# JamesBrofos/Stein

Measured on AMD Instinct MI355X. Metric: SVGD particle-updates/sec, higher is better.
Workload: dtype f32; 1 GPU; C3 bayesian-logreg-shaped synthetic block n=16384 d=256 fp32 (roofline config); n=16384, d=256, rows_per_rank=16384, optimizer=adagrad lr=1e-3 alpha=0.9, parallelism=single GPU

## Files before the change

stein_amd/csrc/stein_common.h:

```cpp
#pragma once

#include <hip/hip_runtime.h>
#include <stdint.h>
#include <math.h>

#include "steinhip.h"

typedef float f32x16 __attribute__((ext_vector_type(16)));
typedef unsigned long long u64;
typedef unsigned int u32;

int stein_fail(int code, const char* fmt, ...);

#define HIP_TRY(expr)                                                                          \
  do {                                                                                         \
    hipError_t e_ = (expr);                                                                    \
    if (e_ != hipSuccess) return stein_fail(STEIN_E_HIP, "%s: %s", #expr, hipGetErrorString(e_)); \
  } while (0)

#define LAUNCH_CHECK(name)                                                                           \
  do {                                                                                               \
    hipError_t e_ = hipGetLastError();                                                               \
    if (e_ != hipSuccess) return stein_fail(STEIN_E_HIP, "launch %s: %s", name, hipGetErrorString(e_)); \
  } while (0)

constexpr int BM = 128;
constexpr int BN = 128;
constexpr int BK = 32;
constexpr int NTHREADS = 256;

__device__ __forceinline__ int xcd_remap(int bid, int nblk) {
  const int q = nblk >> 3, r = nblk & 7, x = bid & 7;
  return (x < r ? x * (q + 1) : r * (q + 1) + (x - r) * q) + (bid >> 3);
}

constexpr int DT_ROWS = 128, DT_COLS = 32, DT_ELEMS = DT_ROWS * DT_COLS;
__host__ __device__ __forceinline__ size_t d_index(long row, long col, long ntc) {
  return ((size_t)(row >> 7) * ntc + (col >> 5)) * DT_ELEMS + (row & 127) * DT_COLS + (col & 31);
}

__device__ __forceinline__ float4 ld4_or_zero(const float* p, bool ok) {
  return ok ? *reinterpret_cast<const float4*>(p) : make_float4(0.f, 0.f, 0.f, 0.f);
}

constexpr int DSB = 8;
__host__ __device__ __forceinline__ long distance_grid(bool sym, int tiles_m, int tiles_n) {
  const long sm = (tiles_m + DSB - 1) / DSB, sn = (tiles_n + DSB - 1) / DSB;
  return (sym ? sn * (sn + 1) / 2 : sm * sn) * (DSB * DSB);
}
template <bool SYM>
__device__ __forceinline__ bool distance_tile(int logical, int tiles_m, int tiles_n, int& tile_m, int& tile_n) {
  const int sb = logical / (DSB * DSB), in = logical % (DSB * DSB);
  int sbm, sbn;
  if (SYM) {
    const int t_ = (tiles_n + DSB - 1) / DSB;
    int tm = (int)(((2.0 * t_ + 1.0) - sqrt((2.0 * t_ + 1.0) * (2.0 * t_ + 1.0) - 8.0 * (double)sb)) * 0.5);
    tm = max(0, min(tm, t_ - 1));
    while (tm > 0 && (long)tm * t_ - (long)tm * (tm - 1) / 2 > sb) --tm;
    while ((long)(tm + 1) * t_ - (long)(tm + 1) * tm / 2 <= sb) ++tm;
    sbm = tm;
    sbn = tm + (sb - (int)((long)tm * t_ - (long)tm * (tm - 1) / 2));
  } else {
    const int sn = (tiles_n + DSB - 1) / DSB;
    sbm = sb / sn;
    sbn = sb % sn;
  }
  tile_m = sbm * DSB + in / DSB;
  tile_n = sbn * DSB + in % DSB;
  return tile_m < tiles_m && tile_n < tiles_n && (!SYM || tile_n >= tile_m);
}

struct SelState {
  u64 rank[2];
  u32 prefix[2];
  u32 diverged;
  u32 even;
  float median;
  float h2;
  float lo, hi;
  u32 pad[4];
};
static_assert(sizeof(SelState) == 64, "SelState must stay 64 bytes");

struct SpecState {
  u32 magic;
  u32 center;
  u32 halfwidth;
  u32 lo_key;
  u32 width;
  u32 count;
  u32 overflow;
  u32 hit;
  u32 earned_hw;
  u32 reserved;
  u64 total;
  u32 last_key;
  u32 skip_l0;
  u32 n_steps;
  u32 n_hits;
};
static_assert(sizeof(SpecState) == 64, "SpecState must stay 64 bytes");
struct FuseState {
  u32 pad0[2];
  u32 gave_up;
  u32 folded;
  u32 pad[12];
};
static_assert(sizeof(FuseState) == 64, "FuseState must stay 64 bytes");
constexpr int HS_NV = 2048;
constexpr int HS_CLASSES = 64;
struct HistSync {
  u32 claim[STEIN_HIST_LEVELS][HS_NV];
  struct Leaf { u32 done; u32 pad[15]; } leaf[STEIN_HIST_LEVELS][HS_CLASSES];
  struct Top { u32 classes; u32 pad[15]; } top[STEIN_HIST_LEVELS];
  struct Line { u32 gen; u32 pub[6]; u32 pad[9]; } line[HS_CLASSES];
  Leaf fin_leaf[HS_CLASSES];
  Top fin_top;
  Leaf cm_leaf[HS_CLASSES];
  Top cm_top;
};
__device__ __forceinline__ bool tree_report_done(HistSync::Leaf* leaf, HistSync::Top* top, u32 id, u32 nblocks) {
  const u32 c = id % HS_CLASSES;
  const u32 quota = (nblocks - c + HS_CLASSES - 1) / HS_CLASSES;
  if (__hip_atomic_fetch_add(&leaf[c].done, 1u, __ATOMIC_RELAXED, __HIP_MEMORY_SCOPE_AGENT) + 1u != quota) return false;
  const u32 nclasses = nblocks < (u32)HS_CLASSES ? nblocks : (u32)HS_CLASSES;
  return __hip_atomic_fetch_add(&top->classes, 1u, __ATOMIC_RELAXED, __HIP_MEMORY_SCOPE_AGENT) + 1u == nclasses;
}
static_assert(sizeof(HistSync) % 8 == 0, "HistSync is carved out of a u64 table");
constexpr u32 SPEC_MAGIC1 = 0x5EED0001u, SPEC_MAGIC2 = 0x5EED0002u;
constexpr u32 SPEC_QCAP = 1016;
constexpr u32 SPEC_CAP = (1u << 21) - 2048u;
constexpr u32 SPEC_SLOTS = 256;
constexpr u32 SPEC_HW_MAX = 32767;
constexpr u32 SPEC_TABLE_HDR = 8;
constexpr u32 SPEC_TABLE = SPEC_TABLE_HDR + 2 * SPEC_HW_MAX + 2;
constexpr u32 SPEC_TABLE_AT = SPEC_SLOTS * 8 + SPEC_CAP;
static_assert(SPEC_TABLE_AT == (1u << 21), "the table starts 2^21 words into the SPEC section (stein_amd/_lib.py)");

__device__ __forceinline__ u32 f32_key(float x) {
  const u32 u = __float_as_uint(x);
  return (u & 0x80000000u) ? ~u : (u | 0x80000000u);
}
__device__ __forceinline__ float key_f32(u32 k) {
  return __uint_as_float((k & 0x80000000u) ? (k & 0x7fffffffu) : ~k);
}

struct MedianBw { float med, h2; };
__device__ __forceinline__ MedianBw median_bandwidth(float lo, float hi, u32 even, float ln_n) {
  MedianBw m;
  m.med = even ? 0.5f * (lo + hi) : lo;
  const float bw = sqrtf(m.med / ln_n);
  m.h2 = bw * bw;
  return m;
}

__device__ __forceinline__ void ksd_terms(float g, double og, float ot, float th, float rs, double ih, double& s, double& sd) {
  const double gd = g, dk = ((double)rs * (double)th - (double)ot) * ih;
  s += gd * og + 2.0 * (gd - (double)th * ih) * dk + (double)rs * ih;
  sd += gd * gd + ih;
}

__device__ __forceinline__ float elem_f32(const float* p) { return *p; }
__device__ __forceinline__ float elem_f32(const unsigned short* p) { return __uint_as_float((u32)*p << 16); }

template <typename TIN>
__device__ __forceinline__ float wave_row_sqnorm(const TIN* row, int d, int lane) {
  float s = 0.f;
  for (int k = lane; k < d; k += 64) {
    const float x = elem_f32(row + k);
    s = fmaf(x, x, s);
  }
#pragma unroll
  for (int o = 32; o > 0; o >>= 1) s += __shfl_xor(s, o);
  return s;
}

template <int N>
__device__ __forceinline__ void block_sum256(double (&v)[N], double* red) {
#pragma unroll
  for (int k = 0; k < N; ++k)
#pragma unroll
    for (int o = 32; o > 0; o >>= 1) v[k] += __shfl_xor(v[k], o);
  if ((threadIdx.x & 63) == 0) {
#pragma unroll
    for (int k = 0; k < N; ++k) red[4 * k + (threadIdx.x >> 6)] = v[k];
  }
  __syncthreads();
#pragma unroll
  for (int k = 0; k < N; ++k) v[k] = (red[4 * k] + red[4 * k + 1]) + (red[4 * k + 2] + red[4 * k + 3]);
}

__device__ __forceinline__ u64 load_fresh(const u64* p) { return __hip_atomic_load(p, __ATOMIC_RELAXED, __HIP_MEMORY_SCOPE_AGENT); }
__device__ __forceinline__ u32 load_fresh(const u32* p) { return __hip_atomic_load(p, __ATOMIC_RELAXED, __HIP_MEMORY_SCOPE_AGENT); }

__device__ __forceinline__ void hist_add(u32* h, u32 digit, bool valid, int lane, u32 w = 1u) {
#pragma unroll
  for (int it = 0; it < 2; ++it) {
    const u64 act = __ballot(valid);
    if (act == 0ull) return;
    const int leader = __ffsll((long long)act) - 1;
    const u32 ld = (u32)__builtin_amdgcn_readlane((int)digit, leader);
    const bool same = valid && digit == ld;
    const u64 m = __ballot(same);
    if (lane == leader) atomicAdd(&h[ld], (u32)__popcll(m) * w);
    valid = valid && !same;
  }
  if (valid) atomicAdd(&h[digit], w);
}

constexpr int EPI_STAGE_LD = 132;
constexpr int EPI_STAGE_BYTES = 64 * EPI_STAGE_LD * 4;
constexpr int EPI_LDS_BYTES = EPI_STAGE_BYTES + 8192 + 64 + 1024;

__device__ __forceinline__ void store_d4(float* p, float a, float b, float c, float d) {
  *reinterpret_cast<float4*>(p) = make_float4(a, b, c, d);
}

__device__ __forceinline__ void distance_store_rows(const float* __restrict__ stage, float* __restrict__ D, long ntc,
                                                    int tile_m, int brow0, int p) {
  const int t = threadIdx.x, f4 = t & 31;
#pragma unroll
  for (int k = 0; k < 8; ++k) {
    const int sr = (t >> 5) + 8 * k;
    const int row = tile_m * BM + (sr >> 5) * 64 + p * 32 + (sr & 31);
    const float4 v4 = *reinterpret_cast<const float4*>(stage + sr * EPI_STAGE_LD + 4 * f4);
    store_d4(D + d_index(row, brow0 + 4 * f4, ntc), v4.x, v4.y, v4.z, v4.w);
  }
}

struct SpecCtx {
  u32 lo, width;
  u32* qcnt;
  u64* q;
  u32 below;
};

template <bool MIRROR, bool PRED, bool DIAG, bool HIST, bool SPEC, bool STOREM>
__device__ __forceinline__ void distance_epilogue_body(const f32x16 (&acc)[2][2], u32* hl, float* __restrict__ D, int n,
                                                       int n_local, long ldD, int tile_m, int brow0, u32 base,
                                                       u64& packed, float two_s,
                                                       SpecCtx& sx, const float* rr, const float* rc, int i,
                                                       float* __restrict__ stage) {
  constexpr bool STAGED = !PRED && !DIAG;
  const long ntc = ldD >> 5;
  const int t = threadIdx.x, lane = t & 63, wid = t >> 6;
  const int wy = wid >> 1, wx = wid & 1;
  const int l31 = lane & 31, h4 = (lane >> 5) * 4;
  u32 below_cnt = 0u;
  {
#pragma unroll
    for (int j = 0; j < 2; ++j) {
      const int col = brow0 + wx * 64 + j * 32 + l31;
      const bool cok = !PRED || col < n;
      const float rj = rc[wx * 64 + j * 32 + l31];
#pragma unroll
      for (int g = 0; g < 4; ++g) {
        const int lrow4 = tile_m * BM + wy * 64 + i * 32 + 8 * g + h4;
        const float4 ri4 = *reinterpret_cast<const float4*>(rr + wy * 64 + i * 32 + 8 * g + h4);
        const float ris[4] = {ri4.x, ri4.y, ri4.z, ri4.w};
        float v[4];
        u32 wq[4];
#pragma unroll
        for (int q = 0; q < 4; ++q) {
          const int lrow = lrow4 + q;
          const bool rok = !PRED || lrow < n_local;
          v[q] = (ris[q] + rj) - two_s * acc[i][j][4 * g + q];
          u32 w = MIRROR ? 2u : 1u;
          if (DIAG) w = lrow < col ? 2u : (lrow == col ? 1u : 0u);
          if (PRED && !(cok && rok)) w = 0u;
          wq[q] = w;
          if ((!PRED && !DIAG) || w) {
            if (STAGED) stage[(wy * 32 + 8 * g + h4 + q) * EPI_STAGE_LD + wx * 64 + j * 32 + l31] = v[q];
            else D[d_index(lrow, col, ntc)] = v[q];
          }
        }
        if (DIAG) {
          if (wq[0] == 2u && wq[3] == 2u) {
            *reinterpret_cast<float4*>(D + d_index(col, lrow4, ntc)) = make_float4(v[0], v[1], v[2], v[3]);
          } else {
#pragma unroll
            for (int q = 0; q < 4; ++q)
              if (wq[q] == 2u) D[d_index(col, lrow4 + q, ntc)] = v[q];
          }
        }
        if (HIST) {
          u32 dg[4];
          bool far = false;
#pragma unroll
          for (int q = 0; q < 4; ++q) {
            dg[q] = f32_key(v[q]) >> 21;
            const u32 off = dg[q] - base;
            const bool near = off < 8u;
            packed += near ? (u64)wq[q] << (8u * (off & 7u)) : 0ull;
            far |= !near && wq[q] != 0u;
          }
          if (__builtin_expect(far, 0)) {
#pragma unroll
            for (int q = 0; q < 4; ++q)
              if (dg[q] - base >= 8u && wq[q]) atomicAdd(&hl[dg[q]], wq[q]);
          }
        }
        if (SPEC) {
          u32 off[4];
#pragma unroll
          for (int q = 0; q < 4; ++q) {
            const u32 raw = __float_as_uint(v[q]);
            const bool lower = (int)raw < (int)sx.lo;
            if (!PRED && !DIAG) below_cnt += lower ? 1u : 0u;
            else sx.below += lower ? wq[q] : 0u;
            off[q] = raw - sx.lo;
            if ((PRED || DIAG) && wq[q] == 0u) off[q] = 0xffffffffu;
          }
          if (__builtin_expect(min(min(off[0], off[1]), min(off[2], off[3])) <= sx.width, 0)) {
#pragma unroll
            for (int q = 0; q < 4; ++q)
              if (off[q] <= sx.width) {
                const u32 slot = atomicAdd(sx.qcnt, 1u);
                if (slot < SPEC_QCAP) sx.q[slot] = ((u64)(__float_as_uint(v[q]) | 0x80000000u) << 2) | wq[q];
              }
          }
        }
        if (MIRROR && STOREM && cok && (!PRED || lrow4 < n_local))
          store_d4(D + d_index(col, lrow4, ntc), v[0], v[1], v[2], v[3]);
      }
    }
  }
  if (SPEC && !PRED && !DIAG) sx.below += below_cnt * (MIRROR ? 2u : 1u);
}

struct EpiPrefetch {
  float norm;
  u32 lo_key, width;
};
__device__ __forceinline__ EpiPrefetch distance_epilogue_prefetch(const float* __restrict__ r, int n, int row0,
                                                                  int n_local, int tile_m, int tile_n,
                                                                  const SpecState* __restrict__ spec) {
  EpiPrefetch pf;
  const int t = threadIdx.x;
  const int idx = t < BM ? tile_m * BM + t : tile_n * BN + (t - BM);
  const bool ok = t < BM ? idx < n_local : idx < n;
  pf.norm = ok ? r[(t < BM ? row0 : 0) + idx] : 0.f;
  pf.lo_key = spec ? spec->lo_key : 0xffffffffu;
  pf.width = spec ? spec->width : 0u;
  return pf;
}

template <bool SYM, bool STORE_MIRROR = SYM>
__device__ __forceinline__ void distance_epilogue(const f32x16 (&acc)[2][2], u32* lds, float* __restrict__ D, int n,
                                                  int n_local, long ldD, int tile_m, int tile_n,
                                                  u64* __restrict__ hist0,
                                                  const EpiPrefetch& pf, float two_s = 2.f,
                                                  SpecState* __restrict__ spec = nullptr,
                                                  u64* __restrict__ spec_buf = nullptr) {
  const int t = threadIdx.x, lane = t & 63, wid = t >> 6;
  const int wy = wid >> 1, wx = wid & 1;
  const int brow0 = tile_n * BN;
  float* stage = reinterpret_cast<float*>(lds);
  u32* hl = lds + EPI_STAGE_BYTES / 4;
  u64 packed = 0ull;
  u32 base = 0u;
  SpecCtx sx;
  sx.lo = 0xffffffffu; sx.width = 0u; sx.below = 0u;
  sx.qcnt = hl + STEIN_HIST_BINS;
  sx.q = reinterpret_cast<u64*>(hl);
  static_assert(8 * SPEC_QCAP <= 4 * STEIN_HIST_BINS, "the window queue lives in the histogram's LDS");
  float* rr = reinterpret_cast<float*>(hl + STEIN_HIST_BINS + 16);
  float* rc = rr + BM;
  rr[t] = pf.norm;
  const bool window = spec && pf.width != 0u;
  const bool hist = hist0 && !window;
  if (window) {
    if (t == 0) { sx.qcnt[0] = 0u; sx.qcnt[2] = 0u; }
    sx.lo = pf.lo_key & 0x7fffffffu;
    sx.width = pf.width;
  }
  if (hist) {
    for (int b = t; b < STEIN_HIST_BINS; b += NTHREADS) hl[b] = 0u;
    __syncthreads();
    const float v0 = (rr[wy * 64] + rc[wx * 64]) - two_s * acc[0][0][0];
    base = (u32)__builtin_amdgcn_readfirstlane((int)(f32_key(v0) >> 21));
    base = base < 3u ? 0u : base - 3u;
  } else {
    __syncthreads();
  }
  const bool diag = SYM && tile_m == tile_n;
  const bool edge = brow0 + BN > n || tile_m * BM + BM > n_local;
#define STEIN_EPI_I(MIRROR, PRED, DIAG, I)                                                                             \
  do {                                                                                                                 \
    if (window)                                                                                                        \
      distance_epilogue_body<MIRROR, PRED, DIAG, false, true, STORE_MIRROR>(acc, hl, D, n, n_local, ldD, tile_m, brow0,             \
                                                              base, packed, two_s, sx, rr, rc, I, stage);             \
    else if (hist)                                                                                                     \
      distance_epilogue_body<MIRROR, PRED, DIAG, true, false, STORE_MIRROR>(acc, hl, D, n, n_local, ldD, tile_m, brow0,             \
                                                              base, packed, two_s, sx, rr, rc, I, stage);             \
    else                                                                                                               \
      distance_epilogue_body<MIRROR, PRED, DIAG, false, false, STORE_MIRROR>(acc, hl, D, n, n_local, ldD, tile_m, brow0,            \
                                                               base, packed, two_s, sx, rr, rc, I, stage);            \
  } while (0)
  const long ntc = ldD >> 5;
  if (diag) {
    STEIN_EPI_I(false, true, true, 0);
    STEIN_EPI_I(false, true, true, 1);
  } else if (edge) {
    STEIN_EPI_I(SYM, true, false, 0);
    STEIN_EPI_I(SYM, true, false, 1);
  } else {
    STEIN_EPI_I(SYM, false, false, 0);
    __syncthreads();
    distance_store_rows(stage, D, ntc, tile_m, brow0, 0);
    __syncthreads();
    STEIN_EPI_I(SYM, false, false, 1);
    __syncthreads();
    distance_store_rows(stage, D, ntc, tile_m, brow0, 1);
  }
#undef STEIN_EPI_I
  if (hist) {
#pragma unroll
    for (int k = 0; k < 8; ++k) {
      u32 c = (u32)(packed >> (8 * k)) & 255u;
#pragma unroll
      for (int o = 32; o > 0; o >>= 1) c += __shfl_xor(c, o);
      if (lane == 0 && c) atomicAdd(&hl[base + k], c);
    }
    __syncthreads();
    for (int b = t; b < STEIN_HIST_BINS; b += NTHREADS)
      if (hl[b]) atomicAdd(&hist0[b], (u64)hl[b]);
  }
  if (window) {
    u32 b = sx.below;
#pragma unroll
    for (int o = 32; o > 0; o >>= 1) b += __shfl_xor(b, o);
    if (lane == 0 && b) atomicAdd(&sx.qcnt[2], b);
    __syncthreads();
    if (t == 0 && sx.qcnt[2])
      atomicAdd(reinterpret_cast<unsigned long long*>(spec_buf + (blockIdx.x % SPEC_SLOTS) * 8),
                (unsigned long long)sx.qcnt[2]);
    const u32 pushed = sx.qcnt[0];
    const u32 nq = min(pushed, SPEC_QCAP);
    if (nq) {
      __syncthreads();
      if (t == 0) {
        if (pushed > SPEC_QCAP) spec->overflow = 1u;
        sx.qcnt[1] = atomicAdd(&spec->count, nq);
      }
      __syncthreads();
      const u32 gbase = sx.qcnt[1];
      for (u32 i = t; i < nq; i += NTHREADS)
        if (gbase + i < SPEC_CAP) spec_buf[SPEC_SLOTS * 8 + gbase + i] = sx.q[i];
    }
  }
}

__device__ __forceinline__ void phi_epilogue(const f32x16 (&acc)[2][2], const float (&rs)[4], float* __restrict__ Oz,
                                             float* __restrict__ RSz, int d, int n_local, int i0, int c0,
                                             bool write_rowsum) {
  const int t = threadIdx.x, lane = t & 63, wid = t >> 6;
  const int wy = wid >> 1, wx = wid & 1;
  const int l31 = lane & 31, h4 = (lane >> 5) * 4;
  const int lr = t >> 3;
#pragma unroll
  for (int i = 0; i < 2; ++i) {
#pragma unroll
    for (int j = 0; j < 2; ++j) {
      const int col = c0 + wx * 64 + j * 32 + l31;
      if (col >= d) continue;
#pragma unroll
      for (int e = 0; e < 16; ++e) {
        const int row = i0 + wy * 64 + i * 32 + (e & 3) + 8 * (e >> 2) + h4;
        if (row < n_local) Oz[(size_t)row * d + col] = acc[i][j][e];
      }
    }
  }
  if (write_rowsum) {
#pragma unroll
    for (int p = 0; p < 4; ++p) {
      float s = rs[p];
      s += __shfl_xor(s, 1);
      s += __shfl_xor(s, 2);
      s += __shfl_xor(s, 4);
      const int row = i0 + lr + 32 * p;
      if ((t & 7) == 0 && row < n_local) RSz[row] = s;
    }
  }
}

struct SteinLayout {
  size_t off[STEIN_WS_NSECTIONS];
  size_t total;
  int64_t ld_dist, split, sq_blocks, jchunk, tiles_m, cblocks;
  int64_t x3_rows, x3_dk;
  int64_t x3_dc, x3_nk;
  size_t x3_t3, x3_tt3, x3_gt3;
  size_t x3_sc;
  int64_t fold, fsplit, fjchunk;
  size_t fold_ow, fold_ot, fold_rs;
};
int stein_make_layout(int64_t n_local, int64_t n, int64_t d, int dtype, int flags, SteinLayout* L);

__device__ __forceinline__ void median_init_body(int gt, int gn, SelState* st, SpecState* sp, u64 total,
                                                 u64* __restrict__ hist, u64* __restrict__ slots, int allow_window = 1) {
  for (int i = gt; i < STEIN_HIST_LEVELS * 2 * STEIN_HIST_BINS; i += gn) hist[i] = 0ull;
  for (int i = gt; i < (int)SPEC_SLOTS * 8; i += gn) slots[i] = 0ull;
  if (gt) return;
  {
    const u32 even = (total & 1ull) ? 0u : 1u;
    st->rank[0] = even ? total / 2 - 1 : total / 2;
    st->rank[1] = total / 2;
    st->prefix[0] = st->prefix[1] = 0u;
    st->diverged = 0u;
    st->even = even;
    st->median = st->h2 = st->lo = st->hi = 0.f;
  }
  if (allow_window && (sp->magic == SPEC_MAGIC1 || sp->magic == SPEC_MAGIC2) && sp->halfwidth <= SPEC_HW_MAX &&
      sp->center >= 0x80000000u + sp->halfwidth && sp->center < 0xff000000u - sp->halfwidth) {
    sp->lo_key = sp->center - sp->halfwidth;
    sp->width = 2u * sp->halfwidth;
  } else {
    sp->lo_key = 0xffffffffu;
    sp->width = 0u;
  }
  sp->count = 0u; sp->overflow = 0u; sp->hit = 0u;
  sp->skip_l0 = sp->width == 0u ? 1u : 0u;
  sp->reserved = 0ull; sp->total = total;
}


struct PrologueArgs {
  int n, d;
  float* r;
  SelState* st; SpecState* sp; FuseState* fs;
  u64 total;
  u64* hist; u64* slots;
  u32* cmax; int ncmax;
  int allow_window;
  float* neutral_sc; int dc;
  u32* hsync; int hsync_words;
  u32 folded;
};
constexpr int PRO_INIT_BLOCKS = 16;
template <typename TIN>
__device__ __forceinline__ void prologue_body(const TIN* __restrict__ T, const PrologueArgs& a, int b, int nb) {
  const int gt = b * 256 + (int)threadIdx.x, gn = nb * 256;
  for (int i = gt; i < a.ncmax; i += gn) a.cmax[i] = 0u;
  if (a.neutral_sc) {
    for (int i = gt; i < 4 * a.dc; i += gn) a.neutral_sc[i] = 1.f;
    if (gt == 0) { a.neutral_sc[4 * a.dc] = 1.f; a.neutral_sc[4 * a.dc + 1] = 2.f; a.neutral_sc[4 * a.dc + 2] = 1.f; }
  }
  if (gt < 16) reinterpret_cast<u32*>(a.fs)[gt] = gt == 3 ? a.folded : 0u;
  for (int i = gt; i < a.hsync_words; i += gn) a.hsync[i] = 0u;
  median_init_body(gt, gn, a.st, a.sp, a.total, a.hist, a.slots, a.allow_window);
  const int lane = threadIdx.x & 63;
  for (int row = gt >> 6; row < a.n; row += gn >> 6) {
    const float s = wave_row_sqnorm(T + (size_t)row * a.d, a.d, lane);
    if (lane == 0) a.r[row] = s;
  }
}
```

stein_amd/csrc/stein_host.h:

```cpp
#pragma once

#include "stein_common.h"

#define fail stein_fail

constexpr int MAX_DEVICES = 64;

static inline int grid_for(long count, int cap) {
  long b = (count + 255) / 256;
  if (b > cap) b = cap;
  if (b < 1) b = 1;
  return (int)b;
}

static inline size_t align_up(size_t x, size_t a) { return (x + a - 1) / a * a; }

constexpr double RESIDENT_ONE_PER_CU = 256.0;

static inline int stein_check_size(int64_t n, int64_t d) {
  if (n > (1ll << 30) || d > (1ll << 24) || n * d > (1ll << 40)) return fail(STEIN_E_SHAPE, "shape too large");
  return STEIN_OK;
}

static inline SpecState* spec_of(void* select_state) { return (SpecState*)((char*)select_state + sizeof(SelState)); }
static inline FuseState* fuse_of(void* select_state) { return (FuseState*)((char*)spec_of(select_state) + sizeof(SpecState)); }
static inline u64* spec_table_of(void* spec_buf) { return (u64*)spec_buf + SPEC_TABLE_AT; }

struct BlockShape { int64_t n, d, row0, n_local; int dtype; };

static inline size_t x3_sc_two_s(int64_t dc) { return (size_t)(4 * dc + 1); }
static inline size_t x3_sc_cmax(int64_t dc) { return (size_t)(4 * dc + 4); }

struct StepViews {
  SteinLayout L;
  float* r; float* D; u64* hist;
  SelState* sel; SpecState* spec; FuseState* fuse;
  u64* spec_buf; u64* table;
  char* planes;
  unsigned short* T3; unsigned short* Tt3; unsigned short* Gt3;
  float* sc; u32* cmax; float* two_s;
  float* OG; float* OT; float* RS; double* SQ;
  int nsplit, jchunk, tsplit;
};
StepViews stein_step_views(const SteinLayout& L, void* workspace, void* planes_override = nullptr);
static inline int stein_staged_flags(bool x3) { return (x3 ? STEIN_FLAG_X3 : 0) | STEIN_FLAG_NO_FOLD; }
static inline int stein_rank_flags(int flags) {
  return (flags & (STEIN_FLAG_X3 | STEIN_FLAG_KSD)) | STEIN_FLAG_TILED | STEIN_FLAG_NO_FOLD;
}

int stein_rank_views(const BlockShape& b, void* workspace, size_t ws_bytes, int flags, StepViews* v);
int stein_rank_begin_on(const StepViews& v, const BlockShape& b, const void* theta_all, bool window, hipStream_t stream);
int stein_rank_pick_on(const StepViews& v, int64_t n, float* h2_out, float* median_out, void* flags_host, hipStream_t stream);
int stein_rank_radix_on(const StepViews& v, const BlockShape& b, int level, int need_pass, float* h2_out, float* median_out,
                        hipStream_t stream);
int stein_rank_finish_on(const StepViews& v, const BlockShape& b, const void* theta_all, const void* score_all,
                         const float* h2_dev, float* phi_local, double* sqnorm_out, float* dK_out, int flags,
                         hipStream_t stream);

int stein_device_error_word(u32** out);
int stein_take_device_error(void);

int stein_stream_jsplit_hook(void);

int stein_fused_select(const StepViews& v, int64_t n, int64_t d, float* h2_out, const void* theta_all, const void* score_all,
                       hipStream_t stream);

int stein_fp32_distance(const StepViews& v, const BlockShape& b, const float* theta_all, bool symmetric, bool window,
                        hipStream_t stream);
int stein_fp32_contract_partial(const StepViews& v, const BlockShape& b, const float* theta_all, const float* score_all,
                                const float* h2_dev, hipStream_t stream);

bool stein_small_ok(int64_t n, int64_t d, int dtype);
int stein_small_phi(const float* theta, const float* score, int64_t n, int64_t d, float* phi, float* h2_out,
                    double* sqpart ,
                    float* K_out, float* dK_out, int* nparts ,
                    double* sqnorm_out, bool ksd ,
                    hipStream_t stream);
```

stein_amd/csrc/stein_select.hip:

```cpp

#include <hip/hip_runtime.h>
#include <stdint.h>
#include <math.h>

#include "stein_host.h"

__global__ void k_sel_init(SelState* st, u64 total) {
  if (threadIdx.x == 0 && blockIdx.x == 0) {
    const u32 even = (total & 1ull) ? 0u : 1u;
    st->rank[0] = even ? total / 2 - 1 : total / 2;
    st->rank[1] = total / 2;
    st->prefix[0] = st->prefix[1] = 0u;
    st->diverged = 0u;
    st->even = even;
    st->median = st->h2 = st->lo = st->hi = 0.f;
  }
}

struct ChainState { u32 prefix[2]; u64 rank[2]; bool two; };
template <bool FRESH>
__device__ __attribute__((noinline)) ChainState chain_resolve(const u64* hist_all, int levels, const SelState* st) {
  __shared__ u64 c_part[256];
  __shared__ u32 c_bin[2];
  __shared__ u64 c_rest[2];
  const int t = threadIdx.x;
  ChainState cs;
  cs.prefix[0] = cs.prefix[1] = 0u;
  cs.rank[0] = st->rank[0]; cs.rank[1] = st->rank[1];
  cs.two = false;
  for (int level = 0; level < levels; ++level) {
    const int bits = level == 2 ? 10 : 11;
    const u64* hl = hist_all + (size_t)level * 2 * STEIN_HIST_BINS;
    for (int tg = 0; tg < 2; ++tg) {
      const u64* src = hl + ((cs.two && tg == 1) ? STEIN_HIST_BINS : 0);
      u64 mine[8], sum = 0;
#pragma unroll
      for (int k = 0; k < 8; ++k) { mine[k] = FRESH ? load_fresh(src + t * 8 + k) : src[t * 8 + k]; sum += mine[k]; }
      c_part[t] = sum;
      __syncthreads();
      for (int o = 1; o < 256; o <<= 1) {
        u64 v = 0;
        if (t >= o) v = c_part[t - o];
        __syncthreads();
        c_part[t] += v;
        __syncthreads();
      }
      const u64 excl = c_part[t] - sum, rank = cs.rank[tg];
      if (t == 255 && rank >= c_part[255]) { c_bin[tg] = (u32)((1 << bits) - 1); c_rest[tg] = 0; }
      if (rank >= excl && rank < excl + sum) {
        u64 cum = excl;
        int k = 0;
        while (k < 7 && cum + mine[k] <= rank) cum += mine[k++];
        c_bin[tg] = (u32)(t * 8 + k);
        c_rest[tg] = rank - cum;
      }
      __syncthreads();
      cs.prefix[tg] = (cs.prefix[tg] << bits) | c_bin[tg];
      cs.rank[tg] = c_rest[tg];
      __syncthreads();
    }
    cs.two = cs.prefix[0] != cs.prefix[1];
  }
  return cs;
}

struct HistFinal {
  SelState* st;
  SpecState* sp;
  float* h2_out;
  float ln_n;
};
__device__ __attribute__((noinline)) void resolve_all_body(u64* hist_all, SelState* st, SpecState* sp, float ln_n, float* h2_out);

template <int LEVEL, bool SYM>
__device__ __forceinline__ void hist_pass_body(const float* __restrict__ D, long ldD, int n_local, int n, u32* h, u32 pa, u32 pb,
                                               bool two, long vb, long nvb) {
  const int lane = threadIdx.x & 63;
  const long ntc = ldD >> 5;
  const int ntr = (n_local + DT_ROWS - 1) / DT_ROWS, ncol_tiles = (n + DT_COLS - 1) / DT_COLS;
  const int vrows = SYM ? (ntr + 1) / 2 : ntr;
  const int W = SYM ? 2 * ncol_tiles - 4 * (ntr - 1) : ncol_tiles;
  const long units = (long)vrows * W;
  for (long u = vb; u < units; u += nvb) {
    int ti, tj;
    if (SYM) {
      const int v = (int)(u / W), x = (int)(u - (long)v * W), len0 = ncol_tiles - 4 * v;
      if (x < len0) { ti = v; tj = 4 * v + x; }
      else {
        ti = ntr - 1 - v;
        if (ti == v) continue;
        tj = 4 * ti + (x - len0);
      }
      if (tj >= ncol_tiles) continue;
    } else {
      ti = (int)(u / ncol_tiles); tj = (int)(u - (long)ti * ncol_tiles);
    }
    const float* tile = D + ((size_t)ti * ntc + tj) * DT_ELEMS;
    float4 v4[4];
#pragma unroll
    for (int q = 0; q < 4; ++q) v4[q] = *reinterpret_cast<const float4*>(tile + (threadIdx.x + 256 * q) * 4);
    const bool interior = ti * DT_ROWS + DT_ROWS <= n_local && tj * DT_COLS + DT_COLS <= n &&
                          (!SYM || tj * DT_COLS >= ti * DT_ROWS + DT_ROWS);
    if (interior) {
      constexpr u32 WT = SYM ? 2u : 1u;
#pragma unroll
      for (int q = 0; q < 4; ++q) {
        const float x[4] = {v4[q].x, v4[q].y, v4[q].z, v4[q].w};
#pragma unroll
        for (int e = 0; e < 4; ++e) {
          const u32 key = f32_key(x[e]);
          if (LEVEL == 0) {
            hist_add(h, key >> 21, true, lane, WT);
          } else {
            const u32 digit = LEVEL == 1 ? ((key >> 10) & 2047u) : (key & 1023u);
            const u32 hi = LEVEL == 1 ? (key >> 21) : (key >> 10);
            if (hi == pa) atomicAdd(&h[digit], WT);
            if (two && hi == pb) atomicAdd(&h[STEIN_HIST_BINS + digit], WT);
          }
        }
      }
      continue;
    }
#pragma unroll
    for (int q = 0; q < 4; ++q) {
      const int f = threadIdx.x + 256 * q;
      const int row = ti * DT_ROWS + (f >> 3), c0 = tj * DT_COLS + (f & 7) * 4;
      const float x[4] = {v4[q].x, v4[q].y, v4[q].z, v4[q].w};
#pragma unroll
      for (int e = 0; e < 4; ++e) {
        const int col = c0 + e;
        const bool inb = row < n_local && col < n && (!SYM || col >= row);
        const u32 key = f32_key(x[e]);
        const u32 w = (SYM && col != row) ? 2u : 1u;
        if (LEVEL == 0) {
          if (SYM) {
            hist_add(h, key >> 21, inb && col != row, lane, 2u);
            if (inb && col == row) atomicAdd(&h[key >> 21], 1u);
          } else {
            hist_add(h, key >> 21, inb, lane);
          }
        } else {
          const u32 digit = LEVEL == 1 ? ((key >> 10) & 2047u) : (key & 1023u);
          const u32 hi = LEVEL == 1 ? (key >> 21) : (key >> 10);
          if (inb && hi == pa) atomicAdd(&h[digit], w);
          if (two && inb && hi == pb) atomicAdd(&h[STEIN_HIST_BINS + digit], w);
        }
      }
    }
  }
}

template <int LEVEL, bool SYM>
__global__ __launch_bounds__(256) void k_hist(const float* __restrict__ D, long ldD, int n_local, int n,
                                              const SelState* st, u64* hist, const u32* __restrict__ skip) {
  if (skip && *skip) return;
  __shared__ u32 h[2 * STEIN_HIST_BINS];
  for (int b = threadIdx.x; b < 2 * STEIN_HIST_BINS; b += 256) h[b] = 0u;
  __syncthreads();
  const u32 pa = st->prefix[0], pb = st->prefix[1];
  const bool two = st->diverged != 0u;
  hist_pass_body<LEVEL, SYM>(D, ldD, n_local, n, h, pa, pb, two, blockIdx.x, gridDim.x);
  __syncthreads();
  for (int b = threadIdx.x; b < (two ? 2 : 1) * STEIN_HIST_BINS; b += 256)
    if (h[b]) atomicAdd(&hist[b], (u64)h[b]);
}

constexpr int HIST_SPIN_MAX = 1 << 20;
constexpr int HIST_PATIENCE = 160;
constexpr int HIST_BLOCKS = 2048;
constexpr int HIST_ALL_SMALL_N = 4096;
constexpr int HIST_ALL_VBLOCKS = 512;
static_assert(sizeof(HistSync) <= (size_t)SPEC_TABLE * 8, "HistSync lives in the window table");
static_assert(HIST_BLOCKS <= HS_NV, "HistSync::claim holds one flag per virtual workgroup");

__device__ __forceinline__ bool hs_report_done(HistSync* hs, int level, u32 v, u32 nvb) {
  return tree_report_done(hs->leaf[level], &hs->top[level], v, nvb);
}
__device__ __attribute__((noinline)) u32 hs_steal(HistSync* hs, int level, u32 nvb) {
  __shared__ u32 s_first, s_got;
  for (u32 attempt = 0;; ++attempt) {
    if (threadIdx.x == 0) s_first = nvb;
    __syncthreads();
    const u32 start = (blockIdx.x * 1021u + attempt * 97u) % nvb;
    u32 mine = nvb;
    for (u32 i = threadIdx.x; i < nvb; i += 256) {
      u32 v = start + i;
      if (v >= nvb) v -= nvb;
      if (load_fresh(&hs->claim[level][v]) == 0u) { mine = i; break; }
    }
    if (mine < nvb) atomicMin(&s_first, mine);
    __syncthreads();
    const u32 pos = s_first;
    if (pos >= nvb) return nvb;
    u32 cand = start + pos;
    if (cand >= nvb) cand -= nvb;
    if (threadIdx.x == 0)
      s_got = __hip_atomic_exchange(&hs->claim[level][cand], 1u, __ATOMIC_RELAXED, __HIP_MEMORY_SCOPE_AGENT) == 0u ? 1u : 0u;
    __syncthreads();
    const bool got = s_got != 0u;
    __syncthreads();
    if (got) return cand;
  }
}

__device__ __forceinline__ bool hs_wait(const u32* gen, u32 want, int max_polls) {
  int nap = 1;
  for (int spin = 0; spin < max_polls; ++spin) {
    if (load_fresh(gen) >= want) return true;
    for (int k = 0; k < nap; ++k) __builtin_amdgcn_s_sleep(8);
    if (spin >= 32 && nap < 8) nap += nap;
  }
  return false;
}

template <int LEVEL>
__device__ __attribute__((noinline)) void hist_pass_sym(const float* __restrict__ D, long ldD, int n, u32* h, u32 pa, u32 pb,
                                                        bool two, u32 v, u32 nvb) {
  hist_pass_body<LEVEL, true>(D, ldD, n, n, h, pa, pb, two, v, nvb);
}

__global__ __launch_bounds__(256) void k_hist_all(const float* __restrict__ D, long ldD, int n, const SelState* st, u64* hist_all,
                                                  const u32* __restrict__ hit, const u32* __restrict__ skip_l0, HistFinal fin,
                                                  FuseState* fs, HistSync* hs , u32 nvb,
                                                  u32* errword ) {
  if (*hit) return;
  __shared__ u32 h[2 * STEIN_HIST_BINS];
  __shared__ u32 s_v, s_flag;
  const int first = *skip_l0 == 0u ? 0 : 1;
  ChainState cs = chain_resolve<false>(hist_all, first, st);
  const HistSync::Line* myline = &hs->line[blockIdx.x % HS_CLASSES];
  for (int level = first; level < STEIN_HIST_LEVELS; ++level) {
    const u32 want = (u32)(level - first + 1);
    if (threadIdx.x == 0)
      s_v = blockIdx.x < nvb && __hip_atomic_exchange(&hs->claim[level][blockIdx.x], 1u, __ATOMIC_RELAXED, __HIP_MEMORY_SCOPE_AGENT) == 0u
                ? blockIdx.x : nvb;
    bool last = false, thief = false;
    for (;;) {
      for (int b = threadIdx.x; b < 2 * STEIN_HIST_BINS; b += 256) h[b] = 0u;
      __syncthreads();
      const u32 v = s_v;
      if (v < nvb) {
        if (level == 0) hist_pass_sym<0>(D, ldD, n, h, cs.prefix[0], cs.prefix[1], cs.two, v, nvb);
        else if (level == 1) hist_pass_sym<1>(D, ldD, n, h, cs.prefix[0], cs.prefix[1], cs.two, v, nvb);
        else hist_pass_sym<2>(D, ldD, n, h, cs.prefix[0], cs.prefix[1], cs.two, v, nvb);
        __syncthreads();
        u64* hl = hist_all + (size_t)level * 2 * STEIN_HIST_BINS;
        for (int b = threadIdx.x; b < (cs.two ? 2 : 1) * STEIN_HIST_BINS; b += 256)
          if (h[b]) atomicAdd(&hl[b], (u64)h[b]);
        asm volatile("s_waitcnt vmcnt(0)" ::: "memory");
        __syncthreads();
        if (threadIdx.x == 0) s_flag = hs_report_done(hs, level, v, nvb) ? 1u : 0u;
        __syncthreads();
        last = s_flag != 0u;
        if (last) break;
      }
      if (!thief) {
        __syncthreads();
        if (threadIdx.x == 0) s_flag = hs_wait(&myline->gen, want, HIST_PATIENCE) ? 1u : 0u;
        __syncthreads();
        if (s_flag) break;
        thief = true;
      }
      const u32 more = hs_steal(hs, level, nvb);
      if (more < nvb) {
        if (threadIdx.x == 0) s_v = more;
        __syncthreads();
        continue;
      }
      if (threadIdx.x == 0) {
        const bool ok = hs_wait(&myline->gen, want, HIST_SPIN_MAX);
        if (!ok) __hip_atomic_store(&fs->gave_up, 1u, __ATOMIC_RELAXED, __HIP_MEMORY_SCOPE_AGENT);
      }
      __syncthreads();
      break;
    }
    const bool final_level = level + 1 == STEIN_HIST_LEVELS;
    if (last) {
      if (final_level) {
        resolve_all_body(hist_all, fin.st, fin.sp, fin.ln_n, fin.h2_out);
        if (threadIdx.x == 0 && load_fresh(&fs->gave_up)) {
          fin.st->median = fin.st->h2 = __builtin_nanf("");
          if (fin.h2_out) *fin.h2_out = __builtin_nanf("");
          if (errword) __hip_atomic_store(errword, 1u, __ATOMIC_RELAXED, __HIP_MEMORY_SCOPE_SYSTEM);
        }
      } else {
        cs = chain_resolve<true>(hist_all, level + 1, st);
      }
      if (threadIdx.x < HS_CLASSES) {
        HistSync::Line* ln = &hs->line[threadIdx.x];
        const u32 w[6] = {cs.prefix[0], cs.prefix[1], (u32)cs.rank[0], (u32)(cs.rank[0] >> 32), (u32)cs.rank[1], (u32)(cs.rank[1] >> 32)};
#pragma unroll
        for (int k = 0; k < 6; ++k) __hip_atomic_store(&ln->pub[k], w[k], __ATOMIC_RELAXED, __HIP_MEMORY_SCOPE_AGENT);
        asm volatile("s_waitcnt vmcnt(0)" ::: "memory");
        __hip_atomic_store(&ln->gen, want, __ATOMIC_RELAXED, __HIP_MEMORY_SCOPE_AGENT);
      }
      continue;
    }
    if (final_level) return;
    u32 w[6];
#pragma unroll
    for (int k = 0; k < 6; ++k) w[k] = load_fresh(&myline->pub[k]);
    cs.prefix[0] = w[0]; cs.prefix[1] = w[1];
    cs.rank[0] = (u64)w[2] | ((u64)w[3] << 32); cs.rank[1] = (u64)w[4] | ((u64)w[5] << 32);
    cs.two = w[0] != w[1];
  }
}

__global__ __launch_bounds__(64) void k_resolve(const u64* __restrict__ hist, int level, SelState* st, float ln_n,
                                                float* h2_out, float* median_out, const u32* __restrict__ skip) {
  if (skip && *skip) return;
  __shared__ u64 bins[STEIN_HIST_BINS];
  __shared__ u64 chunk[64];
  const int lane = threadIdx.x;
  const int bits = level == 2 ? 10 : 11;
  const bool div_in = st->diverged != 0u;
  u32 newp[2];
  u64 newr[2];
  for (int tg = 0; tg < 2; ++tg) {
    const u64* src = hist + ((div_in && tg == 1) ? STEIN_HIST_BINS : 0);
    u64 s = 0;
    for (int b = 0; b < 32; ++b) {
      const u64 c = src[lane * 32 + b];
      bins[lane * 32 + b] = c;
      s += c;
    }
    chunk[lane] = s;
    __syncthreads();
    if (lane == 0) {
      u64 rank = st->rank[tg], cum = 0;
      int c = 0;
      while (c < 63 && cum + chunk[c] <= rank) cum += chunk[c++];
      int b = c * 32;
      const int bend = b + 31;
      while (b < bend && cum + bins[b] <= rank) cum += bins[b++];
      newp[tg] = (st->prefix[tg] << bits) | (u32)b;
      newr[tg] = rank - cum;
    }
    __syncthreads();
  }
  if (lane == 0) {
    st->prefix[0] = newp[0]; st->prefix[1] = newp[1];
    st->rank[0] = newr[0]; st->rank[1] = newr[1];
    st->diverged = (newp[0] != newp[1]) ? 1u : 0u;
    if (level == 2) {
      const float lo = key_f32(newp[0]), hi = key_f32(newp[1]);
      const MedianBw m = median_bandwidth(lo, hi, st->even, ln_n);
      st->lo = lo; st->hi = hi; st->median = m.med; st->h2 = m.h2;
      if (h2_out) *h2_out = m.h2;
      if (median_out) *median_out = m.med;
    }
  }
}

__global__ __launch_bounds__(256) void k_median_init(SelState* st, SpecState* sp, u64 total, u64* __restrict__ hist,
                                                     u64* __restrict__ slots) {
  median_init_body(blockIdx.x * 256 + threadIdx.x, gridDim.x * 256, st, sp, total, hist, slots);
}
__device__ __attribute__((noinline)) void spec_update_dev(const SelState* st, SpecState* sp);

__device__ __forceinline__ void spec_locate2(const u32* hA, u32 rankA, const u32* hB, u32 rankB, u32* scan, u32* bin, u32* rest) {
  const int t = threadIdx.x, lane = t & 63, wave = t >> 6;
  const int side = t >> 8;
  u32 c = 0u, incl = 0u;
  if (t < 512) {
    c = (side ? hB : hA)[t & 255];
    incl = c;
#pragma unroll
    for (int o = 1; o < 64; o <<= 1) {
      const u32 v = __shfl_up(incl, o);
      if (lane >= o) incl += v;
    }
    if (lane == 63) scan[wave] = incl;
  }
  if (t < 2) bin[t] = 256u;
  __syncthreads();
  if (t < 512) {
    u32 base = 0u;
    for (int w = side * 4; w < wave; ++w) base += scan[w];
    const u32 excl = base + incl - c, rank = side ? rankB : rankA;
    if (excl <= rank && rank < excl + c) { bin[side] = (u32)(t & 255); rest[side] = rank - excl; }
  }
  __syncthreads();
}

__device__ __forceinline__ bool spec_select_body(SelState* st, SpecState* sp, const u64* __restrict__ slots, float ln_n,
                                                 float* h2_out, int update) {
  const u64* __restrict__ buf = slots + SPEC_SLOTS * 8;
  __shared__ u32 h1[256], h2a[256], h2b[256], scan[256];
  __shared__ u32 sel[8];
  __shared__ u64 below_s;
  const int t = threadIdx.x;
  const u32 cnt = sp->count, lo = sp->lo_key, width = sp->width;
  if (width == 0u || sp->overflow || cnt > SPEC_CAP || cnt == 0u) return false;
  u32 even0 = 0u;
  if (t == 0) even0 = st->even;
  u64 mine = t < (int)SPEC_SLOTS ? slots[t * 8] : 0ull;
  const u64 total = sp->total;
  if (t == 0) below_s = 0ull;
  if (t < 256) { h1[t] = 0u; h2a[t] = 0u; h2b[t] = 0u; }
  __syncthreads();
  {
#pragma unroll
    for (int o = 32; o > 0; o >>= 1) mine += __shfl_xor(mine, o);
    if ((t & 63) == 0 && mine) atomicAdd(reinterpret_cast<unsigned long long*>(&below_s), (unsigned long long)mine);
  }
  __syncthreads();
  const u64 below = below_s;
  const u64 r0 = (total & 1ull) ? total / 2 : total / 2 - 1, r1 = total / 2;
  if (r0 < below || r1 - below > 0xfffffff0ull) return false;
  constexpr int EPT = 16;
  const bool inreg = cnt <= 1024u * EPT;
  const u32 nb = (width >> 8) + 1u;
  u64 er[EPT];
  if (inreg) {
#pragma unroll
    for (int k = 0; k < EPT; ++k) {
      const u32 i = (u32)k * 1024u + (u32)t;
      er[k] = (u32)k * 1024u < cnt && i < cnt ? buf[i] : 0ull;
    }
  }
  if (inreg && nb <= 8u) {
    u32 c[8] = {0u, 0u, 0u, 0u, 0u, 0u, 0u, 0u};
#pragma unroll
    for (int k = 0; k < EPT; ++k) {
      if ((u32)k * 1024u < cnt) {
        const u64 e = er[k];
        const u32 hb = (((u32)(e >> 2) - lo) >> 8) & 255u, w = (u32)e & 3u;
#pragma unroll
        for (int b = 0; b < 8; ++b) c[b] += hb == (u32)b ? w : 0u;
      }
    }
#pragma unroll
    for (int b = 0; b < 8; ++b) {
      if ((u32)b < nb) {
        u32 v = c[b];
#pragma unroll
        for (int o = 32; o > 0; o >>= 1) v += __shfl_xor(v, o);
        if ((t & 63) == 0 && v) atomicAdd(&h1[b], v);
      }
    }
  } else if (inreg) {
#pragma unroll
    for (int k = 0; k < EPT; ++k) {
      if ((u32)k * 1024u < cnt) {
        const u64 e = er[k];
        const u32 hb = (((u32)(e >> 2) - lo) >> 8) & 255u, w = (u32)e & 3u;
        hist_add(h1, hb, w == 2u, t & 63, 2u);
        hist_add(h1, hb, w == 1u, t & 63, 1u);
        if (w == 3u) atomicAdd(&h1[hb], 3u);
      }
    }
  } else {
    for (u32 i0 = 0; i0 < cnt; i0 += 1024) {
      const u32 i = i0 + (u32)t;
      const bool ok = i < cnt;
      const u64 e = ok ? buf[i] : 0ull;
      const u32 hb = (((u32)(e >> 2) - lo) >> 8) & 255u, w = (u32)e & 3u;
      hist_add(h1, hb, ok && w == 2u, t & 63, 2u);
      hist_add(h1, hb, ok && w == 1u, t & 63, 1u);
      if (ok && w == 3u) atomicAdd(&h1[hb], 3u);
    }
  }
  __syncthreads();
  spec_locate2(h1, (u32)(r0 - below), h1, (u32)(r1 - below), scan, &sel[0], &sel[2]);
  const u32 ba = sel[0], bb = sel[1];
  if (ba == 256u || bb == 256u) return false;
  const bool two_hb = ba != bb;
  if (inreg) {
#pragma unroll
    for (int k = 0; k < EPT; ++k) {
      if ((u32)k * 1024u < cnt) {
        const u64 e = er[k];
        const u32 o = (u32)(e >> 2) - lo, w = (u32)e & 3u;
        if (w && (o >> 8) == ba) atomicAdd(&h2a[o & 255u], w);
        if (w && two_hb && (o >> 8) == bb) atomicAdd(&h2b[o & 255u], w);
      }
    }
  } else {
    for (u32 i = t; i < cnt; i += 1024) {
      const u64 e = buf[i];
      const u32 o = (u32)(e >> 2) - lo, w = (u32)e & 3u;
      if ((o >> 8) == ba) atomicAdd(&h2a[o & 255u], w);
      if (two_hb && (o >> 8) == bb) atomicAdd(&h2b[o & 255u], w);
    }
  }
  __syncthreads();
  spec_locate2(h2a, sel[2], two_hb ? h2b : h2a, sel[3], scan, &sel[4], &sel[6]);
  if (t == 0) {
    const float flo = key_f32(lo + ((ba << 8) | sel[4])), fhi = key_f32(lo + ((bb << 8) | sel[5]));
    const MedianBw m = median_bandwidth(flo, fhi, even0, ln_n);
    st->lo = flo; st->hi = fhi; st->median = m.med; st->h2 = m.h2;
    if (h2_out) *h2_out = m.h2;
    sp->hit = 1u;
    sp->skip_l0 = 1u;
    if (update) spec_update_dev(st, sp);
  }
  return true;
}

constexpr int SOLO_MAX_N = 512;
__device__ __forceinline__ void solo_locate(const u32* h, u32 rank, u32* wsum, u32* out_bin, u32* out_rest) {
  const int t = threadIdx.x, lane = t & 63, wave = t >> 6;
  const u32 c0 = h[2 * t], c1 = h[2 * t + 1];
  u32 incl = c0 + c1;
#pragma unroll
  for (int o = 1; o < 64; o <<= 1) {
    const u32 v = __shfl_up(incl, o);
    if (lane >= o) incl += v;
  }
  if (lane == 63) wsum[wave] = incl;
  __syncthreads();
  u32 base = 0u;
  for (int w = 0; w < wave; ++w) base += wsum[w];
  const u32 excl = base + incl - (c0 + c1);
  if (rank >= excl && rank < excl + c0 + c1) {
    const u32 b = rank < excl + c0 ? 2u * t : 2u * t + 1u;
    *out_bin = b;
    *out_rest = rank - ((b & 1u) ? excl + c0 : excl);
  }
  __syncthreads();
}
__device__ __forceinline__ void solo_select(const float* __restrict__ D, long ldD, int n, SelState* st, SpecState* sp,
                                            float ln_n, float* h2_out) {
  __shared__ u32 sh[2 * STEIN_HIST_BINS];
  __shared__ u32 s_wsum[16], s_bin[2], s_rest[2];
  const int t = threadIdx.x;
  const long ntc = ldD >> 5;
  const int ntr = (n + DT_ROWS - 1) / DT_ROWS, nct = (n + DT_COLS - 1) / DT_COLS;
  const u32 total = (u32)n * (u32)n;
  u32 prefix[2] = {0u, 0u};
  u32 rank[2] = {(total & 1u) ? total / 2 : total / 2 - 1, total / 2};
  bool two = false;
  for (int level = 0; level < STEIN_HIST_LEVELS; ++level) {
    const int bits = level == 2 ? 10 : 11, shift = level == 0 ? 21 : (level == 1 ? 10 : 0);
    for (int b = t; b < 2 * STEIN_HIST_BINS; b += 1024) sh[b] = 0u;
    __syncthreads();
    for (int ti = 0; ti < ntr; ++ti)
      for (int tj = 0; tj < nct; ++tj) {
        if (tj * DT_COLS + DT_COLS <= ti * DT_ROWS) continue;
        const float4 v4 = *reinterpret_cast<const float4*>(D + ((size_t)ti * ntc + tj) * DT_ELEMS + t * 4);
        const int row = ti * DT_ROWS + (t >> 3), c0 = tj * DT_COLS + (t & 7) * 4;
        const float x[4] = {v4.x, v4.y, v4.z, v4.w};
#pragma unroll
        for (int e = 0; e < 4; ++e) {
          const int col = c0 + e;
          if (row < n && col < n && col >= row) {
            const u32 key = f32_key(x[e]), w = col != row ? 2u : 1u;
            const u32 digit = (key >> shift) & ((1u << bits) - 1u);
            const u32 hi = level == 0 ? 0u : key >> (shift + bits);
            if (level == 0 || hi == prefix[0]) atomicAdd(&sh[digit], w);
            if (two && hi == prefix[1]) atomicAdd(&sh[STEIN_HIST_BINS + digit], w);
          }
        }
      }
    __syncthreads();
    solo_locate(sh, rank[0], s_wsum, &s_bin[0], &s_rest[0]);
    solo_locate(sh + (two ? STEIN_HIST_BINS : 0), rank[1], s_wsum, &s_bin[1], &s_rest[1]);
    prefix[0] = (prefix[0] << bits) | s_bin[0];
    prefix[1] = (prefix[1] << bits) | s_bin[1];
    rank[0] = s_rest[0];
    rank[1] = s_rest[1];
    two = prefix[0] != prefix[1];
    __syncthreads();
  }
  if (t == 0) {
    st->prefix[0] = prefix[0]; st->prefix[1] = prefix[1];
    st->rank[0] = rank[0]; st->rank[1] = rank[1];
    st->diverged = two ? 1u : 0u;
    const float lo = key_f32(prefix[0]), hi = key_f32(prefix[1]);
    const MedianBw m = median_bandwidth(lo, hi, st->even, ln_n);
    st->lo = lo; st->hi = hi; st->median = m.med; st->h2 = m.h2;
    if (h2_out) *h2_out = m.h2;
    spec_update_dev(st, sp);
  }
}

__global__ __launch_bounds__(1024) void k_spec_select(SelState* st, SpecState* sp, const u64* __restrict__ slots,
                                                      float ln_n, float* h2_out, int update,
                                                      const float* __restrict__ D, long ldD, int n,
                                                      const float4* __restrict__ warm0, const float4* __restrict__ warm1,
                                                      long warm4) {
  if (blockIdx.x) {
    const long stride = (long)(gridDim.x - 1) * 1024;
    auto keep = [](const float4& a) { asm volatile("" ::"v"(a.x), "v"(a.y), "v"(a.z), "v"(a.w)); };
    long i = (long)(blockIdx.x - 1) * 1024 + threadIdx.x;
    for (; i + 3 * stride < warm4; i += 4 * stride) {
      const float4 a0 = warm0[i], a1 = warm0[i + stride], a2 = warm0[i + 2 * stride], a3 = warm0[i + 3 * stride];
      const float4 b0 = warm1[i], b1 = warm1[i + stride], b2 = warm1[i + 2 * stride], b3 = warm1[i + 3 * stride];
      keep(a0); keep(a1); keep(a2); keep(a3); keep(b0); keep(b1); keep(b2); keep(b3);
    }
    for (; i < warm4; i += stride) {
      const float4 a0 = warm0[i], b0 = warm1[i];
      keep(a0); keep(b0);
    }
    return;
  }
  const bool hit = spec_select_body(st, sp, slots, ln_n, h2_out, update);
  if (!hit && D) {
    __syncthreads();
    solo_select(D, ldD, n, st, sp, ln_n, h2_out);
  }
}

__global__ __launch_bounds__(256) void k_spec_tally(const SpecState* __restrict__ sp, const u64* __restrict__ slots,
                                                    u64* __restrict__ table) {
  const u64* __restrict__ buf = slots + SPEC_SLOTS * 8;
  const u32 cnt = sp->count, lo = sp->lo_key;
  const bool bad = sp->width == 0u || sp->overflow || cnt > SPEC_CAP;
  if (blockIdx.x == 0) {
    if (threadIdx.x < (int)SPEC_SLOTS && slots[threadIdx.x * 8])
      atomicAdd(reinterpret_cast<unsigned long long*>(&table[0]), (unsigned long long)slots[threadIdx.x * 8]);
    if (threadIdx.x == 0) {
      if (bad) atomicAdd(reinterpret_cast<unsigned long long*>(&table[1]), 1ull);
      atomicAdd(reinterpret_cast<unsigned long long*>(&table[2]), (unsigned long long)cnt);
    }
  }
  if (bad) return;
  for (u32 i = blockIdx.x * 256 + threadIdx.x; i < cnt; i += gridDim.x * 256) {
    const u64 e = buf[i];
    atomicAdd(reinterpret_cast<unsigned long long*>(&table[SPEC_TABLE_HDR + ((u32)(e >> 2) - lo)]),
              (unsigned long long)(e & 3ull));
  }
}

__global__ __launch_bounds__(1024) void k_spec_pick(SelState* st, SpecState* sp, const u64* __restrict__ table,
                                                    float ln_n, float* h2_out, float* median_out) {
  __shared__ u64 part[1024];
  __shared__ u32 found[2];
  const int t = threadIdx.x;
  const u32 width = sp->width, lo = sp->lo_key;
  if (t == 0) sp->count = table[2] > 0xffffffffull ? 0xffffffffu : (u32)table[2];
  if (width == 0u || table[1] != 0ull) return;
  const u64 total = sp->total, below = table[0];
  const u64 r0 = (total & 1ull) ? total / 2 : total / 2 - 1, r1 = total / 2;
  if (r0 < below) return;
  constexpr int PER = 64;
  u64 mine = 0ull;
  for (int k = 0; k < PER; ++k) {
    const u32 key = (u32)t * PER + k;
    if (key <= width) mine += table[SPEC_TABLE_HDR + key];
  }
  part[t] = mine;
  if (t < 2) found[t] = 0xffffffffu;
  __syncthreads();
  for (int o = 1; o < 1024; o <<= 1) {
    u64 v = 0ull;
    if (t >= o) v = part[t - o];
    __syncthreads();
    part[t] += v;
    __syncthreads();
  }
  const u64 excl = part[t] - mine;
  for (int tg = 0; tg < 2; ++tg) {
    const u64 rank = (tg ? r1 : r0) - below;
    if (excl <= rank && rank < excl + mine) {
      u64 cum = excl;
      for (int k = 0; k < PER; ++k) {
        const u64 c = table[SPEC_TABLE_HDR + (u32)t * PER + k];
        if (rank < cum + c) { found[tg] = (u32)t * PER + k; break; }
        cum += c;
      }
    }
  }
  __syncthreads();
  if (t == 0 && found[0] != 0xffffffffu && found[1] != 0xffffffffu) {
    const float flo = key_f32(lo + found[0]), fhi = key_f32(lo + found[1]);
    const MedianBw m = median_bandwidth(flo, fhi, st->even, ln_n);
    st->lo = flo; st->hi = fhi; st->median = m.med; st->h2 = m.h2;
    if (h2_out) *h2_out = m.h2;
    if (median_out) *median_out = m.med;
    sp->hit = 1u;
    sp->skip_l0 = 1u;
  }
}

__device__ __attribute__((noinline)) void spec_update_dev(const SelState* st, SpecState* sp) {
  const u32 key = f32_key(st->lo);
  const bool had_window = sp->width != 0u;
  u32 hw = 4096u, next = key, earned = 0u;
  if (sp->magic == SPEC_MAGIC1 || sp->magic == SPEC_MAGIC2) {
    const float pred = 2.f * st->lo - key_f32(sp->last_key);
    long c = (long)f32_key(pred == pred ? pred : st->lo);
    c = c < 65536l ? 65536l : (c > 0xfffe0000l ? 0xfffe0000l : c);
    next = (u32)c;
    if (sp->magic == SPEC_MAGIC2 && had_window) {
      const u32 err = key > sp->center ? key - sp->center : sp->center - key;
      hw = err > SPEC_HW_MAX / 4u ? SPEC_HW_MAX : 4u * err + 48u;
      const u32 floor_hw = sp->earned_hw - sp->earned_hw / 4u;
      if (hw < floor_hw) hw = floor_hw;
      earned = hw;
      if (sp->hit && sp->count > SPEC_CAP / 2 && hw > sp->halfwidth / 2u) hw = sp->halfwidth / 2u + 1u;
    }
    sp->magic = SPEC_MAGIC2;
    sp->n_steps += 1u;
    sp->n_hits += sp->hit ? 1u : 0u;
  } else {
    sp->magic = SPEC_MAGIC1;
    sp->n_steps = 1u;
    sp->n_hits = 0u;
  }
  sp->last_key = key;
  sp->center = next;
  sp->halfwidth = hw > SPEC_HW_MAX ? SPEC_HW_MAX : hw;
  sp->earned_hw = earned > SPEC_HW_MAX ? SPEC_HW_MAX : earned;
}
__global__ void k_spec_update(const SelState* st, SpecState* sp) {
  if (threadIdx.x || blockIdx.x) return;
  spec_update_dev(st, sp);
}

__device__ __attribute__((noinline)) void resolve_all_body(u64* hist_all, SelState* st, SpecState* sp, float ln_n, float* h2_out) {
  const ChainState cs = chain_resolve<true>(hist_all, STEIN_HIST_LEVELS, st);
  if (threadIdx.x == 0) {
    st->prefix[0] = cs.prefix[0]; st->prefix[1] = cs.prefix[1];
    st->rank[0] = cs.rank[0]; st->rank[1] = cs.rank[1];
    st->diverged = cs.two ? 1u : 0u;
    const float lo = key_f32(cs.prefix[0]), hi = key_f32(cs.prefix[1]);
    const MedianBw m = median_bandwidth(lo, hi, st->even, ln_n);
    st->lo = lo; st->hi = hi; st->median = m.med; st->h2 = m.h2;
    if (h2_out) *h2_out = m.h2;
    spec_update_dev(st, sp);
  }
}

extern "C" int stein_median_begin(void* hist, void* select_state, int64_t total, void* stream) {
  if (!hist || !select_state) return fail(STEIN_E_BADARG, "NULL pointer");
  if (total < 1) return fail(STEIN_E_SHAPE, "total < 1");
  HIP_TRY(hipMemsetAsync(hist, 0, (size_t)STEIN_HIST_LEVELS * 2 * STEIN_HIST_BINS * 8, (hipStream_t)stream));
  hipLaunchKernelGGL(k_sel_init, dim3(1), dim3(64), 0, (hipStream_t)stream, (SelState*)select_state,
                     (u64)total);
  LAUNCH_CHECK("k_sel_init");
  return STEIN_OK;
}

template <int LEVEL>
static void launch_hist(bool sym, int blocks, hipStream_t s, const float* dist, long ld, int n_local, int n,
                        const SelState* st, u64* h, const u32* skip) {
  if (sym)
    hipLaunchKernelGGL((k_hist<LEVEL, true>), dim3(blocks), dim3(256), 0, s, dist, ld, n_local, n, st, h, skip);
  else
    hipLaunchKernelGGL((k_hist<LEVEL, false>), dim3(blocks), dim3(256), 0, s, dist, ld, n_local, n, st, h, skip);
}

extern "C" int stein_median_hist_pass(const float* dist, int64_t ld_dist, int64_t n_local, int64_t n, int level,
                                      const void* select_state, void* hist, int flags, void* stream) {
  if (!dist || !select_state || !hist) return fail(STEIN_E_BADARG, "NULL pointer");
  if (level < 0 || level >= STEIN_HIST_LEVELS) return fail(STEIN_E_BADARG, "level %d", level);
  if (ld_dist < n || (ld_dist & 31) || n_local < 1) return fail(STEIN_E_SHAPE, "bad distance block shape (ld_dist must be a multiple of 32)");
  const bool sym = (flags & STEIN_STAGE_SYMMETRIC) != 0;
  if (sym && n_local != n) return fail(STEIN_E_BADARG, "STEIN_STAGE_SYMMETRIC needs a square block");
  const long units = ((n_local + DT_ROWS - 1) / DT_ROWS) * ((n + DT_COLS - 1) / DT_COLS);
  const int blocks = (int)(units < HIST_BLOCKS ? units : HIST_BLOCKS);
  u64* h = (u64*)hist + (size_t)level * 2 * STEIN_HIST_BINS;
  const SelState* st = (const SelState*)select_state;
  hipStream_t s = (hipStream_t)stream;
  if (level == 0) launch_hist<0>(sym, blocks, s, dist, (long)ld_dist, (int)n_local, (int)n, st, h, nullptr);
  else if (level == 1) launch_hist<1>(sym, blocks, s, dist, (long)ld_dist, (int)n_local, (int)n, st, h, nullptr);
  else launch_hist<2>(sym, blocks, s, dist, (long)ld_dist, (int)n_local, (int)n, st, h, nullptr);
  LAUNCH_CHECK("k_hist");
  return STEIN_OK;
}

extern "C" int stein_median_resolve(const void* hist, int level, int64_t n, void* select_state, float* h2_out,
                                    float* median_out, void* stream) {
  if (!hist || !select_state) return fail(STEIN_E_BADARG, "NULL pointer");
  if (level < 0 || level >= STEIN_HIST_LEVELS) return fail(STEIN_E_BADARG, "level %d", level);
  if (n < 2) return fail(STEIN_E_BADARG, "n = %lld: need n >= 2", (long long)n);
  const u64* h = (const u64*)hist + (size_t)level * 2 * STEIN_HIST_BINS;
  const float ln_n = (float)log((double)n);
  hipLaunchKernelGGL(k_resolve, dim3(1), dim3(64), 0, (hipStream_t)stream, h, level, (SelState*)select_state, ln_n,
                     h2_out, median_out, nullptr);
  LAUNCH_CHECK("k_resolve");
  return STEIN_OK;
}

extern "C" int stein_spec_begin(void* hist, void* select_state, void* spec_buf, int64_t total, void* stream) {
  if (!hist || !select_state || !spec_buf) return fail(STEIN_E_BADARG, "NULL pointer");
  if (total < 1) return fail(STEIN_E_SHAPE, "total < 1");
  hipLaunchKernelGGL(k_median_init, dim3(16), dim3(256), 0, (hipStream_t)stream, (SelState*)select_state,
                     spec_of(select_state), (u64)total, (u64*)hist, (u64*)spec_buf);
  LAUNCH_CHECK("k_median_init");
  return STEIN_OK;
}

extern "C" int stein_spec_tally(void* select_state, void* spec_buf, void* stream) {
  if (!select_state || !spec_buf) return fail(STEIN_E_BADARG, "NULL pointer");
  u64* table = spec_table_of(spec_buf);
  HIP_TRY(hipMemsetAsync(table, 0, (size_t)SPEC_TABLE * 8, (hipStream_t)stream));
  hipLaunchKernelGGL(k_spec_tally, dim3(256), dim3(256), 0, (hipStream_t)stream, spec_of(select_state),
                     (const u64*)spec_buf, table);
  LAUNCH_CHECK("k_spec_tally");
  return STEIN_OK;
}

extern "C" int stein_spec_pick(void* select_state, void* spec_buf, int64_t n, float* h2_out, float* median_out,
                               void* stream) {
  if (!select_state || !spec_buf) return fail(STEIN_E_BADARG, "NULL pointer");
  if (n < 2) return fail(STEIN_E_BADARG, "n = %lld: need n >= 2", (long long)n);
  hipLaunchKernelGGL(k_spec_pick, dim3(1), dim3(1024), 0, (hipStream_t)stream, (SelState*)select_state,
                     spec_of(select_state), (const u64*)spec_table_of(spec_buf), (float)log((double)n), h2_out,
                     median_out);
  LAUNCH_CHECK("k_spec_pick");
  return STEIN_OK;
}

extern "C" int stein_spec_update(void* select_state, void* stream) {
  if (!select_state) return fail(STEIN_E_BADARG, "NULL pointer");
  hipLaunchKernelGGL(k_spec_update, dim3(1), dim3(64), 0, (hipStream_t)stream, (const SelState*)select_state,
                     spec_of(select_state));
  LAUNCH_CHECK("k_spec_update");
  return STEIN_OK;
}

static thread_local int g_hist_all_grid = 0, g_hist_all_nvb = 0;
constexpr int SPEC_WARM_WGS = 255;
static thread_local int g_no_warm = 0;
extern "C" int stein_debug_no_warm(int off) {
  if (off != 0 && off != 1) return fail(STEIN_E_BADARG, "off %d", off);
  g_no_warm = off;
  return STEIN_OK;
}
extern "C" int stein_debug_hist_all_grid(int blocks) {
  if (blocks < 0 || blocks > 65535) return fail(STEIN_E_BADARG, "blocks %d", blocks);
  g_hist_all_grid = blocks;
  return STEIN_OK;
}
extern "C" int stein_debug_hist_all_vblocks(int nvb) {
  if (nvb < 0 || nvb > 65535) return fail(STEIN_E_BADARG, "nvb %d", nvb);
  g_hist_all_nvb = nvb;
  return STEIN_OK;
}

int stein_fused_select(const StepViews& v, int64_t n, int64_t d, float* h2_out, const void* theta_all,
                       const void* score_all, hipStream_t s) {
  const bool solo = n <= SOLO_MAX_N;
  long warm4 = 0;
  int warm_wgs = 0;
  if (v.L.fold && !g_no_warm && theta_all && score_all && (((uintptr_t)theta_all | (uintptr_t)score_all) & 15u) == 0) {
    warm4 = (long)(n * d) >> 2;
    const long want = (warm4 + 8191) / 8192;
    warm_wgs = (int)(want < SPEC_WARM_WGS ? want : SPEC_WARM_WGS);
  }
  hipLaunchKernelGGL(k_spec_select, dim3(1 + warm_wgs), dim3(1024), 0, s, v.sel, v.spec, v.spec_buf, (float)log((double)n),
                     h2_out, 1, solo ? (const float*)v.D : (const float*)nullptr, (long)v.L.ld_dist, (int)n,
                     (const float4*)theta_all, (const float4*)score_all, warm4);
  LAUNCH_CHECK("k_spec_select");
  if (solo) return STEIN_OK;
  const HistFinal fin{v.sel, v.spec, h2_out, (float)log((double)n)};
  const long units = ((n + DT_ROWS - 1) / DT_ROWS) * ((n + DT_COLS - 1) / DT_COLS);
  long want = HIST_ALL_VBLOCKS;
  if (n > HIST_ALL_SMALL_N) {
    static int resident[MAX_DEVICES];
    int dev = 0;
    HIP_TRY(hipGetDevice(&dev));
    const bool cached = dev >= 0 && dev < MAX_DEVICES;
    int res = cached ? __atomic_load_n(&resident[dev], __ATOMIC_RELAXED) : 0;
    if (!res) {
      int per_cu = 0, ncu = 0;
      HIP_TRY(hipOccupancyMaxActiveBlocksPerMultiprocessor(&per_cu, k_hist_all, 256, 0));
      HIP_TRY(hipDeviceGetAttribute(&ncu, hipDeviceAttributeMultiprocessorCount, dev));
      const long r = (long)(per_cu > 0 ? per_cu : 4) * (ncu > 0 ? ncu : 256);
      res = (int)(r > HIST_BLOCKS ? HIST_BLOCKS : r);
      if (cached) __atomic_store_n(&resident[dev], res, __ATOMIC_RELAXED);
    }
    want = res;
  }
  if (g_hist_all_nvb > 0) want = g_hist_all_nvb;
  if (want > HS_NV) want = HS_NV;
  const int nvb = (int)(units < want ? units : want);
  const int blocks = g_hist_all_grid > 0 ? g_hist_all_grid : nvb;
  u32* errword = nullptr;
  if (int rc = stein_device_error_word(&errword)) return rc;
  hipLaunchKernelGGL(k_hist_all, dim3(blocks), dim3(256), 0, s, (const float*)v.D, (long)v.L.ld_dist, (int)n,
                     (const SelState*)v.sel, v.hist, (const u32*)&v.spec->hit, (const u32*)&v.spec->skip_l0, fin, v.fuse,
                     (HistSync*)v.table, (u32)nvb, errword);
  LAUNCH_CHECK("k_hist_all");
  return STEIN_OK;
}
```

stein_amd/csrc/stein_x3.h:

```cpp
#pragma once
#include "stein_host.h"

int stein_x3_kind(int dtype);
struct SplitFused {
  HistSync* done;
  const PrologueArgs* prologue;
  int fold;
};
int stein_x3_split(const StepViews& v, const void* theta_all, const void* score_all, int dtype, int64_t n, int64_t d,
                   hipStream_t stream, const SplitFused* fused);
bool stein_fold_pays(int64_t n, int64_t d);
int stein_x3_split_w(const StepViews& v, const float* theta_all, const float* score_all, int64_t n, int64_t d,
                     const float* h2_dev, hipStream_t stream);
int stein_x3_contract_fold(const StepViews& v, const float* h2_dev, int64_t n, int64_t d, bool with_theta,
                           hipStream_t stream);
int stein_x3_distance(const StepViews& v, const BlockShape& b, bool symmetric, bool window, hipStream_t stream,
                      int panel );
bool stein_dpanel_ok(const StepViews& v, const BlockShape& b, bool any_size);
int stein_dpanel_distance(const StepViews& v, const BlockShape& b, bool symmetric, bool window, hipStream_t stream);
int stein_x3_contract_partial(const StepViews& v, const BlockShape& b, const float* h2_dev, hipStream_t stream,
                              bool upper );
```

stein_amd/csrc/stein_x3.hip:

```cpp

#include "stein_x3.h"

#include <stdlib.h>

#include "stein_x3_dev.h"
template <int KIND> struct SplitTraits { static constexpr int pexp = KIND == 2 ? PEXP_H2 : 0; };

#include <type_traits>

__device__ __forceinline__ int xswz(int row, int chunk) { return (chunk ^ ((row >> 2) & 3)) * 16; }

__device__ __forceinline__ u32 cvt_pk_bf16(float lo, float hi) {
  u32 r;
  asm("v_cvt_pk_bf16_f32 %0, %1, %2" : "=v"(r) : "v"(lo), "v"(hi));
  return r;
}

template <int KIND>
__device__ __forceinline__ void split_pair(float x, float y, u32 (&w)[3]) {
  if (KIND == 2) {
    w[0] = cvt_pk_f16(x, y);
    w[1] = cvt_pk_f16(f16_resid_lo(w[0], x), f16_resid_hi(w[0], y));
  } else {
    w[0] = cvt_pk_bf16(x, y);
  }
}

__device__ __forceinline__ u32 abs_bits(float v) { return __float_as_uint(v) & 0x7fffffffu; }
__device__ __forceinline__ u32 abs_bits(u16 v) { return ((u32)v << 16) & 0x7fffffffu; }

__device__ __forceinline__ void make_scales_body(const u32* cmax, int dc, float* __restrict__ sc, int pexp, int enable,
                                                 u32* red) {
  const int t = threadIdx.x;
  u32 m = 0u;
  for (int c = t; c < dc; c += 256) {
    const u32 mg = load_fresh(cmax + c), mt = load_fresh(cmax + dc + c);
    const int sg = enable ? scale_exp(mg, 100) : 0, st = enable ? scale_exp(mt, 100) : 0;
    sc[c] = pow2i(sg);
    sc[dc + c] = pow2i(st);
    sc[2 * dc + c] = pow2i(-sg - pexp);
    sc[3 * dc + c] = pow2i(-st - pexp);
    m = max(m, mt);
  }
  red[t] = m;
  __syncthreads();
  for (int o = 128; o > 0; o >>= 1) {
    if (t < o) red[t] = max(red[t], red[t + o]);
    __syncthreads();
  }
  if (t == 0) {
    const int sa = enable ? scale_exp(red[0], 60) : 0;
    sc[4 * dc + 0] = pow2i(sa);
    sc[4 * dc + 1] = pow2i(1 - 2 * sa);
    sc[4 * dc + 2] = pow2i(-pexp);
  }
}

template <typename TIN, bool V4>
__global__ __launch_bounds__(V4 ? 1024 : 256) void k_colmax(const TIN* __restrict__ X0, const TIN* __restrict__ X1, int n, int d,
                                                            u32* __restrict__ cmax0, int dc, int zbase, float* __restrict__ sc,
                                                            int pexp, HistSync* done) {
  const int z = blockIdx.z + zbase;
  const TIN* __restrict__ X = z ? X1 : X0;
  u32* __restrict__ cmax = cmax0 + (z ? dc : 0);
  constexpr int CW = V4 ? 4 : 1;
  constexpr int NW = V4 ? 16 : 4;
  __shared__ u32 red[NW][64 * CW];
  const int t = threadIdx.x, cx = t & 63, ry = t >> 6;
  const int col = (blockIdx.x * 64 + cx) * CW;
  u32 m[CW];
#pragma unroll
  for (int e = 0; e < CW; ++e) m[e] = 0u;
  if (col < d) {
    const long step = (long)gridDim.y * NW;
    long r = (long)blockIdx.y * NW + ry;
    if constexpr (V4) {
      if constexpr (std::is_same<TIN, float>::value) {
        u32 m1[4] = {0u, 0u, 0u, 0u}, m2[4] = {0u, 0u, 0u, 0u}, m3[4] = {0u, 0u, 0u, 0u};
        auto ld = [&](long row) { return *reinterpret_cast<const float4*>(X + (size_t)row * d + col); };
        auto up = [&](u32 (&acc)[4], const float4& v) {
          acc[0] = max(acc[0], abs_bits(v.x)); acc[1] = max(acc[1], abs_bits(v.y));
          acc[2] = max(acc[2], abs_bits(v.z)); acc[3] = max(acc[3], abs_bits(v.w));
        };
        for (; r + 3 * step < n; r += 4 * step) {
          const float4 a0 = ld(r), a1 = ld(r + step), a2 = ld(r + 2 * step), a3 = ld(r + 3 * step);
          up(m, a0); up(m1, a1); up(m2, a2); up(m3, a3);
        }
        for (; r < n; r += step) { const float4 a0 = ld(r); up(m, a0); }
#pragma unroll
        for (int e = 0; e < 4; ++e) m[e] = max(max(m[e], m1[e]), max(m2[e], m3[e]));
      }
    } else {
      u32 m1 = 0u, m2 = 0u, m3 = 0u;
      for (; r + 3 * step < n; r += 4 * step) {
        const u32 a0 = abs_bits(X[(size_t)r * d + col]), a1 = abs_bits(X[(size_t)(r + step) * d + col]);
        const u32 a2 = abs_bits(X[(size_t)(r + 2 * step) * d + col]), a3 = abs_bits(X[(size_t)(r + 3 * step) * d + col]);
        m[0] = max(m[0], a0); m1 = max(m1, a1); m2 = max(m2, a2); m3 = max(m3, a3);
      }
      for (; r < n; r += step) m[0] = max(m[0], abs_bits(X[(size_t)r * d + col]));
      m[0] = max(max(m[0], m1), max(m2, m3));
    }
  }
#pragma unroll
  for (int e = 0; e < CW; ++e) red[ry][cx * CW + e] = m[e];
  __syncthreads();
  if (t < 64 * CW) {
    const int c = blockIdx.x * 64 * CW + t;
    if (c < d) {
      u32 v = 0u;
#pragma unroll
      for (int w = 0; w < NW; ++w) v = max(v, red[w][t]);
      atomicMax(&cmax[c], v);
    }
  }
  if (done) {
    __shared__ u32 s_last;
    asm volatile("s_waitcnt vmcnt(0)" ::: "memory");
    __syncthreads();
    if (t == 0) {
      const u32 id = (blockIdx.z * gridDim.y + blockIdx.y) * gridDim.x + blockIdx.x;
      s_last = tree_report_done(done->cm_leaf, &done->cm_top, id, gridDim.x * gridDim.y * gridDim.z) ? 1u : 0u;
    }
    __syncthreads();
    if (s_last) make_scales_body(cmax0, dc, sc, pexp, 1, &red[0][0]);
  }
}

__global__ __launch_bounds__(256) void k_make_scales(const u32* __restrict__ cmax, int dc, float* __restrict__ sc, int pexp,
                                                     int enable) {
  __shared__ u32 red[256];
  make_scales_body(cmax, dc, sc, pexp, enable, red);
}

constexpr int TP_WORDS = 64 * 32;
__device__ __forceinline__ int tp_index(int c, int p) { return c * 32 + ((((p >> 2) ^ (c >> 2)) & 7) << 2) + (p & 3); }
__device__ __forceinline__ int tp_pair(int t, int pass) { return 16 * pass + 4 * (t >> 6) + (((t >> 4) & 3) ^ ((t >> 2) & 2)); }

template <typename TIN>
__device__ __forceinline__ void load_row4(const TIN* __restrict__ X, int row, int col, int n, int d, int vec, float (&v)[4]) {
  if constexpr (std::is_same<TIN, float>::value) {
    if (vec) {
      const float4 x = (row < n && col < d) ? *reinterpret_cast<const float4*>(X + (size_t)row * d + col) : make_float4(0.f, 0.f, 0.f, 0.f);
      v[0] = x.x; v[1] = x.y; v[2] = x.z; v[3] = x.w;
      return;
    }
  }
#pragma unroll
  for (int q = 0; q < 4; ++q) v[q] = (row < n && col + q < d) ? elem_f32(X + (size_t)row * d + col + q) : 0.f;
}

template <int KIND>
__device__ __forceinline__ void tp_store(const u32 (*tile)[TP_WORDS], u16* __restrict__ Tt, long ntk_t, int dc, long nk,
                                         int row0, int col0, int t) {
  const int c = col0 + (t >> 2), j = row0 + (t & 3) * 16;
  if (c < dc && j < nk) {
    const int rowc = c & 127, ch0 = (j & 31) >> 3;
#pragma unroll
    for (int s = 0; s < KIND; ++s) {
      const uint4 w0 = *reinterpret_cast<const uint4*>(&tile[s][tp_index(t >> 2, (t & 3) * 8)]);
      const uint4 w1 = *reinterpret_cast<const uint4*>(&tile[s][tp_index(t >> 2, (t & 3) * 8 + 4)]);
      u16* base = Tt + (((size_t)(c >> 7) * ntk_t + (j >> 5)) * 3 + s) * XTILE_E;
      *reinterpret_cast<uint4*>(base + vfrag_offset(rowc, ch0)) = w0;
      *reinterpret_cast<uint4*>(base + vfrag_offset(rowc, ch0 + 1)) = w1;
    }
  }
}

template <typename TIN, int KIND, bool PRO = false>
__global__ __launch_bounds__(256) void k_split(const TIN* __restrict__ X0, const TIN* __restrict__ X1, int n, int d,
                                               u16* __restrict__ R0, long r_rows, int dk, u16* __restrict__ Tt0,
                                               u16* __restrict__ Tt1, int dc, long nk, const float* __restrict__ sc,
                                               int zbase, PrologueArgs pro, int vec) {
  if (PRO && blockIdx.z == gridDim.z - 1) {
    prologue_body<TIN>(X0, pro, (int)(blockIdx.y * gridDim.x + blockIdx.x), (int)(gridDim.x * gridDim.y));
    return;
  }
  const bool score = blockIdx.z + zbase != 0;
  if (score && ((int)blockIdx.x * 64 >= dc || (long)blockIdx.y * 64 >= nk)) return;
  const TIN* __restrict__ X = score ? X1 : X0;
  u16* __restrict__ R = score ? nullptr : R0;
  u16* __restrict__ Tt = score ? Tt1 : Tt0;
  const float* __restrict__ sc_all = sc + 4 * dc;
  const float* __restrict__ sc_col = sc + (score ? 0 : dc);
  __shared__ __attribute__((aligned(16))) u32 tile[KIND][TP_WORDS];
  const int t = threadIdx.x;
  const int row0 = blockIdx.y * 64, col0 = blockIdx.x * 64;
  const int lc = (t & 15) * 4;
  const long ntk_r = dk >> 5, ntk_t = nk >> 5;
  const float sa = (R && !PRO) ? *sc_all : 1.f;
  float scq[4];
#pragma unroll
  for (int q = 0; q < 4; ++q) scq[q] = (!PRO && Tt && col0 + lc + q < dc) ? sc_col[col0 + lc + q] : 1.f;
#pragma unroll
  for (int p = 0; p < 2; ++p) {
    const int pr = tp_pair(t, p), col = col0 + lc;
    float v[2][4];
#pragma unroll
    for (int h = 0; h < 2; ++h) {
      const int row = row0 + 2 * pr + h;
      load_row4(X, row, col, n, d, vec, v[h]);
      if (R && row < r_rows && col < dk) {
        u32 wa[3], wb[3];
        split_pair<KIND>(v[h][0] * sa, v[h][1] * sa, wa);
        split_pair<KIND>(v[h][2] * sa, v[h][3] * sa, wb);
        u16* dst = R + (((size_t)(row >> 7) * ntk_r + (col >> 5)) * 3) * XTILE_E + vfrag_offset(row & 127, (col & 31) >> 3) + (col & 7);
#pragma unroll
        for (int s = 0; s < KIND; ++s) *reinterpret_cast<uint2*>(dst + s * XTILE_E) = make_uint2(wa[s], wb[s]);
      }
    }
    if (Tt) {
#pragma unroll
      for (int q = 0; q < 4; ++q) {
        u32 w[3];
        split_pair<KIND>(v[0][q] * scq[q], v[1][q] * scq[q], w);
#pragma unroll
        for (int s = 0; s < KIND; ++s) tile[s][tp_index(lc + q, pr)] = w[s];
      }
    }
  }
  if (!Tt) return;
  __syncthreads();
  tp_store<KIND>(tile, Tt, ntk_t, dc, nk, row0, col0, t);
}

__global__ __launch_bounds__(256) void k_split_w(const float* __restrict__ T, const float* __restrict__ G, int n, int d,
                                                 u16* __restrict__ Wt, int dc, long nk, float* __restrict__ sc,
                                                 const u32* __restrict__ cmax, const float* __restrict__ h2p, int vec) {
  __shared__ __attribute__((aligned(16))) u32 tile[2][TP_WORDS];
  const int t = threadIdx.x;
  const int row0 = blockIdx.y * 64, col0 = blockIdx.x * 64;
  const int lc = (t & 15) * 4;
  const long ntk_t = nk >> 5;
  const float ih = 1.f / *h2p;
  float scq[4];
#pragma unroll
  for (int q = 0; q < 4; ++q) {
    const int c = col0 + lc + q;
    int se = 0;
    if (c < dc) se = scale_exp(__float_as_uint(__builtin_fmaf(__uint_as_float(cmax[dc + c]), ih, __uint_as_float(cmax[c]))), 100);
    scq[q] = pow2i(se);
    if (blockIdx.y == 0 && (t >> 4) == 0 && c < dc) {
      sc[c] = scq[q];
      sc[2 * dc + c] = pow2i(-se - PEXP_H2);
    }
  }
#pragma unroll
  for (int p = 0; p < 2; ++p) {
    const int pr = tp_pair(t, p), col = col0 + lc;
    float v[2][4];
#pragma unroll
    for (int h = 0; h < 2; ++h) {
      const int row = row0 + 2 * pr + h;
      float th[4], g[4];
      load_row4(T, row, col, n, d, vec, th);
      load_row4(G, row, col, n, d, vec, g);
#pragma unroll
      for (int q = 0; q < 4; ++q) v[h][q] = (row < n && col + q < d) ? __builtin_fmaf(-th[q], ih, g[q]) : 0.f;
    }
#pragma unroll
    for (int q = 0; q < 4; ++q) {
      u32 w[3];
      split_pair<2>(v[0][q] * scq[q], v[1][q] * scq[q], w);
#pragma unroll
      for (int s = 0; s < 2; ++s) tile[s][tp_index(lc + q, pr)] = w[s];
    }
  }
  __syncthreads();
  tp_store<2>(tile, Wt, ntk_t, dc, nk, row0, col0, t);
}

__device__ __forceinline__ const u16* t3_chunk_ptr(const u16* __restrict__ T3, long ntk, long grow, int c16) {
  return T3 + ((size_t)(grow >> 7) * ntk * 3) * XTILE_E + vfrag_offset((int)(grow & 127), c16);
}

template <int NP>
__device__ __forceinline__ void t3_load(const u16* __restrict__ p0, const u16* __restrict__ p1, int kt, u32x4 (&reg)[6]) {
#pragma unroll
  for (int s = 0; s < NP; ++s) {
    reg[s * 2 + 0] = *reinterpret_cast<const u32x4*>(p0 + ((size_t)kt * 3 + s) * XTILE_E);
    reg[s * 2 + 1] = *reinterpret_cast<const u32x4*>(p1 + ((size_t)kt * 3 + s) * XTILE_E);
  }
}

template <int NP>
__device__ __forceinline__ void x3_store_swz(unsigned char* oper, int t, const u32x4 (&reg)[6]) {
#pragma unroll
  for (int s = 0; s < NP; ++s)
#pragma unroll
    for (int q = 0; q < 2; ++q) {
      const int chunk = t + 256 * q;
      *reinterpret_cast<u32x4*>(oper + s * XPLANE + (chunk >> 2) * XROW + xswz(chunk >> 2, chunk & 3)) = reg[s * 2 + q];
    }
}

template <int NP>
__device__ __forceinline__ f32x16 x3_products(const u32x4 (&a)[3], const u32x4 (&b)[3], f32x16 c) {
  if (NP == 2) {
    c = __builtin_amdgcn_mfma_f32_32x32x16_f16(X3_HF(a[1]), X3_HF(b[0]), c, 0, 0, 0);
    c = __builtin_amdgcn_mfma_f32_32x32x16_f16(X3_HF(a[0]), X3_HF(b[1]), c, 0, 0, 0);
    return __builtin_amdgcn_mfma_f32_32x32x16_f16(X3_HF(a[0]), X3_HF(b[0]), c, 0, 0, 0);
  }
  return __builtin_amdgcn_mfma_f32_32x32x16_bf16(X3_BF(a[0]), X3_BF(b[0]), c, 0, 0, 0);
}


template <int NP>
__device__ __forceinline__ void x3_mma_tile(const unsigned char* As, const unsigned char* Bs, int wy, int wx, int lane,
                                            f32x16 (&acc)[2][2]) {
  const int l31 = lane & 31, h = lane >> 5;
#pragma unroll
  for (int ks = 0; ks < 2; ++ks) {
    u32x4 a[2][3], b[2][3];
    const int co = xswz(l31, 2 * ks + h);
#pragma unroll
    for (int i = 0; i < 2; ++i)
#pragma unroll
      for (int s = 0; s < NP; ++s) {
        a[i][s] = *reinterpret_cast<const u32x4*>(As + s * XPLANE + (wy * 64 + i * 32 + l31) * XROW + co);
        b[i][s] = *reinterpret_cast<const u32x4*>(Bs + s * XPLANE + (wx * 64 + i * 32 + l31) * XROW + co);
      }
#pragma unroll
    for (int i = 0; i < 2; ++i)
#pragma unroll
      for (int j = 0; j < 2; ++j) acc[i][j] = x3_products<NP>(a[i], b[j], acc[i][j]);
  }
}

template <bool SYM, int NP>
__global__ __launch_bounds__(NTHREADS, 3) void k_distance_x3(const u16* __restrict__ T3, int ntk,
                                                             const float* __restrict__ r, float* __restrict__ D, int n,
                                                             int row0, int n_local, long ldD, int tiles_m, int tiles_n,
                                                             u64* __restrict__ hist0, const float* __restrict__ two_s,
                                                             SpecState* __restrict__ spec, u64* __restrict__ spec_buf) {
  constexpr int OP = NP * XPLANE;
  __shared__ __attribute__((aligned(16))) unsigned char smem[2 * OP > EPI_LDS_BYTES ? 2 * OP : EPI_LDS_BYTES];
  unsigned char* As = smem;
  unsigned char* Bs = smem + OP;
  int tile_m, tile_n;
  if (!distance_tile<SYM>(xcd_remap(blockIdx.x, gridDim.x), tiles_m, tiles_n, tile_m, tile_n)) return;
  const int t = threadIdx.x, lane = t & 63, wid = t >> 6;
  const int wy = wid >> 1, wx = wid & 1;
  const long arow0 = row0 + (long)tile_m * BM, brow0 = (long)tile_n * BN;
  const EpiPrefetch pf = distance_epilogue_prefetch(r, n, row0, n_local, tile_m, tile_n, spec);
  const float two_s_v = *two_s;

  f32x16 acc[2][2];
#pragma unroll
  for (int i = 0; i < 2; ++i)
#pragma unroll
    for (int j = 0; j < 2; ++j)
#pragma unroll
      for (int e = 0; e < 16; ++e) acc[i][j][e] = 0.f;

  const u16* __restrict__ pa0 = t3_chunk_ptr(T3, ntk, arow0 + (t >> 2), t & 3);
  const u16* __restrict__ pa1 = t3_chunk_ptr(T3, ntk, arow0 + (t >> 2) + 64, t & 3);
  const u16* __restrict__ pb0 = t3_chunk_ptr(T3, ntk, brow0 + (t >> 2), t & 3);
  const u16* __restrict__ pb1 = t3_chunk_ptr(T3, ntk, brow0 + (t >> 2) + 64, t & 3);
  u32x4 ra[6], rb[6];
  t3_load<NP>(pa0, pa1, 0, ra);
  t3_load<NP>(pb0, pb1, 0, rb);
  for (int kt = 0; kt < ntk; ++kt) {
    x3_store_swz<NP>(As, t, ra);
    x3_store_swz<NP>(Bs, t, rb);
    __syncthreads();
    if (kt + 1 < ntk) {
      t3_load<NP>(pa0, pa1, kt + 1, ra);
      t3_load<NP>(pb0, pb1, kt + 1, rb);
    }
    x3_mma_tile<NP>(As, Bs, wy, wx, lane, acc);
    __syncthreads();
  }
  distance_epilogue<SYM, false>(acc, reinterpret_cast<u32*>(smem), D, n, n_local, ldD, tile_m, tile_n, hist0, pf,
                                two_s_v, spec, spec_buf);
}

constexpr int FS_THREADS = 768;

constexpr int FS_KT = 4;
constexpr int FS_ROWS = 128;
constexpr int FS_IB = FS_ROWS / 16;
constexpr int CJ = 2;
constexpr int PR = FS_ROWS / 32;
constexpr int PLN = FS_ROWS * XROW;

template <int NP, bool FOLD = false>
__global__ __launch_bounds__(FS_THREADS) void k_phi_x3fs(const float* __restrict__ D, long ldD,
                                                         const u16* __restrict__ Gt3, const u16* __restrict__ Tt3,
                                                         long ntj, const float* __restrict__ h2p,
                                                         float* __restrict__ OG, float* __restrict__ OT,
                                                         float* __restrict__ RS, int n, int d, int n_local,
                                                         int tiles_m, int cblocks, int split, int jchunk,
                                                         const float* __restrict__ sc, int dc, int upper) {
  const int wpm = FOLD ? (cblocks + 1) >> 1 : cblocks;
  constexpr int FS_KTB = NP * PLN;
  constexpr int FS_STAGE = FS_KT * FS_KTB;
  __shared__ __attribute__((aligned(16))) unsigned char smem[2 * FS_STAGE];

  const int logical = xcd_remap(blockIdx.x, gridDim.x);
  int cb, tile_m;
  const int plane = wpm * tiles_m;
  const int half = FOLD && logical >= plane * split ? 1 : 0;
  const int lw = FOLD ? logical - half * plane * split : logical;
  const int l2 = lw % plane;
  const int z = lw / plane;
  if (wpm > 4 && (wpm & 3) == 0 && (tiles_m & 7) == 0) {
    const int sb = l2 >> 5, in = l2 & 31, cgroups = wpm >> 2;
    cb = (sb % cgroups) * 4 + (in & 3);
    tile_m = (sb / cgroups) * 8 + (in >> 2);
  } else {
    cb = l2 % wpm;
    tile_m = l2 / wpm;
  }
  const int i0 = tile_m * FS_ROWS;
  const int jbeg = z * jchunk;
  const int jend = half ? n : min(n, jbeg + jchunk);
  const int ntile = jend > jbeg ? (jend - jbeg + BK - 1) / BK : 0;
  const int nstage = (ntile + FS_KT - 1) / FS_KT;
  const int rot = (cb % FS_KT) * (wpm >= FS_KT ? 1 : FS_KT / wpm) % FS_KT;
  const int group = wpm <= 32 ? 32 / wpm : 1;
  const bool permute = upper != 0 && (FOLD || (jbeg == 0 && jend == n && nstage == tiles_m)) && (wpm & (wpm - 1)) == 0 &&
                       wpm <= 4 && nstage * FS_KT == ntile && (nstage & (nstage - 1)) == 0 && nstage >= 2 * group;
  const int xmask = permute ? (tile_m & ~(group - 1) & (nstage - 1)) : 0;
  auto stage_of = [&](int v) { return v ^ xmask; };
  auto tile_at = [&](int stage, int u) {
    const int st2 = stage_of(stage + u / FS_KT), u2 = u % FS_KT;
    return st2 * FS_KT + ((st2 + 1) * FS_KT <= ntile ? ((u2 + rot) & (FS_KT - 1)) : u2);
  };

  const bool up = upper != 0;
  const int ntr = up ? max(0, min(nstage, (i0 - jbeg) / (FS_KT * BK))) : 0;

  const int t = threadIdx.x;
  if (t < 256) {
    const int pt = t;
    const int lr = pt >> 3, lc = (pt & 7) * 4;
    float rs[PR];
#pragma unroll
    for (int p = 0; p < PR; ++p) rs[p] = 0.f;
    constexpr int PD = FOLD ? 2 : FS_KT;
    f32x4g rd[PD][PR];
    u32 doff[PR];
    const float cexp = -1.44269504088896341f / (2.f * *h2p);
    constexpr float pofs = (float)SplitTraits<NP>::pexp;
#pragma unroll
    for (int p = 0; p < PR; ++p) doff[p] = (u32)(((i0 & (DT_ROWS - 1)) + lr + 32 * p) * DT_COLS + lc);
    const float* __restrict__ drow = D + (size_t)(i0 / DT_ROWS) * (ldD >> 5) * DT_ELEMS;
    const int jq = (pt >> 3) & 7, ig = (pt >> 6) * 8 + (pt & 7);
    u32 doff_tr[PR];
#pragma unroll
    for (int u = 0; u < PR; ++u) doff_tr[u] = (u32)((ig >> 3) * DT_ELEMS + (4 * jq + u) * DT_COLS + 4 * (ig & 7)) * 4u;
    const long ntc_d = ldD >> 5;
    float rst[4] = {0.f, 0.f, 0.f, 0.f};
    auto request = [&](int j0, bool tr, f32x4g (&rd)[PR]) {
      const float* tile = tr ? D + ((size_t)(j0 >> 7) * ntc_d + 4 * (size_t)(i0 / DT_ROWS)) * DT_ELEMS + (j0 & 127) * DT_COLS
                             : drow + (size_t)(j0 >> 5) * DT_ELEMS;
#pragma unroll
      for (int p = 0; p < PR; ++p) stream_load16(rd[p], tile, tr ? doff_tr[p] : doff[p] * 4u);
    };
    auto wait_loads = [&](int v, f32x4g (&rd)[PR]) {
      const int later = ntile - v - 1;
      (void)rd;
      if constexpr (PD == 4) {
        stream_wait<3 * PR>();
        if (later < 3) {
          stream_wait<2 * PR>();
          if (later < 2) {
            stream_wait<PR>();
            if (later < 1) stream_wait<0>();
          }
        }
      } else {
        static_assert(PD == 2 || PD == 4, "wait_loads is written out for these two leads");
        stream_wait<PR>();
        if (later < 1) stream_wait<0>();
      }
    };
    auto produce = [&](int j0, unsigned char* buf, const f32x4g (&rd)[PR]) {
      const bool full = j0 + BK <= jend;
      float q[PR][4];
#pragma unroll
      for (int p = 0; p < PR; ++p)
#pragma unroll
        for (int e = 0; e < 4; ++e) q[p][e] = __builtin_fmaf(cexp, rd[p][e], pofs);
      __builtin_amdgcn_sched_barrier(0);
#pragma unroll
      for (int p = 0; p < PR; ++p)
#pragma unroll
        for (int e = 0; e < 4; ++e) q[p][e] = __builtin_amdgcn_exp2f(q[p][e]);
      __builtin_amdgcn_sched_barrier(0);
      if (!full) {
        const int j = j0 + lc;
#pragma unroll
        for (int p = 0; p < PR; ++p)
#pragma unroll
          for (int e = 0; e < 4; ++e) q[p][e] = (j + e < jend) ? q[p][e] : 0.f;
      }
      if (NP >= 2) {
        u32 hi[PR][2], lo[PR][2];
        float r[PR][4];
#pragma unroll
        for (int p = 0; p < PR; ++p) rs[p] += (q[p][0] + q[p][1]) + (q[p][2] + q[p][3]);
#pragma unroll
        for (int p = 0; p < PR; ++p) { hi[p][0] = cvt_pk_f16(q[p][0], q[p][1]); hi[p][1] = cvt_pk_f16(q[p][2], q[p][3]); }
        __builtin_amdgcn_sched_barrier(0);
#pragma unroll
        for (int p = 0; p < PR; ++p) {
          r[p][0] = f16_resid_lo(hi[p][0], q[p][0]); r[p][1] = f16_resid_hi(hi[p][0], q[p][1]);
          r[p][2] = f16_resid_lo(hi[p][1], q[p][2]); r[p][3] = f16_resid_hi(hi[p][1], q[p][3]);
        }
        __builtin_amdgcn_sched_barrier(0);
#pragma unroll
        for (int p = 0; p < PR; ++p) { lo[p][0] = cvt_pk_f16(r[p][0], r[p][1]); lo[p][1] = cvt_pk_f16(r[p][2], r[p][3]); }
        __builtin_amdgcn_sched_barrier(0);
#pragma unroll
        for (int p = 0; p < PR; ++p) {
          unsigned char* dst = buf + (lr + 32 * p) * XROW + pswz(lr, lc >> 3) + (lc & 4) * 2;
          *reinterpret_cast<uint2*>(dst) = make_uint2(hi[p][0], hi[p][1]);
          *reinterpret_cast<uint2*>(dst + PLN) = make_uint2(lo[p][0], lo[p][1]);
        }
      } else {
#pragma unroll
        for (int p = 0; p < PR; ++p) {
          unsigned char* dst = buf + (lr + 32 * p) * XROW + pswz(lr, lc >> 3) + (lc & 4) * 2;
          const u32 h0 = cvt_pk_bf16(q[p][0], q[p][1]), h1 = cvt_pk_bf16(q[p][2], q[p][3]);
          rs[p] += (__uint_as_float(h0 << 16) + __uint_as_float(h0 & 0xffff0000u)) +
                   (__uint_as_float(h1 << 16) + __uint_as_float(h1 & 0xffff0000u));
          *reinterpret_cast<uint2*>(dst) = make_uint2(h0, h1);
        }
      }
    };
    auto produce_tr = [&](unsigned char* buf, const f32x4g (&rd)[PR]) {
      float q[4][4];
#pragma unroll
      for (int u = 0; u < 4; ++u)
#pragma unroll
        for (int e = 0; e < 4; ++e) q[u][e] = __builtin_fmaf(cexp, rd[u][e], pofs);
      __builtin_amdgcn_sched_barrier(0);
#pragma unroll
      for (int u = 0; u < 4; ++u)
#pragma unroll
        for (int e = 0; e < 4; ++e) q[u][e] = __builtin_amdgcn_exp2f(q[u][e]);
      __builtin_amdgcn_sched_barrier(0);
      u32 hi[4][2], lo[4][2];
      if (NP >= 2) {
        float r[4][4];
#pragma unroll
        for (int e = 0; e < 4; ++e) rst[e] += (q[0][e] + q[1][e]) + (q[2][e] + q[3][e]);
#pragma unroll
        for (int e = 0; e < 4; ++e) { hi[e][0] = cvt_pk_f16(q[0][e], q[1][e]); hi[e][1] = cvt_pk_f16(q[2][e], q[3][e]); }
        __builtin_amdgcn_sched_barrier(0);
#pragma unroll
        for (int e = 0; e < 4; ++e) {
          r[e][0] = f16_resid_lo(hi[e][0], q[0][e]); r[e][1] = f16_resid_hi(hi[e][0], q[1][e]);
          r[e][2] = f16_resid_lo(hi[e][1], q[2][e]); r[e][3] = f16_resid_hi(hi[e][1], q[3][e]);
        }
        __builtin_amdgcn_sched_barrier(0);
#pragma unroll
        for (int e = 0; e < 4; ++e) { lo[e][0] = cvt_pk_f16(r[e][0], r[e][1]); lo[e][1] = cvt_pk_f16(r[e][2], r[e][3]); }
        __builtin_amdgcn_sched_barrier(0);
      } else {
#pragma unroll
        for (int e = 0; e < 4; ++e) {
          hi[e][0] = cvt_pk_bf16(q[0][e], q[1][e]); hi[e][1] = cvt_pk_bf16(q[2][e], q[3][e]);
          lo[e][0] = lo[e][1] = 0u;
          rst[e] += (__uint_as_float(hi[e][0] << 16) + __uint_as_float(hi[e][0] & 0xffff0000u)) +
                    (__uint_as_float(hi[e][1] << 16) + __uint_as_float(hi[e][1] & 0xffff0000u));
        }
      }
#pragma unroll
      for (int e = 0; e < 4; ++e) {
        const int row = 4 * ig + e;
        unsigned char* dst = buf + row * XROW + pswz(row, jq >> 1) + (jq & 1) * 8;
        *reinterpret_cast<uint2*>(dst) = make_uint2(hi[e][0], hi[e][1]);
        if (NP >= 2) *reinterpret_cast<uint2*>(dst + PLN) = make_uint2(lo[e][0], lo[e][1]);
      }
    };
    auto jt = [&](int tile) { return jbeg + tile * BK; };
#pragma unroll
    for (int u = 0; u < PD; ++u)
      if (tile_at(0, u) < ntile) request(jt(tile_at(0, u)), stage_of(0) < ntr, rd[u]);
    auto produce_stage = [&](int st, unsigned char* buf) {
      const bool tr_now = stage_of(st) < ntr;
#pragma unroll
      for (int u = 0; u < FS_KT; ++u) {
        const int tile_u = tile_at(st, u), next_u = tile_at(st, u + PD);
        const bool tr_next = stage_of(st + (u + PD) / FS_KT) < ntr;
        if (tile_u < ntile) {
          wait_loads(st * FS_KT + u, rd[u % PD]);
          if (tr_now) produce_tr(buf + u * FS_KTB, rd[u % PD]);
          else produce(jt(tile_u), buf + u * FS_KTB, rd[u % PD]);
        }
        if (next_u < ntile) request(jt(next_u), tr_next, rd[u % PD]);
      }
    };
    produce_stage(0, smem);
    __syncthreads();
    for (int st = 0; st < nstage; ++st) {
      if (st + 1 < nstage) produce_stage(st + 1, smem + ((st + 1) & 1) * FS_STAGE);
      __syncthreads();
    }
    if (up) {
      float* red = reinterpret_cast<float*>(smem);
#pragma unroll
      for (int p = 0; p < 4; ++p) {
        float a = rs[p], b = rst[p];
        a += __shfl_xor(a, 1); b += __shfl_xor(b, 8);
        a += __shfl_xor(a, 2); b += __shfl_xor(b, 16);
        a += __shfl_xor(a, 4); b += __shfl_xor(b, 32);
        if ((pt & 7) == 0) red[lr + 32 * p] = a;
        if (jq == 0) red[128 + 4 * ig + p] = b;
      }
      __syncthreads();
      const int row = i0 + pt;
      if (cb == 0 && !half && pt < 128 && row < n_local) RS[(size_t)z * n_local + row] = (red[pt] + red[128 + pt]) * sc[4 * dc + 2];
    } else if (cb == 0 && !half) {
#pragma unroll
      for (int p = 0; p < PR; ++p) {
        float sum = rs[p];
        sum += __shfl_xor(sum, 1);
        sum += __shfl_xor(sum, 2);
        sum += __shfl_xor(sum, 4);
        const int row = i0 + lr + 32 * p;
        if ((pt & 7) == 0 && row < n_local) RS[(size_t)z * n_local + row] = sum * sc[4 * dc + 2];
      }
    }
  } else {
    const int ct = t - 256, lane = ct & 63, cw = ct >> 6;
    const int l15 = lane & 15, lq = lane >> 4;
    const int g = 2 * cb + (cw >> 2);
    const int gl = FOLD ? min(g, cblocks - 1) : g;
    const int wcol = (cw & 3) * 32;
    const u16* vb_wave = (FOLD ? (half ? Tt3 : Gt3) + (size_t)gl * ntj * 3 * XTILE_E
                               : (g < cblocks ? Gt3 + (size_t)g * ntj * 3 * XTILE_E
                                              : Tt3 + (size_t)(g - cblocks) * ntj * 3 * XTILE_E)) +
                         (size_t)(jbeg >> 5) * 3 * XTILE_E + wcol * 32;
    const u16* __restrict__ vb = reinterpret_cast<const u16*>(
        ((unsigned long long)(u32)__builtin_amdgcn_readfirstlane((int)((unsigned long long)vb_wave >> 32)) << 32) |
        (unsigned long long)(u32)__builtin_amdgcn_readfirstlane((int)(unsigned long long)vb_wave));
    u32 boff[CJ][3];
#pragma unroll
    for (int j = 0; j < CJ; ++j)
#pragma unroll
      for (int s = 0; s < 3; ++s) boff[j][s] = (u32)(lane * 8 + s * XTILE_E + j * 512) * 2u;
    const int aoff = l15 * XROW + pswz(l15, lq);
    f32x4 acc[FS_IB][CJ];
#pragma unroll
    for (int i = 0; i < FS_IB; ++i)
#pragma unroll
      for (int j = 0; j < CJ; ++j) acc[i][j] = f32x4{0.f, 0.f, 0.f, 0.f};
    u32x4 bX[CJ][3], bY[CJ][3];
    auto load_b = [&](int tile, u32x4 (&b)[CJ][3]) {
      const u16* __restrict__ src = vb + (size_t)tile * 3 * XTILE_E;
#pragma unroll
      for (int j = 0; j < CJ; ++j)
#pragma unroll
        for (int s = 0; s < NP; ++s) stream_load16(b[j][s], src, boff[j][s]);
    };
    auto wait_b = [&](bool younger, u32x4 (&b)[CJ][3]) {
      (void)b;
      stream_wait<CJ * NP>();
      if (!younger) stream_wait<0>();
    };
    auto read_a = [&](const unsigned char* As, int i, u32x4 (&a)[3]) {
#pragma unroll
      for (int s = 0; s < NP; ++s) a[s] = *reinterpret_cast<const u32x4*>(As + aoff + i * 16 * XROW + s * PLN);
    };
    auto mma_tile = [&](const unsigned char* As, const u32x4 (&b)[CJ][3]) {
      u32x4 a[2][3];
      read_a(As, 0, a[0]);
#pragma unroll
      for (int i = 0; i < FS_IB; ++i) {
        if (i + 1 < FS_IB) read_a(As, i + 1, a[(i + 1) & 1]);
        __builtin_amdgcn_sched_barrier(0);
#pragma unroll
        for (int j = 0; j < CJ; ++j) acc[i][j] = x3_products16<NP>(a[i & 1], b[j], acc[i][j]);
        __builtin_amdgcn_sched_barrier(0);
      }
    };
    if (ntile > 0) load_b(tile_at(0, 0), bX);
    __syncthreads();
    for (int st = 0; st < nstage; ++st) {
      const unsigned char* As = smem + (st & 1) * FS_STAGE;
      auto after = [&](int u) { return tile_at(st, u); };
      constexpr bool kLoadV = true;
#pragma unroll
      for (int u = 0; u < FS_KT; u += 2) {
        if (after(u) >= ntile) break;
        const bool n1 = after(u + 1) < ntile;
        if (kLoadV && n1) load_b(after(u + 1), bY);
        wait_b(kLoadV && n1, bX);
        if (cw >> 2) __builtin_amdgcn_s_setprio(0); else __builtin_amdgcn_s_setprio(2);
        mma_tile(As + u * FS_KTB, bX);
        if (n1) {
          const bool n2 = after(u + 2) < ntile;
          if (kLoadV && n2) load_b(after(u + 2), bX);
          wait_b(kLoadV && n2, bY);
          if (cw >> 2) __builtin_amdgcn_s_setprio(2); else __builtin_amdgcn_s_setprio(0);
          mma_tile(As + (u + 1) * FS_KTB, bY);
        }
      }
      __syncthreads();
    }
    if (up) __syncthreads();
    if (FOLD ? g >= cblocks : g >= 2 * cblocks) return;
    const bool first = FOLD ? half == 0 : g < cblocks;
    float* __restrict__ Oz = (first ? OG : OT) + (size_t)z * n_local * d;
    const int cbase = (FOLD || first ? g : g - cblocks) * BN + wcol + l15;
    const float* __restrict__ osc = sc + (first ? 2 : 3) * dc;
#pragma unroll
    for (int j = 0; j < CJ; ++j) {
      const int col = cbase + j * 16;
      if (col >= d) continue;
      const float os = osc[col];
#pragma unroll
      for (int i = 0; i < FS_IB; ++i)
#pragma unroll
        for (int e = 0; e < 4; ++e) {
          const int row = i0 + i * 16 + 4 * lq + e;
          if (row < n_local) Oz[(size_t)row * d + col] = acc[i][j][e] * os;
        }
    }
  }
}

static int split_kind(int dtype) { return dtype == STEIN_BF16 ? 1 : 2; }
int stein_x3_kind(int dtype) { return split_kind(dtype); }

template <typename TIN, int KIND>
static void launch_split(hipStream_t stream, const TIN* theta, const TIN* score, int64_t n, int64_t d,
                         const SteinLayout& L, u16* T3, u16* Tt3, u16* Gt3, const float* sc, const PrologueArgs* pro = nullptr) {
  const unsigned nz = (theta ? 1u : 0u) + (score ? 1u : 0u);
  const int zbase = theta ? 0 : 1;
  const int vec = std::is_same<TIN, float>::value && d % 4 == 0 && (((uintptr_t)theta | (uintptr_t)score) & 15u) == 0;
  const int64_t rows = L.x3_rows > L.x3_nk ? L.x3_rows : L.x3_nk;
  const int64_t cols = L.x3_dk > L.x3_dc ? L.x3_dk : L.x3_dc;
  if (KIND == 1 && pro && theta) {
    const dim3 grid((unsigned)((cols + 63) / 64), (unsigned)((rows + 63) / 64), nz + 1u);
    hipLaunchKernelGGL((k_split<TIN, KIND, true>), grid, dim3(256), 0, stream, theta, score, (int)n, (int)d, T3,
                       (long)L.x3_rows, (int)L.x3_dk, Tt3, Gt3, (int)L.x3_dc, (long)L.x3_nk, sc, zbase, *pro, vec);
    return;
  }
  const dim3 grid((unsigned)((cols + 63) / 64), (unsigned)((rows + 63) / 64), nz);
  hipLaunchKernelGGL((k_split<TIN, KIND, false>), grid, dim3(256), 0, stream, theta, score, (int)n, (int)d, T3,
                     (long)L.x3_rows, (int)L.x3_dk, Tt3, Gt3, (int)L.x3_dc, (long)L.x3_nk, sc, zbase, PrologueArgs{}, vec);
}

int stein_x3_split(const StepViews& v, const void* theta_all, const void* score_all, int dtype, int64_t n, int64_t d,
                   hipStream_t stream, const SplitFused* fused) {
  const SteinLayout& L = v.L;
  const int dc = (int)L.x3_dc;
  const int kind = split_kind(dtype);
  HistSync* fuse_done = fused && theta_all && score_all ? fused->done : nullptr;
  const PrologueArgs* prologue = fused ? fused->prologue : nullptr;
  const int fold = fused ? fused->fold : 0;
  if (kind == 2) {
    const int zbase = score_all ? 0 : 1;
    const unsigned nz = (score_all ? 1u : 0u) + (theta_all ? 1u : 0u);
    if (!fuse_done) HIP_TRY(hipMemsetAsync(v.cmax + (size_t)zbase * dc, 0, (size_t)nz * dc * sizeof(u32), stream));
    int gy = (int)((n + 63) / 64);
    if (gy > 256) gy = 256;
    const bool v4 = d % 4 == 0 && (!score_all || ((uintptr_t)score_all & 15) == 0) && (!theta_all || ((uintptr_t)theta_all & 15) == 0);
    if (v4) {
      const int gy4 = gy > 64 ? 64 : gy;
      const dim3 grid((unsigned)((d + 255) / 256), (unsigned)gy4, nz);
      hipLaunchKernelGGL((k_colmax<float, true>), grid, dim3(1024), 0, stream, (const float*)score_all, (const float*)theta_all,
                         (int)n, (int)d, v.cmax, dc, zbase, v.sc, PEXP_H2, fuse_done);
    } else {
      const dim3 grid((unsigned)((d + 63) / 64), (unsigned)gy, nz);
      hipLaunchKernelGGL((k_colmax<float, false>), grid, dim3(256), 0, stream, (const float*)score_all, (const float*)theta_all,
                         (int)n, (int)d, v.cmax, dc, zbase, v.sc, PEXP_H2, fuse_done);
    }
    LAUNCH_CHECK("k_colmax");
  }
  if (kind == 2 ? !fuse_done : !prologue) {
    hipLaunchKernelGGL(k_make_scales, dim3(1), dim3(256), 0, stream, v.cmax, dc, v.sc, kind == 2 ? PEXP_H2 : 0,
                       kind == 2 ? 1 : 0);
    LAUNCH_CHECK("k_make_scales");
  }
  if (kind == 1) launch_split<u16, 1>(stream, (const u16*)theta_all, (const u16*)score_all, n, d, L, v.T3, v.Tt3, v.Gt3, v.sc, prologue);
  else if (fold)
    launch_split<float, 2>(stream, (const float*)theta_all, (const float*)nullptr, n, d, L, v.T3, fold == 2 ? v.Tt3 : nullptr, v.Gt3, v.sc);
  else launch_split<float, 2>(stream, (const float*)theta_all, (const float*)score_all, n, d, L, v.T3, v.Tt3, v.Gt3, v.sc);
  LAUNCH_CHECK("k_split");
  return STEIN_OK;
}

constexpr double FOLD_MIN_WORK = 4.0e9;
bool stein_fold_pays(int64_t n, int64_t d) { return d > 128 && (double)n * (double)n * (double)d >= FOLD_MIN_WORK; }

int stein_x3_split_w(const StepViews& v, const float* theta_all, const float* score_all, int64_t n, int64_t d,
                     const float* h2_dev, hipStream_t stream) {
  const SteinLayout& L = v.L;
  const dim3 grid((unsigned)((L.x3_dc + 63) / 64), (unsigned)((L.x3_nk + 63) / 64));
  const int vec = d % 4 == 0 && (((uintptr_t)theta_all | (uintptr_t)score_all) & 15u) == 0;
  hipLaunchKernelGGL(k_split_w, grid, dim3(256), 0, stream, theta_all, score_all, (int)n, (int)d, v.Gt3, (int)L.x3_dc,
                     (long)L.x3_nk, v.sc, (const u32*)v.cmax, h2_dev, vec);
  LAUNCH_CHECK("k_split_w");
  return STEIN_OK;
}

template <bool SYM, int NP>
static void launch_distance_x3(long nblk, hipStream_t stream, const u16* T3, int ntk, const float* r, float* D, int n,
                               int row0, int n_local, long ld, int tiles_m, int tiles_n, u64* hist0, const float* two_s,
                               SpecState* spec, u64* spec_buf) {
  hipLaunchKernelGGL((k_distance_x3<SYM, NP>), dim3((unsigned)nblk), dim3(NTHREADS), 0, stream, T3, ntk, r, D, n, row0,
                     n_local, ld, tiles_m, tiles_n, hist0, two_s, spec, spec_buf);
}

int stein_x3_distance(const StepViews& v, const BlockShape& b, bool symmetric, bool window, hipStream_t stream, int panel) {
  if (panel >= 0 && stein_dpanel_ok(v, b, panel > 0)) return stein_dpanel_distance(v, b, symmetric, window, stream);
  const SteinLayout& L = v.L;
  const int ntk = (int)(L.x3_dk / 32);
  const int tiles_m = (int)((b.n_local + BM - 1) / BM), tiles_n = (int)((b.n + BN - 1) / BN);
  if (b.row0 + (int64_t)tiles_m * BM > L.x3_rows) return stein_fail(STEIN_E_SHAPE, "row block exceeds the padded planes");
  const long nblk = distance_grid(symmetric, tiles_m, tiles_n);
  if (nblk > 0x7fffffffl) return stein_fail(STEIN_E_SHAPE, "too many tiles");
  SpecState* spec = window ? v.spec : nullptr;
  u64* spec_buf = window ? v.spec_buf : nullptr;
#define X3_DIST(SYM, NP) launch_distance_x3<SYM, NP>(nblk, stream, v.T3, ntk, v.r, v.D, (int)b.n, (int)b.row0, (int)b.n_local, (long)L.ld_dist, tiles_m, tiles_n, v.hist, v.two_s, spec, spec_buf)
  switch (split_kind(b.dtype)) {
    case 1: if (symmetric) X3_DIST(true, 1); else X3_DIST(false, 1); break;
    default: if (symmetric) X3_DIST(true, 2); else X3_DIST(false, 2); break;
  }
#undef X3_DIST
  LAUNCH_CHECK("k_distance_x3");
  return STEIN_OK;
}

int stein_x3_contract_partial(const StepViews& v, const BlockShape& b, const float* h2_dev, hipStream_t stream, bool upper) {
  const SteinLayout& L = v.L;
  const long nblk = (long)L.tiles_m * L.cblocks * v.nsplit;
  if (nblk > 0x7fffffffl) return stein_fail(STEIN_E_SHAPE, "too many tiles");
#define X3_PHI(NP) hipLaunchKernelGGL((k_phi_x3fs<NP>), dim3((unsigned)nblk), dim3(FS_THREADS), 0, stream, v.D, (long)L.ld_dist, v.Gt3, v.Tt3, (long)(L.x3_nk / 32), h2_dev, v.OG, v.OT, v.RS, (int)b.n, (int)b.d, (int)b.n_local, (int)L.tiles_m, (int)L.cblocks, v.nsplit, v.jchunk, v.sc, (int)L.x3_dc, upper ? 1 : 0)
  switch (split_kind(b.dtype)) {
    case 1: X3_PHI(1); break;
    default: X3_PHI(2); break;
  }
#undef X3_PHI
  LAUNCH_CHECK("k_phi_x3fs");
  return STEIN_OK;
}

int stein_x3_contract_fold(const StepViews& v, const float* h2_dev, int64_t n, int64_t d, bool with_theta,
                           hipStream_t stream) {
  const SteinLayout& L = v.L;
  const long per_range = (long)L.tiles_m * ((L.cblocks + 1) / 2);
  const long nblk = per_range * (v.nsplit + (with_theta ? 1 : 0));
  if (nblk > 0x7fffffffl) return stein_fail(STEIN_E_SHAPE, "too many tiles");
  hipLaunchKernelGGL((k_phi_x3fs<2, true>), dim3((unsigned)nblk), dim3(FS_THREADS), 0, stream, v.D, (long)L.ld_dist, v.Gt3,
                     with_theta ? v.Tt3 : (const u16*)nullptr, (long)(L.x3_nk / 32), h2_dev, v.OG, v.OT, v.RS, (int)n, (int)d,
                     (int)n, (int)L.tiles_m, (int)L.cblocks, v.nsplit, v.jchunk, v.sc, (int)L.x3_dc, 1);
  LAUNCH_CHECK("k_phi_x3fs");
  return STEIN_OK;
}
```

stein_amd/csrc/steinhip.hip:

```cpp

#include <hip/hip_runtime.h>
#include <stdint.h>
#include <stdio.h>
#include <stdlib.h>
#include <stdarg.h>
#include <string.h>
#include <math.h>

#include "stein_host.h"
#include "stein_x3.h"

#include <type_traits>
#include <vector>

static thread_local char g_err[512] = "";

int stein_fail(int code, const char* fmt, ...) {
  va_list ap;
  va_start(ap, fmt);
  vsnprintf(g_err, sizeof(g_err), fmt, ap);
  va_end(ap);
  return code;
}

extern "C" int stein_version(void) { return STEIN_VERSION; }
extern "C" const char* stein_last_error(void) { return g_err; }

template <typename TIN>
__global__ __launch_bounds__(256) void k_rownorms(const TIN* __restrict__ T, int n, int d, float* __restrict__ r) {
  const int wave = (blockIdx.x * 256 + threadIdx.x) >> 6;
  const int lane = threadIdx.x & 63;
  if (wave >= n) return;
  const float s = wave_row_sqnorm(T + (size_t)wave * d, d, lane);
  if (lane == 0) r[wave] = s;
}

template <typename TIN>
__global__ __launch_bounds__(256) void k_prologue(const TIN* __restrict__ T, PrologueArgs a) {
  prologue_body<TIN>(T, a, (int)blockIdx.x, (int)gridDim.x);
}

__global__ __launch_bounds__(256) void k_kernel_matrix(const float* __restrict__ D, long ldD, int n_local, int n,
                                                       const float* __restrict__ h2p, float* __restrict__ K, long ldK,
                                                       int upper) {
  const float h2 = *h2p;
  const long total = (long)n_local * n;
  for (long e = (long)blockIdx.x * 256 + threadIdx.x; e < total; e += (long)gridDim.x * 256) {
    const long row = e / n, col = e - row * n;
    const bool swap = upper && (col >> 7) < (row >> 7);
    K[row * ldK + col] = expf(-D[d_index(swap ? col : row, swap ? row : col, ldD >> 5)] / h2 / 2.f);
  }
}

__device__ __forceinline__ float4 theta4(const float* p) { return *reinterpret_cast<const float4*>(p); }
__device__ __forceinline__ float4 theta4(const unsigned short* p) {
  const uint2 w = *reinterpret_cast<const uint2*>(p);
  return make_float4(__uint_as_float(w.x << 16), __uint_as_float(w.x & 0xffff0000u), __uint_as_float(w.y << 16),
                     __uint_as_float(w.y & 0xffff0000u));
}
template <typename TIN, bool KSD, bool FOLD = false>
__global__ __launch_bounds__(256) void k_phi_finish(const float* __restrict__ OG, const float* __restrict__ OT,
                                                    const float* __restrict__ RS, const TIN* __restrict__ T,
                                                    const float* __restrict__ h2p, float* __restrict__ phi,
                                                    float* __restrict__ dK, double* __restrict__ sqpart, int n, int d,
                                                    int row0, int n_local, int split, int tsplit, int vec, HistSync* done,
                                                    double* __restrict__ sq_out, const TIN* __restrict__ G) {
  constexpr int NS = KSD ? 3 : 1;
  __shared__ double red[4 * NS];
  const float h2 = *h2p;
  const float fn = (float)n;
  const long total = (long)n_local * d;
  const size_t zs = (size_t)n_local * d;
  double sq = 0.0;
  double ks = 0.0, kd = 0.0;
  const double ih = 1.0 / (double)h2;
  const bool need_t = !FOLD || KSD || dK != nullptr;
  auto kg = [&](float o, float t) { return FOLD ? (double)o + (double)t * ih : (double)o; };
  if (vec) {
    const long total4 = total >> 2;
    const int d4 = d >> 2;
    auto run = [&](auto nz, auto nt) {
      constexpr int NZ = decltype(nz)::value, NT = decltype(nt)::value;
      for (long q = (long)blockIdx.x * 256 + threadIdx.x; q < total4; q += (long)gridDim.x * 256) {
        const int i = (int)(q / d4);
        const long e = q << 2;
        float4 og = make_float4(0.f, 0.f, 0.f, 0.f), ot = og;
        float rs = 0.f;
        float4 th;
        if constexpr (NZ > 0) {
          float4 a[NZ], b[NT > 0 ? NT : 1];
          float r[NZ];
#pragma unroll
          for (int z = 0; z < NZ; ++z) {
            a[z] = *reinterpret_cast<const float4*>(OG + z * zs + e);
            r[z] = RS[(size_t)z * n_local + i];
          }
          th = theta4(T + (size_t)row0 * d + e);
#pragma unroll
          for (int z = 0; z < NT; ++z) b[z] = *reinterpret_cast<const float4*>(OT + z * zs + e);
#pragma unroll
          for (int z = 0; z < NZ; ++z) {
            og.x += a[z].x; og.y += a[z].y; og.z += a[z].z; og.w += a[z].w;
            if (z < NT) { ot.x += b[z].x; ot.y += b[z].y; ot.z += b[z].z; ot.w += b[z].w; }
            rs += r[z];
          }
        } else {
#pragma unroll 8
          for (int z = 0; z < split; ++z) {
            const float4 a = *reinterpret_cast<const float4*>(OG + z * zs + e);
            og.x += a.x; og.y += a.y; og.z += a.z; og.w += a.w;
            if (FOLD ? need_t && z < tsplit : true) {
              const float4 b = *reinterpret_cast<const float4*>(OT + z * zs + e);
              ot.x += b.x; ot.y += b.y; ot.z += b.z; ot.w += b.w;
            }
            rs += RS[(size_t)z * n_local + i];
          }
          th = theta4(T + (size_t)row0 * d + e);
        }
        auto rt_minus = [&](float t, float o) {
          if constexpr (FOLD) {
#pragma clang fp contract(off)
            const float m = rs * t;
            return m - o;
          } else {
            return __builtin_fmaf(rs, t, -o);
          }
        };
        float4 dk, ph;
        dk.x = rt_minus(th.x, ot.x) / h2; dk.y = rt_minus(th.y, ot.y) / h2; dk.z = rt_minus(th.z, ot.z) / h2; dk.w = rt_minus(th.w, ot.w) / h2;
        if constexpr (FOLD) {
          ph.x = (og.x + rs * th.x / h2) / fn; ph.y = (og.y + rs * th.y / h2) / fn;
          ph.z = (og.z + rs * th.z / h2) / fn; ph.w = (og.w + rs * th.w / h2) / fn;
        } else {
          ph.x = (og.x + dk.x) / fn; ph.y = (og.y + dk.y) / fn; ph.z = (og.z + dk.z) / fn; ph.w = (og.w + dk.w) / fn;
        }
        *reinterpret_cast<float4*>(phi + e) = ph;
        if (dK) *reinterpret_cast<float4*>(dK + e) = dk;
        sq += ((double)ph.x * (double)ph.x + (double)ph.y * (double)ph.y) + ((double)ph.z * (double)ph.z + (double)ph.w * (double)ph.w);
        if constexpr (KSD) {
          const float4 g = theta4(G + (size_t)row0 * d + e);
          ksd_terms(g.x, kg(og.x, ot.x), ot.x, th.x, rs, ih, ks, kd);
          ksd_terms(g.y, kg(og.y, ot.y), ot.y, th.y, rs, ih, ks, kd);
          ksd_terms(g.z, kg(og.z, ot.z), ot.z, th.z, rs, ih, ks, kd);
          ksd_terms(g.w, kg(og.w, ot.w), ot.w, th.w, rs, ih, ks, kd);
        }
      }
    };
    using std::integral_constant;
    auto run_nz = [&](auto nz) {
      if constexpr (!FOLD) run(nz, nz);
      else if (need_t) run(nz, integral_constant<int, 1>());
      else run(nz, integral_constant<int, 0>());
    };
    if (split == 1) run_nz(integral_constant<int, 1>());
    else if (split == 2) run_nz(integral_constant<int, 2>());
    else if (split == 4) run_nz(integral_constant<int, 4>());
    else run(integral_constant<int, 0>(), integral_constant<int, 0>());
  } else {
    for (long e = (long)blockIdx.x * 256 + threadIdx.x; e < total; e += (long)gridDim.x * 256) {
      const int i = (int)(e / d);
      float og = 0.f, ot = 0.f, rs = 0.f;
      for (int z = 0; z < split; ++z) {
        og += OG[z * zs + e];
        if (FOLD ? need_t && z < tsplit : true) ot += OT[z * zs + e];
        rs += RS[(size_t)z * n_local + i];
      }
      const float th = elem_f32(T + (size_t)row0 * d + e);
      const float dk = (rs * th - ot) / h2;
      const float ph = FOLD ? (og + rs * th / h2) / fn : (og + dk) / fn;
      phi[e] = ph;
      if (dK) dK[e] = dk;
      sq += (double)ph * (double)ph;
      if constexpr (KSD) ksd_terms(elem_f32(G + (size_t)row0 * d + e), kg(og, ot), ot, th, rs, ih, ks, kd);
    }
  }
  double part[NS];
  part[0] = sq;
  if constexpr (KSD) { part[1] = ks; part[2] = kd; }
  block_sum256(part, red);
  if (!done) {
    if (threadIdx.x == 0)
      for (int k = 0; k < NS; ++k) sqpart[k * gridDim.x + blockIdx.x] = part[k];
    return;
  }
  if (threadIdx.x == 0)
    for (int k = 0; k < NS; ++k)
      __hip_atomic_store(reinterpret_cast<u64*>(sqpart) + k * gridDim.x + blockIdx.x, (u64)__double_as_longlong(part[k]),
                         __ATOMIC_RELAXED, __HIP_MEMORY_SCOPE_AGENT);
  {
    __shared__ u32 s_last;
    asm volatile("s_waitcnt vmcnt(0)" ::: "memory");
    __syncthreads();
    if (threadIdx.x == 0) s_last = tree_report_done(done->fin_leaf, &done->fin_top, blockIdx.x, gridDim.x) ? 1u : 0u;
    __syncthreads();
    if (!s_last) return;
  }
  double tot[NS];
  for (int k = 0; k < NS; ++k) {
    tot[k] = 0.0;
    for (int i = threadIdx.x; i < (int)gridDim.x; i += 256)
      tot[k] += __longlong_as_double((long long)load_fresh(reinterpret_cast<const u64*>(sqpart) + k * gridDim.x + i));
  }
  __syncthreads();
  block_sum256(tot, red);
  if (threadIdx.x == 0)
    for (int k = 0; k < NS; ++k) sq_out[k] = tot[k];
}

__global__ __launch_bounds__(256) void k_sum_partial_sets(const double* __restrict__ part, int count, double* out) {
  __shared__ double red[4];
  const double* p = part + (size_t)blockIdx.x * count;
  double s[1] = {0.0};
  for (int i = threadIdx.x; i < count; i += 256) s[0] += p[i];
  block_sum256(s, red);
  if (threadIdx.x == 0) out[blockIdx.x] = s[0];
}

static int sum_partials(const double* part, int count, bool ksd, double* out, hipStream_t s) {
  hipLaunchKernelGGL(k_sum_partial_sets, dim3(ksd ? 3 : 1), dim3(256), 0, s, part, count, out);
  LAUNCH_CHECK("k_sum_partial_sets");
  return STEIN_OK;
}

static thread_local int g_fold_split = 0;
extern "C" int stein_debug_fold_split(int ranges) {
  if (ranges < 0 || ranges > 65535) return fail(STEIN_E_BADARG, "ranges %d", ranges);
  g_fold_split = ranges;
  return STEIN_OK;
}

int stein_make_layout(int64_t n_local, int64_t n, int64_t d, int dtype, int flags, SteinLayout* L) {
  if (n < 2) return fail(STEIN_E_BADARG, "n = %lld: the bandwidth divides by ln(n), need n >= 2", (long long)n);
  if (d < 1 || n_local < 1 || n_local > n) return fail(STEIN_E_SHAPE, "bad shape n_local=%lld n=%lld d=%lld", (long long)n_local, (long long)n, (long long)d);
  if (int rc = stein_check_size(n, d)) return rc;
  if (dtype != STEIN_F32 && dtype != STEIN_BF16) return fail(STEIN_E_UNSUPPORTED, "dtype %d", dtype);
  if (flags & ~(STEIN_FLAG_X3 | STEIN_FLAG_TIMING | STEIN_FLAG_TILED | STEIN_FLAG_NO_WINDOW | STEIN_FLAG_RANK_WINDOW | STEIN_FLAG_TILE_DISTANCE | STEIN_FLAG_TIMING_CONTRACT | STEIN_FLAG_KSD | STEIN_FLAG_FOLD | STEIN_FLAG_NO_FOLD)) return fail(STEIN_E_BADARG, "unknown flags 0x%x", flags);
  if ((flags & STEIN_FLAG_FOLD) && (flags & STEIN_FLAG_NO_FOLD)) return fail(STEIN_E_BADARG, "STEIN_FLAG_FOLD and STEIN_FLAG_NO_FOLD exclude each other");
  L->ld_dist = (int64_t)align_up((size_t)n, 64);
  L->tiles_m = (n_local + BM - 1) / BM;
  L->cblocks = (d + BN - 1) / BN;
  const bool x3 = (flags & STEIN_FLAG_X3) != 0;
  const int64_t base = x3 ? L->tiles_m * L->cblocks : L->tiles_m * 2 * L->cblocks;
  const int64_t jt = (n + BK - 1) / BK;
  const double resident = x3 ? RESIDENT_ONE_PER_CU : 768.0;
  int64_t max_split = jt / 8 > 0 ? jt / 8 : 1;
  if (max_split > 16) max_split = 16;
  auto choose_split = [&](int64_t base_wgs, int64_t* jchunk_out, int64_t forced = 0) {
    int64_t split = 1;
    double best = -1.0;
    if (forced > 0) split = forced < jt ? forced : jt;
    for (int64_t s = 1; forced <= 0 && s <= max_split; ++s) {
      const double rounds = (double)(base_wgs * s) / resident;
      const double eff = rounds / ceil(rounds) - 0.004 * (double)(s - 1);
      if (eff > best + 1e-9) { best = eff; split = s; }
    }
    int64_t tiles_per = (jt + split - 1) / split;
    if (x3) tiles_per = (tiles_per + 3) / 4 * 4;
    *jchunk_out = tiles_per * BK;
    return (jt + tiles_per - 1) / tiles_per;
  };
  const int64_t split = choose_split(base, &L->jchunk);
  L->split = split;
  const int64_t elems = n_local * d;
  int64_t sqb = (elems + 1023) / 1024;
  if (sqb > 1024) sqb = 1024;
  L->sq_blocks = sqb;

  size_t at = 0;
  auto put = [&](int sec, size_t bytes) { L->off[sec] = at; at = align_up(at + bytes, 256); };
  put(STEIN_WS_ROWNORM, (size_t)n * 4);
  put(STEIN_WS_DIST, align_up((size_t)n_local, DT_ROWS) * L->ld_dist * 4);
  put(STEIN_WS_HIST, (size_t)STEIN_HIST_LEVELS * 2 * STEIN_HIST_BINS * 8);
  put(STEIN_WS_SELECT, sizeof(SelState) + sizeof(SpecState) + sizeof(FuseState));
  put(STEIN_WS_PART_G, (size_t)split * n_local * d * 4);
  put(STEIN_WS_PART_T, (size_t)split * n_local * d * 4);
  put(STEIN_WS_PART_RS, (size_t)split * n_local * 4);
  {
    const int64_t small = (d + 31) / 32;
    put(STEIN_WS_SQPART, (size_t)(sqb > small ? sqb : small) * 8 * ((flags & STEIN_FLAG_KSD) ? 3 : 1));
  }
  const bool small_path = !(flags & STEIN_FLAG_TILED) && n_local == n && stein_small_ok(n, d, dtype);
  put(STEIN_WS_SPEC, small_path ? 0 : ((size_t)SPEC_CAP + SPEC_SLOTS * 8 + SPEC_TABLE) * 8);
  L->x3_rows = (int64_t)align_up((size_t)n, 128) + 128;
  L->x3_dk = (int64_t)align_up((size_t)d, 32);
  L->x3_dc = (int64_t)align_up((size_t)d, 128);
  L->x3_nk = (int64_t)align_up((size_t)n, 32);
  const size_t t3 = align_up((size_t)3 * L->x3_rows * L->x3_dk * 2, 256);
  const size_t tt3 = align_up((size_t)3 * L->x3_dc * L->x3_nk * 2, 256);
  L->x3_t3 = 0;
  L->x3_tt3 = t3;
  L->x3_gt3 = t3 + tt3;
  L->x3_sc = t3 + 2 * tt3;
  const size_t scb = align_up((size_t)(6 * L->x3_dc + 4) * 4, 256);
  const bool fold_forced = (flags & STEIN_FLAG_FOLD) != 0;
  L->fold = x3 && dtype == STEIN_F32 && n_local == n && !small_path && !(flags & STEIN_FLAG_NO_FOLD) &&
            (fold_forced || stein_fold_pays(n, d));
  L->fsplit = L->fjchunk = 0;
  size_t fold_extra = 0;
  if (L->fold) {
    L->fsplit = choose_split(L->tiles_m * ((L->cblocks + 1) / 2), &L->fjchunk, g_fold_split);
    const size_t ow = align_up((size_t)L->fsplit * n_local * d * 4, 256), ot = align_up((size_t)n_local * d * 4, 256),
                 rs = align_up((size_t)L->fsplit * n_local * 4, 256);
    if (ow <= L->off[STEIN_WS_PART_RS] - L->off[STEIN_WS_PART_G] && ot + rs <= t3) {
      L->fold_ow = L->off[STEIN_WS_PART_G];
      L->fold_ot = at + L->x3_t3;
      L->fold_rs = L->fold_ot + ot;
    } else if (fold_forced) {
      L->fold_ow = at + t3 + 2 * tt3 + scb;
      L->fold_ot = L->fold_ow + ow;
      L->fold_rs = L->fold_ot + ot;
      fold_extra = ow + ot + rs;
    } else {
      L->fold = 0;
      L->fsplit = L->fjchunk = 0;
    }
  }
  put(STEIN_WS_PLANES, (flags & STEIN_FLAG_X3) ? t3 + 2 * tt3 + scb + fold_extra : 0);
  L->total = at;
  return STEIN_OK;
}

StepViews stein_step_views(const SteinLayout& L, void* workspace, void* planes_override) {
  char* ws = (char*)workspace;
  StepViews v{};
  v.L = L;
  v.nsplit = (int)L.split; v.jchunk = (int)L.jchunk; v.tsplit = (int)L.split;
  if (ws) {
    v.r = (float*)(ws + L.off[STEIN_WS_ROWNORM]);
    v.D = (float*)(ws + L.off[STEIN_WS_DIST]);
    v.hist = (u64*)(ws + L.off[STEIN_WS_HIST]);
    v.sel = (SelState*)(ws + L.off[STEIN_WS_SELECT]);
    v.spec = spec_of(v.sel);
    v.fuse = fuse_of(v.sel);
    v.spec_buf = (u64*)(ws + L.off[STEIN_WS_SPEC]);
    v.table = spec_table_of(v.spec_buf);
    v.OG = (float*)(ws + L.off[STEIN_WS_PART_G]);
    v.OT = (float*)(ws + L.off[STEIN_WS_PART_T]);
    v.RS = (float*)(ws + L.off[STEIN_WS_PART_RS]);
    v.SQ = (double*)(ws + L.off[STEIN_WS_SQPART]);
  }
  if (planes_override) v.planes = (char*)planes_override;
  else if (ws && L.total > L.off[STEIN_WS_PLANES]) v.planes = ws + L.off[STEIN_WS_PLANES];
  if (v.planes) {
    v.T3 = (unsigned short*)(v.planes + L.x3_t3);
    v.Tt3 = (unsigned short*)(v.planes + L.x3_tt3);
    v.Gt3 = (unsigned short*)(v.planes + L.x3_gt3);
    v.sc = (float*)(v.planes + L.x3_sc);
    v.cmax = (u32*)(v.sc + x3_sc_cmax(L.x3_dc));
    v.two_s = v.sc + x3_sc_two_s(L.x3_dc);
  }
  if (L.fold && ws && !planes_override) {
    v.OG = (float*)(ws + L.fold_ow);
    v.OT = (float*)(ws + L.fold_ot);
    v.RS = (float*)(ws + L.fold_rs);
    v.nsplit = (int)L.fsplit; v.jchunk = (int)L.fjchunk; v.tsplit = 1;
  }
  return v;
}

extern "C" int stein_workspace_bytes(int64_t n_local, int64_t n, int64_t d, int dtype, int flags, size_t* out) {
  if (!out) return fail(STEIN_E_BADARG, "out is NULL");
  SteinLayout L;
  int rc = stein_make_layout(n_local, n, d, dtype, flags, &L);
  if (rc) return rc;
  *out = L.total;
  return STEIN_OK;
}

extern "C" int stein_workspace_layout(int64_t n_local, int64_t n, int64_t d, int dtype, int flags, size_t* offsets,
                                      int64_t* extra) {
  if (!offsets || !extra) return fail(STEIN_E_BADARG, "NULL output");
  SteinLayout L;
  int rc = stein_make_layout(n_local, n, d, dtype, flags, &L);
  if (rc) return rc;
  for (int i = 0; i < STEIN_WS_NSECTIONS; ++i) offsets[i] = L.off[i];
  extra[STEIN_WSX_LD_DIST] = L.ld_dist;
  extra[STEIN_WSX_SPLIT] = L.split;
  extra[STEIN_WSX_SQ_BLOCKS] = L.sq_blocks;
  extra[STEIN_WSX_HIST_BINS] = STEIN_HIST_BINS;
  return STEIN_OK;
}

extern "C" int stein_layout_fold_ranges(int64_t n_local, int64_t n, int64_t d, int dtype, int flags, int* out) {
  if (!out) return fail(STEIN_E_BADARG, "out is NULL");
  SteinLayout L;
  int rc = stein_make_layout(n_local, n, d, dtype, flags, &L);
  if (rc) return rc;
  *out = L.fold ? (int)L.fsplit : 0;
  return STEIN_OK;
}

extern "C" int stein_layout_folds(int64_t n_local, int64_t n, int64_t d, int dtype, int flags, int* out) {
  if (!out) return fail(STEIN_E_BADARG, "out is NULL");
  SteinLayout L;
  int rc = stein_make_layout(n_local, n, d, dtype, flags, &L);
  if (rc) return rc;
  *out = (int)L.fold;
  return STEIN_OK;
}

extern "C" int stein_x3_prepare(const void* theta_all, const void* score_all, int64_t n, int64_t d, int dtype,
                                void* x3_planes, size_t planes_bytes, void* stream) {
  if ((!theta_all && !score_all) || !x3_planes) return fail(STEIN_E_BADARG, "NULL pointer");
  SteinLayout L;
  int rc = stein_make_layout(n, n, d, dtype, stein_staged_flags(true), &L);
  if (rc) return rc;
  if (planes_bytes < L.total - L.off[STEIN_WS_PLANES])
    return fail(STEIN_E_WORKSPACE, "planes buffer %zu < %zu bytes", planes_bytes, L.total - L.off[STEIN_WS_PLANES]);
  return stein_x3_split(stein_step_views(L, nullptr, x3_planes), theta_all, score_all, dtype, n, d, (hipStream_t)stream, nullptr);
}

extern "C" int stein_rownorms(const void* theta_all, int64_t n, int64_t d, int dtype, float* r_out, void* stream) {
  if (!theta_all || !r_out) return fail(STEIN_E_BADARG, "NULL pointer");
  if (n < 1 || d < 1) return fail(STEIN_E_SHAPE, "bad shape");
  if (dtype != STEIN_F32 && dtype != STEIN_BF16) return fail(STEIN_E_UNSUPPORTED, "rownorms: dtype %d", dtype);
  const int blocks = (int)((n + 3) / 4);
  if (dtype == STEIN_BF16)
    hipLaunchKernelGGL(k_rownorms<unsigned short>, dim3(blocks), dim3(256), 0, (hipStream_t)stream,
                       (const unsigned short*)theta_all, (int)n, (int)d, r_out);
  else
    hipLaunchKernelGGL(k_rownorms<float>, dim3(blocks), dim3(256), 0, (hipStream_t)stream, (const float*)theta_all,
                       (int)n, (int)d, r_out);
  LAUNCH_CHECK("k_rownorms");
  return STEIN_OK;
}

static int check_block(const char* stage, const BlockShape& b, bool bf16_ok) {
  if (b.dtype != STEIN_F32 && b.dtype != STEIN_BF16) return fail(STEIN_E_UNSUPPORTED, "%s: dtype %d", stage, b.dtype);
  if (b.dtype == STEIN_BF16 && !bf16_ok)
    return fail(STEIN_E_UNSUPPORTED, "%s: bf16 inputs need the operand planes (STEIN_FLAG_X3)", stage);
  if (b.row0 < 0 || b.n_local < 1 || b.row0 + b.n_local > b.n) return fail(STEIN_E_SHAPE, "bad row block");
  return STEIN_OK;
}

static int distance_stage(const StepViews& v, const BlockShape& b, const void* theta_all, int stage_flags, bool window,
                          hipStream_t s) {
  const bool sym = (stage_flags & STEIN_STAGE_SYMMETRIC) != 0;
  if (v.planes)
    return stein_x3_distance(v, b, sym, window, s, (stage_flags & STEIN_STAGE_TILES) ? -1 : ((stage_flags & STEIN_STAGE_PANEL) ? 1 : 0));
  return stein_fp32_distance(v, b, (const float*)theta_all, sym, window, s);
}

static int contract_stage(const StepViews& v, const BlockShape& b, const void* theta_all, const void* score_all,
                          const float* h2_dev, bool upper, hipStream_t s) {
  return v.planes ? stein_x3_contract_partial(v, b, h2_dev, s, upper)
                  : stein_fp32_contract_partial(v, b, (const float*)theta_all, (const float*)score_all, h2_dev, s);
}

static int finish_stage(const StepViews& v, const BlockShape& b, const void* theta_all, const void* score_all,
                        const float* h2_dev, float* phi_local, double* sqnorm_out, float* dK_out, bool ksd, HistSync* done,
                        hipStream_t s) {
  const SteinLayout& L = v.L;
  auto al16 = [](const void* p) { return ((uintptr_t)p & 15u) == 0; };
  const size_t tsz = b.dtype == STEIN_BF16 ? 2 : 4;
  auto rows_aligned = [&](const void* p) { return (((uintptr_t)p + (size_t)b.row0 * b.d * tsz) & (4 * tsz - 1)) == 0; };
  const int vec = (b.d % 4 == 0) && al16(v.OG) && al16(v.OT) && al16(phi_local) && al16(dK_out) && rows_aligned(theta_all) &&
                  (!ksd || rows_aligned(score_all));
  auto launch = [&](auto tin, auto ksd_tag, auto fold_tag) {
    using TIN = decltype(tin);
    hipLaunchKernelGGL((k_phi_finish<TIN, decltype(ksd_tag)::value, decltype(fold_tag)::value>), dim3((unsigned)L.sq_blocks),
                       dim3(256), 0, s, v.OG, v.OT, v.RS, (const TIN*)theta_all, h2_dev, phi_local, dK_out, v.SQ, (int)b.n, (int)b.d,
                       (int)b.row0, (int)b.n_local, v.nsplit, v.tsplit, vec, done, sqnorm_out, (const TIN*)score_all);
  };
  auto launch_ksd = [&](auto tin, auto fold_tag) {
    if (ksd) launch(tin, std::true_type(), fold_tag);
    else launch(tin, std::false_type(), fold_tag);
  };
  if (L.fold) launch_ksd(0.f, std::true_type());
  else if (b.dtype == STEIN_BF16) launch_ksd((unsigned short)0, std::false_type());
  else launch_ksd(0.f, std::false_type());
  LAUNCH_CHECK("k_phi_finish");
  return done ? STEIN_OK : sum_partials(v.SQ, (int)L.sq_blocks, ksd, sqnorm_out, s);
}

static int distance_block(const void* theta_all, const float* r_all, const BlockShape& b, float* dist_out, int64_t ld_dist,
                          void* hist_level0, const void* x3_planes, int flags, void* stream, SpecState* spec, u64* spec_buf) {
  if ((!theta_all && !x3_planes) || !r_all || !dist_out) return fail(STEIN_E_BADARG, "NULL pointer");
  if (b.n < 1 || b.d < 1) return fail(STEIN_E_SHAPE, "bad row block");
  int rc = check_block("distance", b, x3_planes != nullptr);
  if (rc) return rc;
  if (ld_dist < b.n || (ld_dist & 63)) return fail(STEIN_E_SHAPE, "ld_dist must be >= n and a multiple of 64");
  if ((flags & STEIN_STAGE_SYMMETRIC) && (b.row0 != 0 || b.n_local != b.n))
    return fail(STEIN_E_BADARG, "STEIN_STAGE_SYMMETRIC needs the whole matrix (row0 = 0, n_local = n) and ld_dist %% 64 == 0");
  StepViews v{};
  if (x3_planes) {
    SteinLayout L;
    if ((rc = stein_make_layout(b.n_local, b.n, b.d, b.dtype, stein_staged_flags(true), &L))) return rc;
    v = stein_step_views(L, nullptr, const_cast<void*>(x3_planes));
  }
  v.r = const_cast<float*>(r_all); v.D = dist_out; v.L.ld_dist = ld_dist; v.hist = (u64*)hist_level0;
  v.spec = spec; v.spec_buf = spec_buf;
  return distance_stage(v, b, theta_all, flags, spec != nullptr, (hipStream_t)stream);
}

extern "C" int stein_distance_block(const void* theta_all, const float* r_all, int64_t n, int64_t d, int64_t row0,
                                    int64_t n_local, int dtype, float* dist_out, int64_t ld_dist, void* hist_level0,
                                    const void* x3_planes, int flags, void* stream) {
  return distance_block(theta_all, r_all, BlockShape{n, d, row0, n_local, dtype}, dist_out, ld_dist, hist_level0, x3_planes,
                        flags, stream, nullptr, nullptr);
}

extern "C" int stein_distance_block_spec(const void* theta_all, const float* r_all, int64_t n, int64_t d, int64_t row0,
                                         int64_t n_local, int dtype, float* dist_out, int64_t ld_dist, void* hist_level0,
                                         const void* x3_planes, int flags, void* select_state, void* spec_buf,
                                         void* stream) {
  if (!hist_level0 || !select_state || !spec_buf) return fail(STEIN_E_BADARG, "NULL pointer");
  return distance_block(theta_all, r_all, BlockShape{n, d, row0, n_local, dtype}, dist_out, ld_dist, hist_level0, x3_planes,
                        flags, stream, spec_of(select_state), (u64*)spec_buf);
}

extern "C" int stein_kernel_matrix(const float* dist, int64_t ld_dist, int64_t n_local, int64_t n,
                                   const float* h2_dev, float* K_out, int64_t ld_K, int dist_flags, void* stream) {
  if (!dist || !h2_dev || !K_out) return fail(STEIN_E_BADARG, "NULL pointer");
  if (ld_dist < n || ld_K < n || n_local < 1) return fail(STEIN_E_SHAPE, "bad shape");
  if (dist_flags & ~(STEIN_STAGE_SYMMETRIC | STEIN_STAGE_UPPER)) return fail(STEIN_E_BADARG, "unknown distance flags 0x%x", dist_flags);
  if ((dist_flags & STEIN_STAGE_UPPER) && n_local != n) return fail(STEIN_E_BADARG, "STEIN_STAGE_UPPER needs the whole matrix");
  hipLaunchKernelGGL(k_kernel_matrix, dim3(grid_for((long)n_local * n, 4096)), dim3(256), 0, (hipStream_t)stream,
                     dist, (long)ld_dist, (int)n_local, (int)n, h2_dev, K_out, (long)ld_K,
                     (dist_flags & STEIN_STAGE_UPPER) ? 1 : 0);
  LAUNCH_CHECK("k_kernel_matrix");
  return STEIN_OK;
}

static int contract_partial_views(const float* dist, int64_t ld_dist, const void* theta_all, const void* score_all,
                                  const BlockShape& b, const float* h2_dev, const void* x3_planes, void* workspace,
                                  size_t ws_bytes, int dist_flags, StepViews* v) {
  if (dist_flags & ~(STEIN_STAGE_SYMMETRIC | STEIN_STAGE_UPPER)) return fail(STEIN_E_BADARG, "unknown distance flags 0x%x", dist_flags);
  if ((dist_flags & STEIN_STAGE_UPPER) && (!x3_planes || b.row0 != 0 || b.n_local != b.n))
    return fail(STEIN_E_BADARG, "STEIN_STAGE_UPPER: only the split path's symmetric distance pass stores the upper triangle alone");
  if (!dist || (!x3_planes && (!theta_all || !score_all)) || !h2_dev || !workspace)
    return fail(STEIN_E_BADARG, "NULL pointer");
  int rc = check_block("contract", b, x3_planes != nullptr);
  if (rc) return rc;
  SteinLayout L;
  if ((rc = stein_make_layout(b.n_local, b.n, b.d, b.dtype, stein_staged_flags(x3_planes != nullptr), &L))) return rc;
  if (ws_bytes < L.off[STEIN_WS_PLANES]) return fail(STEIN_E_WORKSPACE, "workspace %zu < %zu bytes", ws_bytes, L.off[STEIN_WS_PLANES]);
  if (ld_dist != L.ld_dist) return fail(STEIN_E_SHAPE, "ld_dist %lld != %lld", (long long)ld_dist, (long long)L.ld_dist);
  *v = stein_step_views(L, workspace, const_cast<void*>(x3_planes));
  v->D = const_cast<float*>(dist);
  return STEIN_OK;
}

extern "C" int stein_contract_partial(const float* dist, int64_t ld_dist, const void* theta_all,
                                      const void* score_all, int64_t n, int64_t d, int64_t row0, int64_t n_local,
                                      int dtype, const float* h2_dev, const void* x3_planes, void* workspace,
                                      size_t ws_bytes, int dist_flags, void* stream) {
  const BlockShape b{n, d, row0, n_local, dtype};
  StepViews v;
  int rc = contract_partial_views(dist, ld_dist, theta_all, score_all, b, h2_dev, x3_planes, workspace, ws_bytes, dist_flags, &v);
  if (rc) return rc;
  return contract_stage(v, b, theta_all, score_all, h2_dev, (dist_flags & STEIN_STAGE_UPPER) != 0, (hipStream_t)stream);
}

static int check_finish(const void* theta_all, const BlockShape& b, const float* h2_dev, float* phi_local, double* sqnorm_out,
                        void* workspace) {
  if (!theta_all || !h2_dev || !phi_local || !sqnorm_out || !workspace) return fail(STEIN_E_BADARG, "NULL pointer");
  return check_block("contract", b, true);
}

extern "C" int stein_contract_finish(const void* theta_all, int64_t n, int64_t d, int64_t row0, int64_t n_local,
                                     int dtype, const float* h2_dev, float* phi_local, double* sqnorm_out,
                                     float* dK_out, void* workspace, size_t ws_bytes, int flags, void* stream) {
  if (flags & STEIN_FLAG_KSD)
    return fail(STEIN_E_BADARG, "STEIN_FLAG_KSD: stein_contract_finish has no score operand; the statistic comes from "
                                "stein_svgd_phi, stein_rank_finish or stein_rank_step");
  const BlockShape b{n, d, row0, n_local, dtype};
  int rc = check_finish(theta_all, b, h2_dev, phi_local, sqnorm_out, workspace);
  if (rc) return rc;
  SteinLayout L;
  if ((rc = stein_make_layout(n_local, n, d, dtype, (flags & ~STEIN_FLAG_FOLD) | STEIN_FLAG_NO_FOLD, &L))) return rc;
  if (ws_bytes < L.off[STEIN_WS_PLANES]) return fail(STEIN_E_WORKSPACE, "workspace %zu < %zu bytes", ws_bytes, L.off[STEIN_WS_PLANES]);
  return finish_stage(stein_step_views(L, workspace), b, theta_all, nullptr, h2_dev, phi_local, sqnorm_out, dK_out, false,
                      nullptr, (hipStream_t)stream);
}

extern "C" int stein_kernel_contract(const float* dist, int64_t ld_dist, const void* theta_all, const void* score_all,
                                     int64_t n, int64_t d, int64_t row0, int64_t n_local, int dtype,
                                     const float* h2_dev, float* phi_local, double* sqnorm_out, float* dK_out,
                                     const void* x3_planes, void* workspace, size_t ws_bytes, int dist_flags,
                                     void* stream) {
  if (dist_flags & STEIN_FLAG_KSD)
    return fail(STEIN_E_BADARG, "STEIN_FLAG_KSD: stein_kernel_contract takes distance flags only; the statistic comes from "
                                "stein_svgd_phi, stein_rank_finish or stein_rank_step");
  const BlockShape b{n, d, row0, n_local, dtype};
  StepViews v;
  int rc = contract_partial_views(dist, ld_dist, theta_all, score_all, b, h2_dev, x3_planes, workspace, ws_bytes, dist_flags, &v);
  if (rc) return rc;
  if ((rc = check_finish(theta_all, b, h2_dev, phi_local, sqnorm_out, workspace))) return rc;
  const hipStream_t s = (hipStream_t)stream;
  if ((rc = contract_stage(v, b, theta_all, score_all, h2_dev, (dist_flags & STEIN_STAGE_UPPER) != 0, s))) return rc;
  return finish_stage(v, b, theta_all, nullptr, h2_dev, phi_local, sqnorm_out, dK_out, false, nullptr, s);
}

static thread_local std::vector<hipEvent_t> g_tevents;
static thread_local int g_tcalls_reserved = 0, g_tcalls_used = 0;
static thread_local std::vector<unsigned char> g_tmode;

struct StageTimer {
  hipEvent_t* ev = nullptr;
  bool contract_only = false;
  explicit StageTimer(int flags) {
    if (!(flags & STEIN_FLAG_TIMING) || g_tcalls_used >= g_tcalls_reserved) return;
    contract_only = (flags & STEIN_FLAG_TIMING_CONTRACT) != 0;
    g_tmode[(size_t)g_tcalls_used] = contract_only ? 1 : 0;
    ev = &g_tevents[(size_t)(g_tcalls_used++) * (STEIN_T_NSTAGES + 1)];
  }
  int mark(int k, hipStream_t s) const {
    if (ev && (!contract_only || k == STEIN_T_CONTRACT || k == STEIN_T_FINISH)) HIP_TRY(hipEventRecord(ev[k], s));
    return STEIN_OK;
  }
};

int stein_rank_views(const BlockShape& b, void* workspace, size_t ws_bytes, int flags, StepViews* v) {
  if (!workspace) return fail(STEIN_E_BADARG, "NULL pointer");
  int rc = check_block("rank step", b, (flags & STEIN_FLAG_X3) != 0);
  if (rc) return rc;
  if (flags & ~(STEIN_FLAG_X3 | STEIN_FLAG_TILED | STEIN_FLAG_RANK_WINDOW | STEIN_FLAG_TIMING | STEIN_FLAG_KSD)) return fail(STEIN_E_BADARG, "unknown flags 0x%x", flags);
  SteinLayout L;
  if ((rc = stein_make_layout(b.n_local, b.n, b.d, b.dtype, stein_rank_flags(flags), &L))) return rc;
  if (ws_bytes < L.total) return fail(STEIN_E_WORKSPACE, "workspace %zu < %zu bytes", ws_bytes, L.total);
  *v = stein_step_views(L, workspace);
  return STEIN_OK;
}

int stein_rank_begin_on(const StepViews& v, const BlockShape& b, const void* theta_all, bool window, hipStream_t s) {
  int rc;
  if ((rc = stein_rownorms(theta_all, b.n, b.d, b.dtype, v.r, s))) return rc;
  if (v.planes && (rc = stein_x3_split(v, theta_all, nullptr, b.dtype, b.n, b.d, s, nullptr))) return rc;
  if (window) rc = stein_spec_begin(v.hist, v.sel, v.spec_buf, b.n * b.n, s);
  else rc = stein_median_begin(v.hist, v.sel, b.n * b.n, s);
  if (rc) return rc;
  if ((rc = distance_stage(v, b, theta_all, 0, window, s))) return rc;
  if (window) rc = stein_spec_tally(v.sel, v.spec_buf, s);
  return rc;
}

extern "C" int stein_rank_begin(const void* theta_all, int64_t n, int64_t d, int64_t row0, int64_t n_local, int dtype,
                                void* workspace, size_t ws_bytes, int flags, void* stream) {
  if (!theta_all) return fail(STEIN_E_BADARG, "NULL pointer");
  const BlockShape b{n, d, row0, n_local, dtype};
  StepViews v;
  int rc = stein_rank_views(b, workspace, ws_bytes, flags, &v);
  return rc ? rc : stein_rank_begin_on(v, b, theta_all, (flags & STEIN_FLAG_RANK_WINDOW) != 0, (hipStream_t)stream);
}

int stein_rank_pick_on(const StepViews& v, int64_t n, float* h2_out, float* median_out, void* flags_host, hipStream_t s) {
  int rc = stein_spec_pick(v.sel, v.spec_buf, n, h2_out, median_out, s);
  if (rc) return rc;
  HIP_TRY(hipMemcpyAsync(flags_host, &v.spec->hit, 28, hipMemcpyDeviceToHost, s));
  return STEIN_OK;
}

extern "C" int stein_rank_pick(int64_t n, int64_t d, int64_t row0, int64_t n_local, int dtype, void* workspace,
                               size_t ws_bytes, int flags, float* h2_out, float* median_out, void* flags_host,
                               void* stream) {
  if (!h2_out || !flags_host) return fail(STEIN_E_BADARG, "NULL pointer");
  StepViews v;
  int rc = stein_rank_views(BlockShape{n, d, row0, n_local, dtype}, workspace, ws_bytes, flags, &v);
  return rc ? rc : stein_rank_pick_on(v, n, h2_out, median_out, flags_host, (hipStream_t)stream);
}

int stein_rank_radix_on(const StepViews& v, const BlockShape& b, int level, int need_pass, float* h2_out, float* median_out,
                        hipStream_t s) {
  if (level < 0 || level >= STEIN_HIST_LEVELS) return fail(STEIN_E_BADARG, "level %d", level);
  if (need_pass) return stein_median_hist_pass(v.D, v.L.ld_dist, b.n_local, b.n, level, v.sel, v.hist, 0, s);
  int rc = stein_median_resolve(v.hist, level, b.n, v.sel, h2_out, median_out, s);
  if (rc) return rc;
  if (level + 1 < STEIN_HIST_LEVELS)
    rc = stein_median_hist_pass(v.D, v.L.ld_dist, b.n_local, b.n, level + 1, v.sel, v.hist, 0, s);
  return rc;
}

extern "C" int stein_rank_radix(int level, int need_pass, int64_t n, int64_t d, int64_t row0, int64_t n_local, int dtype,
                                void* workspace, size_t ws_bytes, int flags, float* h2_out, float* median_out,
                                void* stream) {
  const BlockShape b{n, d, row0, n_local, dtype};
  StepViews v;
  int rc = stein_rank_views(b, workspace, ws_bytes, flags, &v);
  return rc ? rc : stein_rank_radix_on(v, b, level, need_pass, h2_out, median_out, (hipStream_t)stream);
}

int stein_rank_finish_on(const StepViews& v, const BlockShape& b, const void* theta_all, const void* score_all,
                         const float* h2_dev, float* phi_local, double* sqnorm_out, float* dK_out, int flags,
                         hipStream_t s) {
  int rc;
  if ((flags & STEIN_FLAG_RANK_WINDOW) && (rc = stein_spec_update(v.sel, s))) return rc;
  const StageTimer clk(flags);
  for (int k = 0; k <= STEIN_T_CONTRACT; ++k)
    if ((rc = clk.mark(k, s))) return rc;
  if ((rc = contract_stage(v, b, theta_all, score_all, h2_dev, false, s))) return rc;
  if ((rc = clk.mark(STEIN_T_FINISH, s))) return rc;
  rc = finish_stage(v, b, theta_all, score_all, h2_dev, phi_local, sqnorm_out, dK_out, (flags & STEIN_FLAG_KSD) != 0, nullptr, s);
  return rc ? rc : clk.mark(STEIN_T_NSTAGES, s);
}

extern "C" int stein_rank_finish(const void* theta_all, const void* score_all, int64_t n, int64_t d, int64_t row0,
                                 int64_t n_local, int dtype, const float* h2_dev, float* phi_local, double* sqnorm_out,
                                 float* dK_out, void* workspace, size_t ws_bytes, int flags, void* stream) {
  if (!theta_all || !score_all || !h2_dev || !phi_local || !sqnorm_out) return fail(STEIN_E_BADARG, "NULL pointer");
  const BlockShape b{n, d, row0, n_local, dtype};
  StepViews v;
  int rc = stein_rank_views(b, workspace, ws_bytes, flags, &v);
  return rc ? rc : stein_rank_finish_on(v, b, theta_all, score_all, h2_dev, phi_local, sqnorm_out, dK_out, flags,
                                        (hipStream_t)stream);
}

static u32* g_errword[MAX_DEVICES];
int stein_device_error_word(u32** out) {
  int dev = 0;
  HIP_TRY(hipGetDevice(&dev));
  if (dev < 0 || dev >= MAX_DEVICES) { *out = nullptr; return STEIN_OK; }
  u32* w = __atomic_load_n(&g_errword[dev], __ATOMIC_ACQUIRE);
  if (!w) {
    void* p = nullptr;
    HIP_TRY(hipHostMalloc(&p, 64, hipHostMallocMapped | hipHostMallocPortable));
    *(volatile u32*)p = 0u;
    u32* expect = nullptr;
    if (!__atomic_compare_exchange_n(&g_errword[dev], &expect, (u32*)p, false, __ATOMIC_ACQ_REL, __ATOMIC_ACQUIRE)) {
      (void)hipHostFree(p);
      w = expect;
    } else {
      w = (u32*)p;
    }
  }
  *out = w;
  return STEIN_OK;
}
int stein_take_device_error(void) {
  int dev = 0;
  if (hipGetDevice(&dev) != hipSuccess || dev < 0 || dev >= MAX_DEVICES) return STEIN_OK;
  u32* w = __atomic_load_n(&g_errword[dev], __ATOMIC_ACQUIRE);
  if (!w || !*(volatile u32*)w) return STEIN_OK;
  *(volatile u32*)w = 0u;
  return fail(STEIN_E_HIP, "an earlier step on device %d gave up inside k_hist_all (bounded wait exhausted): its bandwidth and "
                           "everything computed from it are NaN", dev);
}
extern "C" int stein_debug_raise_device_error(void) {
  u32* w = nullptr;
  int rc = stein_device_error_word(&w);
  if (rc) return rc;
  if (w) *(volatile u32*)w = 1u;
  return STEIN_OK;
}


extern "C" int stein_timing_reserve(int calls) {
  if (calls < 0) return fail(STEIN_E_BADARG, "calls < 0");
  const size_t need = (size_t)calls * (STEIN_T_NSTAGES + 1);
  while (g_tevents.size() < need) {
    hipEvent_t e;
    HIP_TRY(hipEventCreate(&e));
    g_tevents.push_back(e);
  }
  g_tmode.assign((size_t)calls, 0);
  g_tcalls_reserved = calls;
  g_tcalls_used = 0;
  return STEIN_OK;
}

extern "C" int stein_timing_read(float* ms_out, int max_calls, int* calls_out) {
  if (!ms_out || !calls_out) return fail(STEIN_E_BADARG, "NULL pointer");
  const int calls = g_tcalls_used < max_calls ? g_tcalls_used : max_calls;
  for (int c = 0; c < calls; ++c) {
    hipEvent_t* ev = &g_tevents[(size_t)c * (STEIN_T_NSTAGES + 1)];
    if (g_tmode[(size_t)c]) {
      HIP_TRY(hipEventSynchronize(ev[STEIN_T_FINISH]));
      for (int k = 0; k < STEIN_T_NSTAGES; ++k) ms_out[c * STEIN_T_NSTAGES + k] = -1.f;
      HIP_TRY(hipEventElapsedTime(&ms_out[c * STEIN_T_NSTAGES + STEIN_T_CONTRACT], ev[STEIN_T_CONTRACT], ev[STEIN_T_FINISH]));
      continue;
    }
    HIP_TRY(hipEventSynchronize(ev[STEIN_T_NSTAGES]));
    for (int k = 0; k < STEIN_T_NSTAGES; ++k) HIP_TRY(hipEventElapsedTime(&ms_out[c * STEIN_T_NSTAGES + k], ev[k], ev[k + 1]));
  }
  *calls_out = calls;
  return STEIN_OK;
}

static int fused_prologue(const StepViews& v, const BlockShape& b, const void* theta_all, const void* score_all, int flags,
                          hipStream_t s, int fold) {
  const bool bf16_split = b.dtype == STEIN_BF16 && v.planes;
  PrologueArgs pa;
  pa.n = (int)b.n; pa.d = (int)b.d; pa.r = v.r; pa.st = v.sel; pa.sp = v.spec; pa.fs = v.fuse; pa.total = (u64)(b.n * b.n);
  pa.hist = v.hist; pa.slots = v.spec_buf;
  pa.cmax = v.cmax;
  pa.ncmax = v.planes ? (int)(2 * v.L.x3_dc) : 0;
  pa.allow_window = (flags & STEIN_FLAG_NO_WINDOW) ? 0 : 1;
  pa.hsync = (u32*)v.table; pa.hsync_words = (int)(sizeof(HistSync) / 4);
  pa.neutral_sc = bf16_split ? v.sc : (float*)nullptr;
  pa.dc = (int)v.L.x3_dc;
  pa.folded = fold ? 1u : 0u;
  const SplitFused fused{(HistSync*)v.table, bf16_split ? &pa : nullptr, fold};
  if (bf16_split) return stein_x3_split(v, theta_all, score_all, b.dtype, b.n, b.d, s, &fused);
  const dim3 grid((unsigned)((b.n + 3) / 4 + PRO_INIT_BLOCKS));
  if (b.dtype == STEIN_BF16)
    hipLaunchKernelGGL(k_prologue<unsigned short>, grid, dim3(256), 0, s, (const unsigned short*)theta_all, pa);
  else
    hipLaunchKernelGGL(k_prologue<float>, grid, dim3(256), 0, s, (const float*)theta_all, pa);
  LAUNCH_CHECK("k_prologue");
  return v.planes ? stein_x3_split(v, theta_all, score_all, b.dtype, b.n, b.d, s, &fused) : STEIN_OK;
}

extern "C" int stein_svgd_phi(const void* theta_all, const void* score_all, int64_t n, int64_t d, int64_t row0,
                              int64_t n_local, int dtype, float* phi_local, float* h2_out, double* sqnorm_out,
                              float* K_out, float* dK_out, void* workspace, size_t ws_bytes, int flags, void* stream) {
  if (!theta_all || !score_all || !phi_local || !h2_out || !sqnorm_out || !workspace)
    return fail(STEIN_E_BADARG, "NULL pointer");
  if (row0 != 0 || n_local != n)
    return fail(STEIN_E_BADARG, "stein_svgd_phi is the single-rank path (row0 = 0, n_local = n); use the staged calls");
  const BlockShape b{n, d, row0, n_local, dtype};
  SteinLayout L;
  int rc = stein_make_layout(n_local, n, d, dtype, flags, &L);
  if (rc) return rc;
  if ((rc = stein_take_device_error())) return rc;
  if ((rc = check_block("stein_svgd_phi", b, (flags & STEIN_FLAG_X3) != 0))) return rc;
  if (ws_bytes < L.total) return fail(STEIN_E_WORKSPACE, "workspace %zu < %zu bytes", ws_bytes, L.total);
  const StepViews v = stein_step_views(L, workspace);
  hipStream_t s = (hipStream_t)stream;
  const bool ksd = (flags & STEIN_FLAG_KSD) != 0;
  const StageTimer clk(flags);
  if ((rc = clk.mark(STEIN_T_PREPARE, s))) return rc;
  if (!(flags & STEIN_FLAG_TILED) && stein_small_ok(n, d, dtype)) {
    for (int k = STEIN_T_DISTANCE; k <= STEIN_T_CONTRACT; ++k)
      if ((rc = clk.mark(k, s))) return rc;
    int nparts = 0;
    if ((rc = stein_small_phi((const float*)theta_all, (const float*)score_all, n, d, phi_local, h2_out, v.SQ, K_out,
                              dK_out, &nparts, sqnorm_out, ksd, s)))
      return rc;
    if ((rc = clk.mark(STEIN_T_FINISH, s))) return rc;
    if (nparts && (rc = sum_partials(v.SQ, nparts, ksd, sqnorm_out, s))) return rc;
    return clk.mark(STEIN_T_NSTAGES, s);
  }
  const bool fold_theta = L.fold && (dK_out || ksd);
  if ((rc = fused_prologue(v, b, theta_all, score_all, flags, s, L.fold ? (fold_theta ? 2 : 1) : 0))) return rc;
  if ((rc = clk.mark(STEIN_T_DISTANCE, s))) return rc;
  const int sf = STEIN_STAGE_SYMMETRIC | ((flags & STEIN_FLAG_TILE_DISTANCE) ? STEIN_STAGE_TILES : 0);
  if ((rc = distance_stage(v, b, theta_all, sf, true, s))) return rc;
  if ((rc = clk.mark(STEIN_T_MEDIAN, s))) return rc;
  if ((rc = stein_fused_select(v, n, d, h2_out, theta_all, score_all, s))) return rc;
  const bool upper = v.planes != nullptr;
  if (K_out && (rc = stein_kernel_matrix(v.D, L.ld_dist, n_local, n, h2_out, K_out, n,
                                         STEIN_STAGE_SYMMETRIC | (upper ? STEIN_STAGE_UPPER : 0), stream)))
    return rc;
  if (L.fold && (rc = stein_x3_split_w(v, (const float*)theta_all, (const float*)score_all, n, d, h2_out, s))) return rc;
  if ((rc = clk.mark(STEIN_T_CONTRACT, s))) return rc;
  if (L.fold) rc = stein_x3_contract_fold(v, h2_out, n, d, fold_theta, s);
  else rc = contract_stage(v, b, theta_all, score_all, h2_out, upper, s);
  if (rc) return rc;
  if ((rc = clk.mark(STEIN_T_FINISH, s))) return rc;
  if ((rc = finish_stage(v, b, theta_all, score_all, h2_out, phi_local, sqnorm_out, dK_out, ksd, (HistSync*)v.table, s)))
    return rc;
  return clk.mark(STEIN_T_NSTAGES, s);
}
```

Measured before the change: 27.45 million particle-updates/s.

## Fuse column-max scaling into prologue and select warm-up workgroups

Computes per-row absolute maxima inside the sqnorm prologue, with four rows processed per wave, and writes per-workgroup maxima. This lets the theta split kernel run without a separate column-max pass. Score/theta column maxima are now computed by the otherwise idle warm-up workgroups of the median-select kernel, replacing the cache-warming reads. A vec==2 finish path handles rows that are not 16-byte aligned. The goal is to remove a standalone colmax kernel launch and its extra full read of the inputs, at the cost of more complex fused kernels and a capped prologue grid.

```diff
diff --git a/stein_amd/csrc/stein_common.h b/stein_amd/csrc/stein_common.h
--- a/stein_amd/csrc/stein_common.h
+++ b/stein_amd/csrc/stein_common.h
@@ -162,18 +162,45 @@
 
 __device__ __forceinline__ float elem_f32(const float* p) { return *p; }
 __device__ __forceinline__ float elem_f32(const unsigned short* p) { return __uint_as_float((u32)*p << 16); }
+__device__ __forceinline__ u32 abs_bits(float v) { return __float_as_uint(v) & 0x7fffffffu; }
+__device__ __forceinline__ u32 abs_bits(unsigned short v) { return ((u32)v << 16) & 0x7fffffffu; }
 
 template <typename TIN>
-__device__ __forceinline__ float wave_row_sqnorm(const TIN* row, int d, int lane) {
+__device__ __forceinline__ float wave_row_sqnorm(const TIN* row, int d, int lane, u32& amax) {
   float s = 0.f;
   for (int k = lane; k < d; k += 64) {
     const float x = elem_f32(row + k);
     s = fmaf(x, x, s);
+    amax = max(amax, abs_bits(x));
   }
 #pragma unroll
   for (int o = 32; o > 0; o >>= 1) s += __shfl_xor(s, o);
   return s;
 }
+template <typename TIN>
+__device__ __forceinline__ float wave_row_sqnorm(const TIN* row, int d, int lane) {
+  u32 unused = 0u;
+  return wave_row_sqnorm(row, d, lane, unused);
+}
+template <int NR, typename TIN>
+__device__ __forceinline__ void wave_rows_sqnorm(const TIN* row, size_t stride, int d, int lane, float (&s)[NR], u32& amax) {
+#pragma unroll
+  for (int e = 0; e < NR; ++e) s[e] = 0.f;
+  for (int k = lane; k < d; k += 64) {
+    float x[NR];
+#pragma unroll
+    for (int e = 0; e < NR; ++e) x[e] = elem_f32(row + e * stride + k);
+#pragma unroll
+    for (int e = 0; e < NR; ++e) {
+      s[e] = fmaf(x[e], x[e], s[e]);
+      amax = max(amax, abs_bits(x[e]));
+    }
+  }
+#pragma unroll
+  for (int e = 0; e < NR; ++e)
+#pragma unroll
+    for (int o = 32; o > 0; o >>= 1) s[e] += __shfl_xor(s[e], o);
+}
 
 template <int N>
 __device__ __forceinline__ void block_sum256(double (&v)[N], double* red) {
@@ -192,6 +219,81 @@
 
 __device__ __forceinline__ u64 load_fresh(const u64* p) { return __hip_atomic_load(p, __ATOMIC_RELAXED, __HIP_MEMORY_SCOPE_AGENT); }
 __device__ __forceinline__ u32 load_fresh(const u32* p) { return __hip_atomic_load(p, __ATOMIC_RELAXED, __HIP_MEMORY_SCOPE_AGENT); }
+
+template <typename TIN, bool V4, int NM>
+__device__ __forceinline__ void colmax_scan(const TIN* const (&X)[NM], int n, int d, int col, long r, long step,
+                                            u32 (&m)[NM][V4 ? 4 : 1]) {
+  constexpr int CW = V4 ? 4 : 1;
+#pragma unroll
+  for (int z = 0; z < NM; ++z)
+#pragma unroll
+    for (int e = 0; e < CW; ++e) m[z][e] = 0u;
+  if (col >= d) return;
+  const size_t off = (size_t)step * d;
+  const TIN* p[NM];
+#pragma unroll
+  for (int z = 0; z < NM; ++z) p[z] = X[z] + (size_t)r * d + col;
+  if constexpr (V4) {
+    auto ld = [](const TIN* q) { return *reinterpret_cast<const float4*>(q); };
+    auto up = [](u32 (&a)[CW], const float4& v) {
+      a[0] = max(a[0], abs_bits(v.x)); a[1] = max(a[1], abs_bits(v.y));
+      a[2] = max(a[2], abs_bits(v.z)); a[3] = max(a[3], abs_bits(v.w));
+    };
+    for (; r + 3 * step < n; r += 4 * step) {
+      float4 v[NM][4];
+#pragma unroll
+      for (int z = 0; z < NM; ++z) {
+#pragma unroll
+        for (int k = 0; k < 4; ++k) v[z][k] = ld(p[z] + k * off);
+        p[z] += 4 * off;
+      }
+#pragma unroll
+      for (int z = 0; z < NM; ++z)
+#pragma unroll
+        for (int k = 0; k < 4; ++k) up(m[z], v[z][k]);
+    }
+    for (; r < n; r += step) {
+      float4 v[NM];
+#pragma unroll
+      for (int z = 0; z < NM; ++z) { v[z] = ld(p[z]); p[z] += off; }
+#pragma unroll
+      for (int z = 0; z < NM; ++z) up(m[z], v[z]);
+    }
+  } else {
+    for (; r + 3 * step < n; r += 4 * step) {
+      u32 v[NM][4];
+#pragma unroll
+      for (int z = 0; z < NM; ++z) {
+#pragma unroll
+        for (int k = 0; k < 4; ++k) v[z][k] = abs_bits(p[z][k * off]);
+        p[z] += 4 * off;
+      }
+#pragma unroll
+      for (int z = 0; z < NM; ++z) m[z][0] = max(max(m[z][0], v[z][0]), max(max(v[z][1], v[z][2]), v[z][3]));
+    }
+    for (; r < n; r += step) {
+#pragma unroll
+      for (int z = 0; z < NM; ++z) { m[z][0] = max(m[z][0], abs_bits(*p[z])); p[z] += off; }
+    }
+  }
+}
+
+template <int CW, int NM>
+__device__ __forceinline__ void colmax_commit(const u32 (&m)[NM][CW], int cx, int cb, int d, u32* red,
+                                              u32* __restrict__ cmax0, int dc) {
+  const int t = threadIdx.x, nt = blockDim.x;
+  for (int i = t; i < NM * 64 * CW; i += nt) red[i] = 0u;
+  __syncthreads();
+#pragma unroll
+  for (int z = 0; z < NM; ++z)
+#pragma unroll
+    for (int e = 0; e < CW; ++e) atomicMax(&red[(z * 64 + cx) * CW + e], m[z][e]);
+  __syncthreads();
+  for (int i = t; i < NM * 64 * CW; i += nt) {
+    const int z = i / (64 * CW), c = cb * 64 * CW + i % (64 * CW);
+    if (c < d) atomicMax(&cmax0[(size_t)z * dc + c], red[i]);
+  }
+}
 
 __device__ __forceinline__ void hist_add(u32* h, u32 digit, bool valid, int lane, u32 w = 1u) {
 #pragma unroll
@@ -536,8 +638,13 @@
   float* neutral_sc; int dc;
   u32* hsync; int hsync_words;
   u32 folded;
+  u32* wgmax;
 };
 constexpr int PRO_INIT_BLOCKS = 16;
+constexpr int PRO_MAX_WGS = 1024;
+constexpr int PRO_ROWS = 4;
+constexpr size_t PRO_WGMAX_AT = (sizeof(HistSync) + 255) / 256 * 256;
+static_assert(PRO_WGMAX_AT + (size_t)PRO_MAX_WGS * 4 <= (size_t)SPEC_TABLE * 8, "wgmax must fit behind HistSync in the table");
 template <typename TIN>
 __device__ __forceinline__ void prologue_body(const TIN* __restrict__ T, const PrologueArgs& a, int b, int nb) {
   const int gt = b * 256 + (int)threadIdx.x, gn = nb * 256;
@@ -550,8 +657,33 @@
   for (int i = gt; i < a.hsync_words; i += gn) a.hsync[i] = 0u;
   median_init_body(gt, gn, a.st, a.sp, a.total, a.hist, a.slots, a.allow_window);
   const int lane = threadIdx.x & 63;
-  for (int row = gt >> 6; row < a.n; row += gn >> 6) {
-    const float s = wave_row_sqnorm(T + (size_t)row * a.d, a.d, lane);
+  u32 amax = 0u;
+  const int wstep = gn >> 6;
+  int row = gt >> 6;
+  if constexpr (PRO_ROWS > 1) {
+    if (a.wgmax) {
+      for (; (long)row + (PRO_ROWS - 1) * (long)wstep < a.n; row += PRO_ROWS * wstep) {
+        float s[PRO_ROWS];
+        wave_rows_sqnorm<PRO_ROWS>(T + (size_t)row * a.d, (size_t)wstep * a.d, a.d, lane, s, amax);
+        if (lane == 0) {
+#pragma unroll
+          for (int e = 0; e < PRO_ROWS; ++e) a.r[row + e * wstep] = s[e];
+        }
+      }
+    }
+  }
+  for (; row < a.n; row += wstep) {
+    const float s = wave_row_sqnorm(T + (size_t)row * a.d, a.d, lane, amax);
     if (lane == 0) a.r[row] = s;
   }
-}
+  if (a.wgmax) {
+    __shared__ u32 s_amax;
+    if (threadIdx.x == 0) s_amax = 0u;
+    __syncthreads();
+#pragma unroll
+    for (int o = 32; o > 0; o >>= 1) amax = max(amax, (u32)__shfl_xor((int)amax, o));
+    if (lane == 0) atomicMax(&s_amax, amax);
+    __syncthreads();
+    if (threadIdx.x == 0) a.wgmax[b] = s_amax;
+  }
+}
diff --git a/stein_amd/csrc/stein_host.h b/stein_amd/csrc/stein_host.h
--- a/stein_amd/csrc/stein_host.h
+++ b/stein_amd/csrc/stein_host.h
@@ -63,7 +63,7 @@
 int stein_stream_jsplit_hook(void);
 
 int stein_fused_select(const StepViews& v, int64_t n, int64_t d, float* h2_out, const void* theta_all, const void* score_all,
-                       hipStream_t stream);
+                       bool want_maxima, bool* took_maxima, hipStream_t stream);
 
 int stein_fp32_distance(const StepViews& v, const BlockShape& b, const float* theta_all, bool symmetric, bool window,
                         hipStream_t stream);
diff --git a/stein_amd/csrc/stein_select.hip b/stein_amd/csrc/stein_select.hip
--- a/stein_amd/csrc/stein_select.hip
+++ b/stein_amd/csrc/stein_select.hip
@@ -575,12 +575,34 @@
   }
 }
 
+enum { SLICE_READ = 0, SLICE_MAX16 = 1, SLICE_MAX4 = 2 };
+template <bool V4>
+__device__ __forceinline__ void slice_maxima(const float* __restrict__ G, const float* __restrict__ T, int n, int d,
+                                             u32* __restrict__ cmax, int dc, int ncg, int nrg, u32* red) {
+  constexpr int CW = V4 ? 4 : 1;
+  const int w = (int)blockIdx.x - 1, cb = w % ncg, rg = w / ncg;
+  const int cx = threadIdx.x & 63, ry = threadIdx.x >> 6;
+  const float* const X[2] = {G, T};
+  u32 m[2][CW];
+  colmax_scan<float, V4, 2>(X, n, d, (cb * 64 + cx) * CW, (long)rg * 16 + ry, (long)nrg * 16, m);
+  colmax_commit<CW, 2>(m, cx, cb, d, red, cmax, dc);
+}
+
 __global__ __launch_bounds__(1024) void k_spec_select(SelState* st, SpecState* sp, const u64* __restrict__ slots,
                                                       float ln_n, float* h2_out, int update,
                                                       const float* __restrict__ D, long ldD, int n,
                                                       const float4* __restrict__ warm0, const float4* __restrict__ warm1,
-                                                      long warm4) {
+                                                      long warm4, int slice, int d, u32* __restrict__ cmax, int dc, int ncg,
+                                                      int nrg) {
   if (blockIdx.x) {
+    if (slice != SLICE_READ) {
+      __shared__ u32 red[2 * 256];
+      if (slice == SLICE_MAX16)
+        slice_maxima<true>((const float*)warm0, (const float*)warm1, n, d, cmax, dc, ncg, nrg, red);
+      else
+        slice_maxima<false>((const float*)warm0, (const float*)warm1, n, d, cmax, dc, ncg, nrg, red);
+      return;
+    }
     const long stride = (long)(gridDim.x - 1) * 1024;
     auto keep = [](const float4& a) { asm volatile("" ::"v"(a.x), "v"(a.y), "v"(a.z), "v"(a.w)); };
     long i = (long)(blockIdx.x - 1) * 1024 + threadIdx.x;
@@ -832,18 +854,31 @@
 }
 
 int stein_fused_select(const StepViews& v, int64_t n, int64_t d, float* h2_out, const void* theta_all,
-                       const void* score_all, hipStream_t s) {
+                       const void* score_all, bool want_maxima, bool* took_maxima, hipStream_t s) {
   const bool solo = n <= SOLO_MAX_N;
   long warm4 = 0;
-  int warm_wgs = 0;
-  if (v.L.fold && !g_no_warm && theta_all && score_all && (((uintptr_t)theta_all | (uintptr_t)score_all) & 15u) == 0) {
+  int warm_wgs = 0, slice = SLICE_READ, ncg = 1, nrg = 1;
+  const bool aligned = (((uintptr_t)theta_all | (uintptr_t)score_all) & 15u) == 0;
+  *took_maxima = false;
+  if (v.L.fold && !g_no_warm && theta_all && score_all && want_maxima) {
+    const bool v4 = aligned && d % 4 == 0;
+    slice = v4 ? SLICE_MAX16 : SLICE_MAX4;
+    const int64_t cw = v4 ? 256 : 64;
+    const int64_t blocks = (d + cw - 1) / cw, slots = (n + 15) / 16;
+    const int64_t max_rg = SPEC_WARM_WGS / blocks > 0 ? SPEC_WARM_WGS / blocks : 1;
+    const int64_t rounds = (slots + 4 * max_rg - 1) / (4 * max_rg);
+    ncg = (int)blocks;
+    nrg = (int)((slots + 4 * rounds - 1) / (4 * rounds));
+    warm_wgs = ncg * nrg;
+    *took_maxima = true;
+  } else if (v.L.fold && !g_no_warm && theta_all && score_all && aligned) {
     warm4 = (long)(n * d) >> 2;
     const long want = (warm4 + 8191) / 8192;
     warm_wgs = (int)(want < SPEC_WARM_WGS ? want : SPEC_WARM_WGS);
   }
   hipLaunchKernelGGL(k_spec_select, dim3(1 + warm_wgs), dim3(1024), 0, s, v.sel, v.spec, v.spec_buf, (float)log((double)n),
                      h2_out, 1, solo ? (const float*)v.D : (const float*)nullptr, (long)v.L.ld_dist, (int)n,
-                     (const float4*)theta_all, (const float4*)score_all, warm4);
+                     (const float4*)score_all, (const float4*)theta_all, warm4, slice, (int)d, v.cmax, (int)v.L.x3_dc, ncg, nrg);
   LAUNCH_CHECK("k_spec_select");
   if (solo) return STEIN_OK;
   const HistFinal fin{v.sel, v.spec, h2_out, (float)log((double)n)};
diff --git a/stein_amd/csrc/stein_x3.h b/stein_amd/csrc/stein_x3.h
--- a/stein_amd/csrc/stein_x3.h
+++ b/stein_amd/csrc/stein_x3.h
@@ -6,12 +6,15 @@
   HistSync* done;
   const PrologueArgs* prologue;
   int fold;
+  const u32* wgmax; int nwg;
 };
 int stein_x3_split(const StepViews& v, const void* theta_all, const void* score_all, int dtype, int64_t n, int64_t d,
                    hipStream_t stream, const SplitFused* fused);
 bool stein_fold_pays(int64_t n, int64_t d);
 int stein_x3_split_w(const StepViews& v, const float* theta_all, const float* score_all, int64_t n, int64_t d,
                      const float* h2_dev, hipStream_t stream);
+int stein_x3_colmax(const StepViews& v, const float* theta_all, const float* score_all, int64_t n, int64_t d,
+                    hipStream_t stream);
 int stein_x3_contract_fold(const StepViews& v, const float* h2_dev, int64_t n, int64_t d, bool with_theta,
                            hipStream_t stream);
 int stein_x3_distance(const StepViews& v, const BlockShape& b, bool symmetric, bool window, hipStream_t stream,
diff --git a/stein_amd/csrc/stein_x3.hip b/stein_amd/csrc/stein_x3.hip
--- a/stein_amd/csrc/stein_x3.hip
+++ b/stein_amd/csrc/stein_x3.hip
@@ -26,34 +26,35 @@
   }
 }
 
-__device__ __forceinline__ u32 abs_bits(float v) { return __float_as_uint(v) & 0x7fffffffu; }
-__device__ __forceinline__ u32 abs_bits(u16 v) { return ((u32)v << 16) & 0x7fffffffu; }
+
+__device__ __forceinline__ void write_global_scales(float* __restrict__ sc, int dc, int sa, int pexp) {
+  sc[4 * dc + 0] = pow2i(sa);
+  sc[4 * dc + 1] = pow2i(1 - 2 * sa);
+  sc[4 * dc + 2] = pow2i(-pexp);
+}
 
 __device__ __forceinline__ void make_scales_body(const u32* cmax, int dc, float* __restrict__ sc, int pexp, int enable,
                                                  u32* red) {
   const int t = threadIdx.x;
-  u32 m = 0u;
-  for (int c = t; c < dc; c += 256) {
-    const u32 mg = load_fresh(cmax + c), mt = load_fresh(cmax + dc + c);
-    const int sg = enable ? scale_exp(mg, 100) : 0, st = enable ? scale_exp(mt, 100) : 0;
-    sc[c] = pow2i(sg);
-    sc[dc + c] = pow2i(st);
-    sc[2 * dc + c] = pow2i(-sg - pexp);
-    sc[3 * dc + c] = pow2i(-st - pexp);
-    m = max(m, mt);
-  }
-  red[t] = m;
+  if (t < 256) {
+    u32 m = 0u;
+    for (int c = t; c < dc; c += 256) {
+      const u32 mg = load_fresh(cmax + c), mt = load_fresh(cmax + dc + c);
+      const int sg = enable ? scale_exp(mg, 100) : 0, st = enable ? scale_exp(mt, 100) : 0;
+      sc[c] = pow2i(sg);
+      sc[dc + c] = pow2i(st);
+      sc[2 * dc + c] = pow2i(-sg - pexp);
+      sc[3 * dc + c] = pow2i(-st - pexp);
+      m = max(m, mt);
+    }
+    red[t] = m;
+  }
   __syncthreads();
   for (int o = 128; o > 0; o >>= 1) {
     if (t < o) red[t] = max(red[t], red[t + o]);
     __syncthreads();
   }
-  if (t == 0) {
-    const int sa = enable ? scale_exp(red[0], 60) : 0;
-    sc[4 * dc + 0] = pow2i(sa);
-    sc[4 * dc + 1] = pow2i(1 - 2 * sa);
-    sc[4 * dc + 2] = pow2i(-pexp);
-  }
+  if (t == 0) write_global_scales(sc, dc, enable ? scale_exp(red[0], 60) : 0, pexp);
 }
 
 template <typename TIN, bool V4>
@@ -61,58 +62,14 @@
                                                             u32* __restrict__ cmax0, int dc, int zbase, float* __restrict__ sc,
                                                             int pexp, HistSync* done) {
   const int z = blockIdx.z + zbase;
-  const TIN* __restrict__ X = z ? X1 : X0;
-  u32* __restrict__ cmax = cmax0 + (z ? dc : 0);
   constexpr int CW = V4 ? 4 : 1;
   constexpr int NW = V4 ? 16 : 4;
-  __shared__ u32 red[NW][64 * CW];
+  __shared__ u32 red[256];
   const int t = threadIdx.x, cx = t & 63, ry = t >> 6;
-  const int col = (blockIdx.x * 64 + cx) * CW;
-  u32 m[CW];
-#pragma unroll
-  for (int e = 0; e < CW; ++e) m[e] = 0u;
-  if (col < d) {
-    const long step = (long)gridDim.y * NW;
-    long r = (long)blockIdx.y * NW + ry;
-    if constexpr (V4) {
-      if constexpr (std::is_same<TIN, float>::value) {
-        u32 m1[4] = {0u, 0u, 0u, 0u}, m2[4] = {0u, 0u, 0u, 0u}, m3[4] = {0u, 0u, 0u, 0u};
-        auto ld = [&](long row) { return *reinterpret_cast<const float4*>(X + (size_t)row * d + col); };
-        auto up = [&](u32 (&acc)[4], const float4& v) {
-          acc[0] = max(acc[0], abs_bits(v.x)); acc[1] = max(acc[1], abs_bits(v.y));
-          acc[2] = max(acc[2], abs_bits(v.z)); acc[3] = max(acc[3], abs_bits(v.w));
-        };
-        for (; r + 3 * step < n; r += 4 * step) {
-          const float4 a0 = ld(r), a1 = ld(r + step), a2 = ld(r + 2 * step), a3 = ld(r + 3 * step);
-          up(m, a0); up(m1, a1); up(m2, a2); up(m3, a3);
-        }
-        for (; r < n; r += step) { const float4 a0 = ld(r); up(m, a0); }
-#pragma unroll
-        for (int e = 0; e < 4; ++e) m[e] = max(max(m[e], m1[e]), max(m2[e], m3[e]));
-      }
-    } else {
-      u32 m1 = 0u, m2 = 0u, m3 = 0u;
-      for (; r + 3 * step < n; r += 4 * step) {
-        const u32 a0 = abs_bits(X[(size_t)r * d + col]), a1 = abs_bits(X[(size_t)(r + step) * d + col]);
-        const u32 a2 = abs_bits(X[(size_t)(r + 2 * step) * d + col]), a3 = abs_bits(X[(size_t)(r + 3 * step) * d + col]);
-        m[0] = max(m[0], a0); m1 = max(m1, a1); m2 = max(m2, a2); m3 = max(m3, a3);
-      }
-      for (; r < n; r += step) m[0] = max(m[0], abs_bits(X[(size_t)r * d + col]));
-      m[0] = max(max(m[0], m1), max(m2, m3));
-    }
-  }
-#pragma unroll
-  for (int e = 0; e < CW; ++e) red[ry][cx * CW + e] = m[e];
-  __syncthreads();
-  if (t < 64 * CW) {
-    const int c = blockIdx.x * 64 * CW + t;
-    if (c < d) {
-      u32 v = 0u;
-#pragma unroll
-      for (int w = 0; w < NW; ++w) v = max(v, red[w][t]);
-      atomicMax(&cmax[c], v);
-    }
-  }
+  const TIN* const X[1] = {z ? X1 : X0};
+  u32 m[1][CW];
+  colmax_scan<TIN, V4, 1>(X, n, d, ((int)blockIdx.x * 64 + cx) * CW, (long)blockIdx.y * NW + ry, (long)gridDim.y * NW, m);
+  colmax_commit<CW, 1>(m, cx, (int)blockIdx.x, d, red, cmax0 + (z ? dc : 0), dc);
   if (done) {
     __shared__ u32 s_last;
     asm volatile("s_waitcnt vmcnt(0)" ::: "memory");
@@ -122,7 +79,7 @@
       s_last = tree_report_done(done->cm_leaf, &done->cm_top, id, gridDim.x * gridDim.y * gridDim.z) ? 1u : 0u;
     }
     __syncthreads();
-    if (s_last) make_scales_body(cmax0, dc, sc, pexp, 1, &red[0][0]);
+    if (s_last) make_scales_body(cmax0, dc, sc, pexp, 1, red);
   }
 }
 
@@ -223,6 +180,43 @@
   tp_store<KIND>(tile, Tt, ntk_t, dc, nk, row0, col0, t);
 }
 
+__global__ __launch_bounds__(256) void k_split_rows(const float* __restrict__ X, int n, int d, u16* __restrict__ R, long r_rows,
+                                                    int dk, int dc, float* __restrict__ sc, int vec,
+                                                    const u32* __restrict__ wgmax, int nwg) {
+  __shared__ u32 s_wmax[4];
+  const int t = threadIdx.x;
+  const int row0 = blockIdx.y * 64, col = blockIdx.x * 64 + (t & 15) * 4;
+  const long ntk_r = dk >> 5;
+  u32 m = 0u;
+  for (int i = t; i < nwg; i += 256) m = max(m, wgmax[i]);
+  float v[2][2][4];
+#pragma unroll
+  for (int p = 0; p < 2; ++p)
+#pragma unroll
+    for (int h = 0; h < 2; ++h) load_row4(X, row0 + 2 * tp_pair(t, p) + h, col, n, d, vec, v[p][h]);
+#pragma unroll
+  for (int o = 32; o > 0; o >>= 1) m = max(m, (u32)__shfl_xor((int)m, o));
+  if ((t & 63) == 0) s_wmax[t >> 6] = m;
+  __syncthreads();
+  const int sae = scale_exp(max(max(s_wmax[0], s_wmax[1]), max(s_wmax[2], s_wmax[3])), 60);
+  const float sa = pow2i(sae);
+  if (t == 0 && blockIdx.x == 0 && blockIdx.y == 0) write_global_scales(sc, dc, sae, PEXP_H2);
+#pragma unroll
+  for (int p = 0; p < 2; ++p)
+#pragma unroll
+    for (int h = 0; h < 2; ++h) {
+      const int row = row0 + 2 * tp_pair(t, p) + h;
+      if (row < r_rows && col < dk) {
+        u32 wa[3], wb[3];
+        split_pair<2>(v[p][h][0] * sa, v[p][h][1] * sa, wa);
+        split_pair<2>(v[p][h][2] * sa, v[p][h][3] * sa, wb);
+        u16* dst = R + (((size_t)(row >> 7) * ntk_r + (col >> 5)) * 3) * XTILE_E + vfrag_offset(row & 127, (col & 31) >> 3) + (col & 7);
+#pragma unroll
+        for (int s = 0; s < 2; ++s) *reinterpret_cast<uint2*>(dst + s * XTILE_E) = make_uint2(wa[s], wb[s]);
+      }
+    }
+}
+
 __global__ __launch_bounds__(256) void k_split_w(const float* __restrict__ T, const float* __restrict__ G, int n, int d,
                                                  u16* __restrict__ Wt, int dc, long nk, float* __restrict__ sc,
                                                  const u32* __restrict__ cmax, const float* __restrict__ h2p, int vec) {
@@ -242,6 +236,9 @@
     if (blockIdx.y == 0 && (t >> 4) == 0 && c < dc) {
       sc[c] = scq[q];
       sc[2 * dc + c] = pow2i(-se - PEXP_H2);
+      const int st = scale_exp(cmax[dc + c], 100);
+      sc[dc + c] = pow2i(st);
+      sc[3 * dc + c] = pow2i(-st - PEXP_H2);
     }
   }
 #pragma unroll
@@ -745,6 +742,26 @@
                      (long)L.x3_rows, (int)L.x3_dk, Tt3, Gt3, (int)L.x3_dc, (long)L.x3_nk, sc, zbase, PrologueArgs{}, vec);
 }
 
+static void launch_colmax(const StepViews& v, const float* score_all, const float* theta_all, int64_t n, int64_t d,
+                          HistSync* fuse_done, hipStream_t stream) {
+  const int dc = (int)v.L.x3_dc;
+  const int zbase = score_all ? 0 : 1;
+  const unsigned nz = (score_all ? 1u : 0u) + (theta_all ? 1u : 0u);
+  int gy = (int)((n + 63) / 64);
+  if (gy > 256) gy = 256;
+  const bool v4 = d % 4 == 0 && (!score_all || ((uintptr_t)score_all & 15) == 0) && (!theta_all || ((uintptr_t)theta_all & 15) == 0);
+  if (v4) {
+    const int gy4 = gy > 64 ? 64 : gy;
+    const dim3 grid((unsigned)((d + 255) / 256), (unsigned)gy4, nz);
+    hipLaunchKernelGGL((k_colmax<float, true>), grid, dim3(1024), 0, stream, score_all, theta_all, (int)n, (int)d, v.cmax, dc,
+                       zbase, v.sc, PEXP_H2, fuse_done);
+  } else {
+    const dim3 grid((unsigned)((d + 63) / 64), (unsigned)gy, nz);
+    hipLaunchKernelGGL((k_colmax<float, false>), grid, dim3(256), 0, stream, score_all, theta_all, (int)n, (int)d, v.cmax, dc,
+                       zbase, v.sc, PEXP_H2, fuse_done);
+  }
+}
+
 int stein_x3_split(const StepViews& v, const void* theta_all, const void* score_all, int dtype, int64_t n, int64_t d,
                    hipStream_t stream, const SplitFused* fused) {
   const SteinLayout& L = v.L;
@@ -753,23 +770,20 @@
   HistSync* fuse_done = fused && theta_all && score_all ? fused->done : nullptr;
   const PrologueArgs* prologue = fused ? fused->prologue : nullptr;
   const int fold = fused ? fused->fold : 0;
+  const u32* wgmax = fused && kind == 2 && fold == 1 ? fused->wgmax : nullptr;
+  if (wgmax) {
+    const int vec = d % 4 == 0 && ((uintptr_t)theta_all & 15u) == 0;
+    const dim3 grid((unsigned)((L.x3_dk + 63) / 64), (unsigned)((L.x3_rows + 63) / 64));
+    hipLaunchKernelGGL(k_split_rows, grid, dim3(256), 0, stream, (const float*)theta_all, (int)n, (int)d, v.T3, (long)L.x3_rows,
+                       (int)L.x3_dk, dc, v.sc, vec, wgmax, fused->nwg);
+    LAUNCH_CHECK("k_split_rows");
+    return STEIN_OK;
+  }
   if (kind == 2) {
     const int zbase = score_all ? 0 : 1;
     const unsigned nz = (score_all ? 1u : 0u) + (theta_all ? 1u : 0u);
     if (!fuse_done) HIP_TRY(hipMemsetAsync(v.cmax + (size_t)zbase * dc, 0, (size_t)nz * dc * sizeof(u32), stream));
-    int gy = (int)((n + 63) / 64);
-    if (gy > 256) gy = 256;
-    const bool v4 = d % 4 == 0 && (!score_all || ((uintptr_t)score_all & 15) == 0) && (!theta_all || ((uintptr_t)theta_all & 15) == 0);
-    if (v4) {
-      const int gy4 = gy > 64 ? 64 : gy;
-      const dim3 grid((unsigned)((d + 255) / 256), (unsigned)gy4, nz);
-      hipLaunchKernelGGL((k_colmax<float, true>), grid, dim3(1024), 0, stream, (const float*)score_all, (const float*)theta_all,
-                         (int)n, (int)d, v.cmax, dc, zbase, v.sc, PEXP_H2, fuse_done);
-    } else {
-      const dim3 grid((unsigned)((d + 63) / 64), (unsigned)gy, nz);
-      hipLaunchKernelGGL((k_colmax<float, false>), grid, dim3(256), 0, stream, (const float*)score_all, (const float*)theta_all,
-                         (int)n, (int)d, v.cmax, dc, zbase, v.sc, PEXP_H2, fuse_done);
-    }
+    launch_colmax(v, (const float*)score_all, (const float*)theta_all, n, d, fuse_done, stream);
     LAUNCH_CHECK("k_colmax");
   }
   if (kind == 2 ? !fuse_done : !prologue) {
@@ -787,6 +801,13 @@
 
 constexpr double FOLD_MIN_WORK = 4.0e9;
 bool stein_fold_pays(int64_t n, int64_t d) { return d > 128 && (double)n * (double)n * (double)d >= FOLD_MIN_WORK; }
+
+int stein_x3_colmax(const StepViews& v, const float* theta_all, const float* score_all, int64_t n, int64_t d,
+                    hipStream_t stream) {
+  launch_colmax(v, score_all, theta_all, n, d, nullptr, stream);
+  LAUNCH_CHECK("k_colmax");
+  return STEIN_OK;
+}
 
 int stein_x3_split_w(const StepViews& v, const float* theta_all, const float* score_all, int64_t n, int64_t d,
                      const float* h2_dev, hipStream_t stream) {
diff --git a/stein_amd/csrc/steinhip.hip b/stein_amd/csrc/steinhip.hip
--- a/stein_amd/csrc/steinhip.hip
+++ b/stein_amd/csrc/steinhip.hip
@@ -76,7 +76,7 @@
   const double ih = 1.0 / (double)h2;
   const bool need_t = !FOLD || KSD || dK != nullptr;
   auto kg = [&](float o, float t) { return FOLD ? (double)o + (double)t * ih : (double)o; };
-  if (vec) {
+  if (vec == 1) {
     const long total4 = total >> 2;
     const int d4 = d >> 2;
     auto run = [&](auto nz, auto nt) {
@@ -156,6 +156,30 @@
     else if (split == 2) run_nz(integral_constant<int, 2>());
     else if (split == 4) run_nz(integral_constant<int, 4>());
     else run(integral_constant<int, 0>(), integral_constant<int, 0>());
+  } else if (vec == 2) {
+    for (long q = (long)blockIdx.x * 256 + threadIdx.x; q < (total >> 2); q += (long)gridDim.x * 256) {
+      const int i = (int)(q / (d >> 2));
+      float rs = 0.f;
+      for (int z = 0; z < split; ++z) rs += RS[(size_t)z * n_local + i];
+      double p2[4];
+#pragma unroll
+      for (int c = 0; c < 4; ++c) {
+        const long e = (q << 2) + c;
+        float og = 0.f, ot = 0.f;
+        for (int z = 0; z < split; ++z) {
+          og += OG[z * zs + e];
+          if (FOLD ? need_t && z < tsplit : true) ot += OT[z * zs + e];
+        }
+        const float th = elem_f32(T + (size_t)row0 * d + e);
+        const float dk = (rs * th - ot) / h2;
+        const float ph = FOLD ? (og + rs * th / h2) / fn : (og + dk) / fn;
+        phi[e] = ph;
+        if (dK) dK[e] = dk;
+        p2[c] = (double)ph * (double)ph;
+        if constexpr (KSD) ksd_terms(elem_f32(G + (size_t)row0 * d + e), kg(og, ot), ot, th, rs, ih, ks, kd);
+      }
+      sq += (p2[0] + p2[1]) + (p2[2] + p2[3]);
+    }
   } else {
     for (long e = (long)blockIdx.x * 256 + threadIdx.x; e < total; e += (long)gridDim.x * 256) {
       const int i = (int)(e / d);
@@ -454,8 +478,8 @@
   auto al16 = [](const void* p) { return ((uintptr_t)p & 15u) == 0; };
   const size_t tsz = b.dtype == STEIN_BF16 ? 2 : 4;
   auto rows_aligned = [&](const void* p) { return (((uintptr_t)p + (size_t)b.row0 * b.d * tsz) & (4 * tsz - 1)) == 0; };
-  const int vec = (b.d % 4 == 0) && al16(v.OG) && al16(v.OT) && al16(phi_local) && al16(dK_out) && rows_aligned(theta_all) &&
-                  (!ksd || rows_aligned(score_all));
+  const bool group4 = (b.d % 4 == 0) && al16(v.OG) && al16(v.OT) && al16(phi_local) && al16(dK_out);
+  const int vec = !group4 ? 0 : (rows_aligned(theta_all) && (!ksd || rows_aligned(score_all))) ? 1 : 2;
   auto launch = [&](auto tin, auto ksd_tag, auto fold_tag) {
     using TIN = decltype(tin);
     hipLaunchKernelGGL((k_phi_finish<TIN, decltype(ksd_tag)::value, decltype(fold_tag)::value>), dim3((unsigned)L.sq_blocks),
@@ -789,9 +813,12 @@
   pa.neutral_sc = bf16_split ? v.sc : (float*)nullptr;
   pa.dc = (int)v.L.x3_dc;
   pa.folded = fold ? 1u : 0u;
-  const SplitFused fused{(HistSync*)v.table, bf16_split ? &pa : nullptr, fold};
+  pa.wgmax = fold == 1 ? (u32*)((char*)v.table + PRO_WGMAX_AT) : (u32*)nullptr;
+  int64_t nwg = (b.n + 3) / 4 + PRO_INIT_BLOCKS;
+  if (pa.wgmax && nwg > PRO_MAX_WGS) nwg = PRO_MAX_WGS;
+  const SplitFused fused{(HistSync*)v.table, bf16_split ? &pa : nullptr, fold, pa.wgmax, (int)nwg};
   if (bf16_split) return stein_x3_split(v, theta_all, score_all, b.dtype, b.n, b.d, s, &fused);
-  const dim3 grid((unsigned)((b.n + 3) / 4 + PRO_INIT_BLOCKS));
+  const dim3 grid((unsigned)nwg);
   if (b.dtype == STEIN_BF16)
     hipLaunchKernelGGL(k_prologue<unsigned short>, grid, dim3(256), 0, s, (const unsigned short*)theta_all, pa);
   else
@@ -836,7 +863,11 @@
   const int sf = STEIN_STAGE_SYMMETRIC | ((flags & STEIN_FLAG_TILE_DISTANCE) ? STEIN_STAGE_TILES : 0);
   if ((rc = distance_stage(v, b, theta_all, sf, true, s))) return rc;
   if ((rc = clk.mark(STEIN_T_MEDIAN, s))) return rc;
-  if ((rc = stein_fused_select(v, n, d, h2_out, theta_all, score_all, s))) return rc;
+  const bool want_maxima = L.fold && !fold_theta;
+  bool slice_maxima = false;
+  if ((rc = stein_fused_select(v, n, d, h2_out, theta_all, score_all, want_maxima, &slice_maxima, s))) return rc;
+  if (want_maxima && !slice_maxima && (rc = stein_x3_colmax(v, (const float*)theta_all, (const float*)score_all, n, d, s)))
+    return rc;
   const bool upper = v.planes != nullptr;
   if (K_out && (rc = stein_kernel_matrix(v.D, L.ld_dist, n_local, n, h2_out, K_out, n,
                                          STEIN_STAGE_SYMMETRIC | (upper ? STEIN_STAGE_UPPER : 0), stream)))
```

Measured after the change: 27.77 million particle-updates/s, median of 6. 1.01x the previous value.
